# smarterclayton/kubernetes

Measured on AMD Instinct MI355X. Metric: pods scheduled/sec, higher is better.
Workload: dtype int64; 1 GPU; config2: 5000 nodes, 1776000 pods, DefaultProvider; nodes=5000, prefix_pods=0, placed_in_prefix=0, parallelism=speculative windows: all-CU snapshot scoring + in-order exact resolver

## Files before the change

kubernetes_amd/csrc/ksg_internal.h:

```cpp
#pragma once
#include <stdint.h>
#include "../../include/kschedgpu.h"

#define KSG_NT 1024
#define KSG_NWAVE (KSG_NT / 64)
#define KSG_R_LDS 32
#define KSG_R_MAX 128

#define KSG_MODE_EVAL 0
#define KSG_MODE_BEGIN 1

#define KSG_SCORE_NONE (-0x7fffffffffffffffLL - 1)
#define KSG_S32_NONE ((int32_t)0x80000000)
#define KSG_SCORE_BOUND (1LL << 30)
#define KSG_WIN_MAX_ANTI 4
#define KSG_WIN_LR_BOUND (1LL << 49)
#define KSG_WIN_XREQ_BOUND (1LL << 16)

struct KsgDev {
  uint32_t n_nodes, nw;
  uint32_t lo, hi;
  uint32_t wlo, nwords;
  uint32_t n_pairs, n_services, max_keys, n_domains_total;
  uint32_t preds;
  int64_t w_lr, w_spread;
  uint32_t n_anti;
  int64_t w_anti[KSG_MAX_ANTI];
  uint32_t anti_dom_off[KSG_MAX_ANTI];
  uint32_t n_aff;
  uint32_t n_aff_groups;
  uint32_t aff_group_mask[KSG_MAX_AFF_GROUPS];
  int32_t equal_fallback;
  int32_t empty_priorities;
  int32_t has_static_score;
  int32_t has_static_fit;
  int32_t dbg;
  int32_t wide;
  uint32_t rr_dz;
  int32_t* dbgbuf;
  const int64_t* cap_cpu;
  const int64_t* cap_mem;
  const double* inv10_cpu;
  const double* inv10_mem;
  int64_t* used_cpu;
  int64_t* used_mem;
  const uint64_t* draws;
  const uint64_t* static_fit;
  const int64_t* static_score;
  uint64_t* keymap;
  const uint64_t* pairmap;
  int32_t* svc_cnt;
  uint64_t* svc_bits;
  int32_t* svc_max;
  int32_t* svc_total;
  int32_t* svc_peer;
  const int32_t* anti_domain;
  const int32_t* aff_pair;
  void* score_scratch;
  uint32_t ext_filters;
  int32_t w_taint, w_bal;
  uint32_t n_scalar;
  const int64_t* scalar_cap;
  int64_t* scalar_used;
  const uint64_t* taintmap;
  const uint64_t* ntaint;
};

struct KsgStaticCfg {
  uint32_t n_presence;
  uint32_t presence_n_keys[KSG_MAX_PRESENCE];
  uint32_t presence_keys[KSG_MAX_PRESENCE][KSG_MAX_PRESENCE_KEYS];
  uint32_t presence_flag[KSG_MAX_PRESENCE];
  uint32_t n_pref;
  uint32_t pref_key[KSG_MAX_LABEL_PREF];
  uint32_t pref_presence[KSG_MAX_LABEL_PREF];
  int64_t w_pref[KSG_MAX_LABEL_PREF];
  int64_t w_equal;
  uint32_t n_anti;
  uint32_t anti_key[KSG_MAX_ANTI];
  uint32_t n_aff;
  uint32_t aff_key[KSG_MAX_AFF];
};

#define KSG_WIN_INLINE 24
#define KSG_WIN_SUM_AFF 4
struct KsgWinSum {
  int32_t m0;
  uint32_t k0;
  int32_t error;
  int32_t service;
  int32_t host;
  int32_t spread_max;
  int32_t svc_total;
  uint32_t n_inline;
  int64_t milli_cpu;
  int64_t memory;
  int32_t req_aff[KSG_WIN_SUM_AFF];
  uint16_t n_ports, n_pds, n_sel, n_svcs;
  uint32_t xmask;
  uint32_t ids[KSG_WIN_INLINE];
  int32_t xreq[4];
  uint32_t pad2;
};
static_assert(sizeof(KsgWinSum) == 192, "KsgWinSum layout");
#define KSG_WIN_SUM_DWORDS (sizeof(KsgWinSum) / 4)

#define KSG_MAX_WORLD 16
struct KsgWinXchg {
  const uint8_t* buf;
  uint64_t blk;
  uint32_t ostride;
  uint32_t wcap;
  uint32_t world;
  uint32_t fit_off;
  uint32_t wlo[KSG_MAX_WORLD], nw[KSG_MAX_WORLD];
  int32_t* dcnt;
  uint32_t dcnt_n;
  uint8_t* img;
  const ksg_pod_ext* exts;
  uint32_t img_stride;
  uint32_t esc;
  uint32_t efit_off;
  uint32_t d1;
  uint32_t d1_off;
  int32_t* tmax;
  uint64_t* psoft;
  int32_t* thist;
  uint32_t rr;
  uint32_t dz;
  uint32_t b_off;
  int32_t* dmb;
  const uint64_t* zmap;
};
#define KSG_TBINS 65
#define KSG_RR_MAXZ 32
#define KSG_RR_MAXSVC 4096

#define KSG_HALT_OVERSIZE 4
#define KSG_HALT_BADCOUNT 8
#define KSG_HALT_HANG 9
#define KSG_HALT_BAD 10
struct KsgWinRun {
  uint32_t pos;
  uint32_t n;
  uint32_t halt;
  uint32_t windows;
  uint32_t stops[4];
};

struct KsgFused {
  const ksg_pod* batch;
  const uint32_t* ids;
  KsgWinRun* run_out;
  uint32_t* cnt;
  uint32_t set;
  uint32_t ngroups;
};

typedef ksg_shard_record KsgRecordHdr;

#define KSG_EXPLAIN_TILE 256
#define KSG_EXPLAIN_CHUNK 32

#define KSG_ADMIT_MODE_CAPACITY 1
#define KSG_ADMIT_MODE_SELECTOR 2

struct KsgPatch {
  uint64_t addr;
  uint64_t value;
  uint32_t width;
  uint32_t pad;
};

#define KSG_SRV_CHUNKS 64
#define KSG_SRV_CHUNK_DW 3
#define KSG_SRV_HDR_DW 8
#define KSG_SRV_INLINE_DW (KSG_SRV_CHUNKS * KSG_SRV_CHUNK_DW - KSG_SRV_HDR_DW)
#define KSG_SRV_EXT_DW 4096
#define KSG_SRV_PAY_DW (KSG_SRV_INLINE_DW + KSG_SRV_EXT_DW)
#define KSG_SRV_PATCHES 4096
#define KSG_SRV_MAX_R 16
enum {
  KSG_SRV_BEGIN = 1,
  KSG_SRV_COMMIT = 2,
  KSG_SRV_PATCH = 3,
  KSG_SRV_EXIT = 4,
};
enum { KSG_SRVH_KIND = 0, KSG_SRVH_ARG, KSG_SRVH_RSV, KSG_SRVH_FLAGS, KSG_SRVH_PAYDW, KSG_SRVH_IDS_AT,
       KSG_SRVH_EXT_AT, KSG_SRVH_NPATCH };
#define KSG_SRV_BADREQ 0xFFFFFFFEu
#define KSG_SRV_RESP_REJECTED 12
#define KSG_SRVF_WANT_FAIL 1u
#define KSG_SRVF_EXT 2u
#define KSG_GSRV_NT 256
#define KSG_GSRV_MAXW 255
#define KSG_GSRV_TIEW 16
#define KSG_GSRV_MAXD 64
struct alignas(64) KsgSrvPart {
  uint32_t seq;
  int32_t max;
  uint32_t cnt;
  uint32_t err;
  uint64_t tie[4];
  uint32_t stamp[4];
};
struct KsgSrvBox {
  uint32_t req[KSG_SRV_CHUNKS * 4];
  uint32_t creq[KSG_SRV_CHUNKS * 4];
  uint32_t cext[KSG_SRV_EXT_DW];
  uint32_t resp[16];
  uint32_t ext[KSG_SRV_EXT_DW];
  KsgPatch patch[KSG_SRV_PATCHES];
  uint32_t dbg[256];
  uint64_t ties[KSG_SRV_MAX_R * 16];
  KsgSrvPart part[KSG_GSRV_MAXW];
  uint64_t part_tie[KSG_GSRV_MAXW * KSG_GSRV_TIEW];
};
struct KsgSrvGrid {
  uint32_t quit;
  uint32_t applied;
  uint32_t pad[14];
  uint64_t tmx[KSG_GSRV_MAXW];
  uint64_t dcx[KSG_GSRV_MAXW * KSG_GSRV_MAXD];
};
struct KsgSrvArgs {
  KsgSrvBox* box;
  uint8_t* fail;
  uint32_t start_seq;
  uint64_t idle_ticks;
  uint32_t stamps;
  KsgSrvGrid* grid;
  uint32_t n_workers;
  uint32_t epoch;
  uint32_t grid_opts;
};
#define KSG_GSRV_POLL1 256u

#ifdef __HIP__
#define KSG_HD __host__ __device__
#else
#define KSG_HD
#endif

static inline KSG_HD uint64_t ksg_splitmix_next(uint64_t* s) {
  uint64_t z = (*s += 0x9E3779B97F4A7C15ULL);
  z = (z ^ (z >> 30)) * 0xBF58476D1CE4E5B9ULL;
  z = (z ^ (z >> 27)) * 0x94D049BB133111EBULL;
  return z ^ (z >> 31);
}
static inline KSG_HD uint64_t ksg_rng_step(const uint64_t* draws) { return draws ? 1ULL : 0x9E3779B97F4A7C15ULL; }
static inline KSG_HD uint64_t ksg_rng_draw(const uint64_t* draws, uint64_t s) {
  if (draws) return draws[s];
  return ksg_splitmix_next(&s) >> 1;
}
```

kubernetes_amd/csrc/ksg_plain.hip:

```cpp
#include "ksg_resolver.h"
#include "ksg_score.h"

#define KSG_NCAND 6
#define KSG_CSV_MAX 10
#define KSG_NO_CAND 7u
#define KSG_CSNAP 10
#define KSG_XR_W 20
#ifndef KSG_PL_PROD_SLEEP
#define KSG_PL_PROD_SLEEP 1
#endif
#ifndef KSG_PL_CHK_SLEEP
#define KSG_PL_CHK_SLEEP 2
#endif
#ifndef KSG_PL_XN_SLEEP
#define KSG_PL_XN_SLEEP 0
#endif
__host__ __device__ constexpr uint32_t pl_nt(int P) { return P >= 32 ? 512u : 768u; }
#define KSG_PL_FW KSG_RES_P0
#define KSG_PL_P0 (KSG_PL_FW + 1)
__host__ __device__ constexpr bool pl_d1(uint32_t P) { return P <= 4; }

struct alignas(16) PlCommit {
  uint32_t kind;
  uint32_t slot;
// ... 1689 lines not shown
        const uint32_t na = (uint32_t)__builtin_amdgcn_readlane((int)(lo ? cn0 : cn1), (int)l);
        const uint32_t bd = (uint32_t)__popcll(__ballot(d0 < pa)) + (uint32_t)__popcll(__ballot(d1 < pa)) +
                            (xdp < pa ? 1u : 0u);
        const uint32_t ba = (uint32_t)__popcll(__ballot(ap0 != ~0u && (ap0 < pa || (ap0 == pa && cn0 < na)))) +
                            (uint32_t)__popcll(__ballot(ap1 != ~0u && (ap1 < pa || (ap1 == pa && cn1 < na))));
        if (pa - bd + ba == t) woff = na;
      }
      for (uint32_t j = 0; woff == ~0u && j <= n_add && j <= t; ++j) {
        const uint32_t tp = t0_minus_drops(t - j);
        if (tp >= k0) continue;
        const uint32_t ca = (uint32_t)__popcll(__ballot(ap0 != ~0u && ap0 <= tp)) +
                            (uint32_t)__popcll(__ballot(ap1 != ~0u && ap1 <= tp));
        if (ca == j) woff = t0_node(tp);
      }
    } else if (dropped == 0) {
      woff = (uint32_t)pred;
    } else if (dropped <= 2) {
      KSG_COUNTP(7, 64)
      uint32_t pa = ~0u, pb = ~0u;
      for (uint64_t mm = msk0; mm; mm &= mm - 1) {
        const uint32_t p = (uint32_t)__builtin_amdgcn_readlane((int)dp0, (int)__builtin_ctzll(mm));
        if (p < pa) { pb = pa; pa = p; } else if (p < pb) { pb = p; }
      }
      for (uint64_t mm = msk1; mm; mm &= mm - 1) {
        const uint32_t p = (uint32_t)__builtin_amdgcn_readlane((int)dp1, (int)__builtin_ctzll(mm));
        if (p < pa) { pb = pa; pa = p; } else if (p < pb) { pb = p; }
      }
      if (x_drop) {
        const uint32_t p = xpos0 + (uint32_t)__popcll(t0x & ((1ULL << (xnode & 63)) - 1ULL));
        if (p < pa) { pb = pa; pa = p; } else if (p < pb) { pb = p; }
      }
      const uint32_t ix = (uint32_t)__builtin_amdgcn_readlane((int)rmod, (int)dropped);
      const uint32_t t = k - 1 - ix;
      uint32_t tp = t;
      if (pa <= tp) ++tp;
      if (pb <= tp) ++tp;
      woff = (uint32_t)__builtin_amdgcn_readlane((int)cand, (int)((dropped == 1 ? 1u : 3u) + (tp - t)));
    } else {
      KSG_COUNTP(7, 64)
      uint32_t ix;
      if (dropped < 64) {
        ix = (uint32_t)__builtin_amdgcn_readlane((int)rmod, (int)dropped);
      } else {
        ix = umod64_32(r_draw(), k);
      }
      woff = t0_node(t0_minus_drops(k - 1 - ix));
    }
    if (KSG_UNLIKELY(woff >= d.hi - d.lo)) {
      resolved = i;
      reason = KSG_STOP_BAD;
      break;
    }
    const uint64_t cm = __ballot(cand == woff);
    const uint32_t cidx = cm ? (uint32_t)__builtin_ctzll(cm) : KSG_NO_CAND;
    if (lane == 0) {
      L_cm[i].xn = woff | (cidx << 28);
      if constexpr (STAMP) ctl->t_n = (uint32_t)__builtin_amdgcn_s_memtime();
      st_post(&ctl->xn_seq, i + 1);
    }
    KSG_STAMPP(3)
    const uint64_t hit0 = __ballot(cn0 == woff);
    const uint64_t hit1 = __ballot(cn1 == woff);
    const bool in_c = (hit0 | hit1) != 0;
    uint32_t slot, base_nk = 0, base_ns = 0;
    int64_t base_dc = 0, base_dm = 0;
    if (in_c) {
      slot = hit0 ? (uint32_t)__builtin_ctzll(hit0) : 64u + (uint32_t)__builtin_ctzll(hit1);
      const uint32_t sl = slot & 63;
      base_nk = (uint32_t)__builtin_amdgcn_readlane((int)(slot < 64 ? sk0 : sk1), (int)sl);
      base_ns = (uint32_t)__builtin_amdgcn_readlane((int)(slot < 64 ? ss0 : ss1), (int)sl);
      if (KSG_UNLIKELY(base_nk + nk > KSG_SLOT_KEYS || base_ns + n_svcs > KSG_SLOT_SVCS)) {
        resolved = i;
        reason = KSG_STOP_SLOT;
        break;
      }
      base_dc = (int64_t)readlane64((uint64_t)(slot < 64 ? dc0 : dc1), (int)sl);
      base_dm = (int64_t)readlane64((uint64_t)(slot < 64 ? dm0 : dm1), (int)sl);
    } else {
      if (KSG_UNLIKELY(n_slots == KSG_MAX_SLOTS)) {
        resolved = i;
        reason = KSG_STOP_SLOT;
        break;
      }
      slot = n_slots++;
    }
    const int64_t new_dc = (int64_t)((uint64_t)base_dc + (uint64_t)pv.req_c);
    const int64_t new_dm = (int64_t)((uint64_t)base_dm + (uint64_t)pv.req_m);
    const uint32_t wn = d.lo + woff;
    KSG_STAMPP(4)
    {
      uint32_t* row = L_cl + (size_t)slot * KSG_CL_W;
      const uint32_t kt = lane - WS_IDS, st_ = lane - (WS_IDS + nk + n_sel);
      if (kt < nk) row[KSG_CL_KEY + base_nk + kt] = rec;
      if (st_ < n_svcs) row[KSG_CL_SV + base_ns + st_] = rec;
    }
    if (lane == 0) {
      *reinterpret_cast<uint4*>(&L_cm[i]) =
          uint4{1u, slot, woff, (in_c ? 0u : 1u) | (cidx << 1) | (n_svcs << 8) | (base_ns << 16) | (base_nk << 24)};
      L_cm[i].out = (int32_t)wn;
      st_post(&ctl->sel_seq, i + 1);
    }
    if ((int32_t)woff != pred) KSG_COUNTP(8, 64)
    if (lane == (slot & 63)) {
      if (slot >= 64) {
        if (!in_c) cn1 = woff;
        dc1 = new_dc;
        dm1 = new_dm;
        sk1 = base_nk + nk;
        ss1 = base_ns + n_svcs;
      } else {
        if (!in_c) cn0 = woff;
        dc0 = new_dc;
        dm0 = new_dm;
        sk0 = base_nk + nk;
        ss0 = base_ns + n_svcs;
      }
    }
    have_x = true;
    xnode = woff;
    xslot = slot;
    x_fresh = !in_c;
    ++n_draws;
    KSG_STAMPP(5)
  }
  if (lane == 0) {
    ctl->resolved = resolved;
    st_rel(&ctl->stop, 1u);
  }
  bool drained = false;
  for (uint32_t spin = 0; spin <= 16 * KSG_SPIN_LIMIT; ++spin) {
    bool done = ld_acq(&ctl->fin_x) != 0 && ld_acq(&ctl->fin_f) != 0;
#pragma unroll
    for (int c = 0; c < KSG_RES_NCHK; ++c) done = done && ld_acq(&ctl->fin[c]) != 0;
    if (done) {
      drained = true;
      break;
    }
  }
  if (ld_acq(&ctl->bad)) reason = KSG_STOP_BAD;
  else if (!drained || ld_acq(&ctl->hang)) reason = KSG_STOP_HANG;
  if constexpr (STAMP) {
    if (d.dbgbuf && (lane < 16 || lane == 43 || lane == 44)) atomicAdd(d.dbgbuf + lane, (int32_t)(t_acc / 64));
  }
#undef KSG_STAMPP
#undef KSG_COUNTP
  const uint32_t n_peer = __builtin_amdgcn_readfirstlane(ctl->n_peer);
  for (uint32_t t = lane; t < n_peer; t += 64) {
    const uint32_t sv = L_peer[2 * t];
    int32_t expect = -1;
    __hip_atomic_compare_exchange_strong(d.svc_peer + sv, &expect, (int32_t)L_peer[2 * t + 1], __ATOMIC_RELAXED,
                                         __ATOMIC_RELAXED, __HIP_MEMORY_SCOPE_AGENT);
  }
  for (uint32_t t = lane; t < resolved; t += 64) out[t] = L_cm[t].out;
  if (esc && x.tmax) {
    for (uint32_t t = lane; t < wcap; t += 64) x.tmax[t] = 0;
    for (uint32_t t = lane; t < n_pods * KSG_TBINS; t += 64) x.thist[t] = 0;
  }
  if (XS) {
    for (uint32_t t = lane; t < resolved; t += 64) {
      if (L_cm[t].kind != 1) continue;
      const ksg_pod_ext& pe = x.exts[pos + t];
      const uint32_t wn = d.lo + L_cm[t].node;
      for (uint32_t r = 0; r < d.n_scalar; ++r)
        if (pe.scalar[r] != 0)
          __hip_atomic_fetch_add(reinterpret_cast<uint64_t*>(d.scalar_used + (size_t)r * d.n_nodes + wn),
                                 (uint64_t)pe.scalar[r], __ATOMIC_RELAXED, __HIP_MEMORY_SCOPE_AGENT);
    }
    drain_stores();
  }
  if (lane == 0) {
    *rng_io = rng0 + (uint64_t)n_draws * ksg_rng_step(d.draws);
    if constexpr (STAMP && FUSED)
      if (d.dbgbuf) __hip_atomic_store(d.dbgbuf + 55, 0, __ATOMIC_RELAXED, __HIP_MEMORY_SCOPE_AGENT);
    KsgWinRun r = *run;
    if (reason == KSG_STOP_HANG) {
      r.halt = KSG_HALT_HANG;
    } else if (reason == KSG_STOP_BAD) {
      r.halt = KSG_HALT_BAD;
    } else if (reason == KSG_STOP_OVERSIZE) {
      r.halt = KSG_HALT_OVERSIZE;
    } else if (resolved == 0 || resolved > n_pods) {
      r.halt = KSG_HALT_BADCOUNT;
    } else {
      r.pos = pos + resolved;
      r.windows += 1;
      r.stops[1] += reason == 1 ? 1u : 0u;
      r.stops[2] += reason == 2 ? 1u : 0u;
      r.stops[3] += reason == 3 ? 1u : 0u;
    }
    *run_out = r;
  }
}

template <int P, bool STAMP, bool XS>
__global__ __launch_bounds__(pl_nt(P)) void ksg_win_plain_kernel(KsgDev d, uint32_t wcap, KsgWinRun* run,
                                                            const KsgWinSum* __restrict__ sums, const KsgWinXchg x,
                                                            uint64_t* rng_io, int32_t* __restrict__ out_batch) {
  win_plain_body<P, STAMP, XS, false>(d, wcap, run, sums, x, rng_io, out_batch, KsgFused{});
}

template <int P, bool STAMP>
__global__ __launch_bounds__(pl_nt(P)) void ksg_win_fused_kernel(KsgDev d, uint32_t wcap, KsgWinRun* run,
                                                            const KsgWinSum* __restrict__ sums, const KsgWinXchg x,
                                                            uint64_t* rng_io, int32_t* __restrict__ out_batch,
                                                            const KsgFused f) {
  win_plain_body<P, STAMP, false, true>(d, wcap, run, sums, x, rng_io, out_batch, f);
}

template <int PP, bool ST, bool XS, bool FU = false>
static hipError_t win_plain_launch_x(const KsgDev& d, uint32_t wcap, size_t lds, KsgWinRun* run,
                                     const KsgWinSum* sums, const KsgWinXchg& x, uint64_t* rng, int32_t* out,
                                     hipStream_t st, const KsgFused& f = KsgFused{}, uint32_t grid = 1) {
  const void* fn;
  if constexpr (FU) fn = reinterpret_cast<const void*>(ksg_win_fused_kernel<PP, ST>);
  else fn = reinterpret_cast<const void*>(ksg_win_plain_kernel<PP, ST, XS>);
  static bool once = false;
  if (!once) {
    (void)hipFuncSetAttribute(fn, hipFuncAttributeMaxDynamicSharedMemorySize, 160 * 1024);
    (void)hipGetLastError();
    once = true;
  }
  if constexpr (FU)
    hipLaunchKernelGGL((ksg_win_fused_kernel<PP, ST>), dim3(grid), dim3(pl_nt(PP)), lds, st, d, wcap, run, sums, x,
                       rng, out, f);
  else
    hipLaunchKernelGGL((ksg_win_plain_kernel<PP, ST, XS>), dim3(grid), dim3(pl_nt(PP)), lds, st, d, wcap, run, sums,
                       x, rng, out);
  return hipGetLastError();
}

static bool plain_xs(const KsgDev& d, const KsgWinXchg& x) {
  return x.exts != nullptr && (((d.ext_filters & KSG_EXT_SCALAR) && d.n_scalar > 0) || x.esc);
}

static bool plain_stamp(const KsgDev& d) { return (d.dbg & 8) != 0 || ((uint32_t)d.dbg & KSG_DBG_RESOLVER_MASK) != 0; }

#define KSG_PLAIN_CASE(PP, XS)                                                                              \
  if (P == PP)                                                                                              \
    return plain_stamp(d) ? win_plain_launch_x<PP, true, XS>(d, wcap, lds, run, sums, x, rng, out, st)    \
                          : win_plain_launch_x<PP, false, XS>(d, wcap, lds, run, sums, x, rng, out, st);

hipError_t ksg_launch_win_plain_ilp(const KsgDev& d, uint32_t P, uint32_t wcap, size_t lds, KsgWinRun* run,
                                    const KsgWinSum* sums, const KsgWinXchg& x, uint64_t* rng, int32_t* out,
                                    hipStream_t st)
#ifdef KSG_PLAIN_LARGE_TU
{
  if (plain_xs(d, x)) {
    KSG_PLAIN_CASE(1, true)
    KSG_PLAIN_CASE(2, true)
    KSG_PLAIN_CASE(4, true)
    KSG_PLAIN_CASE(8, true)
    KSG_PLAIN_CASE(16, true)
    KSG_PLAIN_CASE(32, true)
  } else {
    KSG_PLAIN_CASE(16, false)
    KSG_PLAIN_CASE(32, false)
  }
  return hipErrorInvalidValue;
}
#else
    ;

static uint32_t plain_P(const KsgDev& d);
uint32_t ksg_win_plain_lds(const KsgDev& d, uint32_t wcap) {
  return plain_lds_offsets(plain_P(d), (d.n_services + 31) / 32, wcap).total;
}

static uint32_t plain_P(const KsgDev& d) {
  const uint32_t P = (d.nwords + 63) / 64;
  return P <= 1 ? 1 : P <= 2 ? 2 : P <= 4 ? 4 : P <= 8 ? 8 : P <= 16 ? 16 : 32;
}

uint32_t ksg_win_t0_stride(const KsgDev& d) { return t0img_stride(plain_P(d)); }

hipError_t ksg_launch_win_t0(const KsgDev& d, uint32_t wcap, const KsgWinRun* run, const KsgWinXchg& x,
                             hipStream_t st) {
  const uint32_t P = plain_P(d);
#define KSG_T0_CASE(PP) \
  if (P == PP) hipLaunchKernelGGL((ksg_win_t0_kernel<PP>), dim3(wcap), dim3(256), 0, st, d.nwords, wcap, run, x);
  KSG_T0_CASE(1)
  KSG_T0_CASE(2)
  KSG_T0_CASE(4)
  KSG_T0_CASE(8)
  KSG_T0_CASE(16)
  KSG_T0_CASE(32)
#undef KSG_T0_CASE
  return hipGetLastError();
}

hipError_t ksg_launch_win_plain(const KsgDev& d, uint32_t P, uint32_t wcap, KsgWinRun* run, const KsgWinSum* sums,
                                const KsgWinXchg& x, uint64_t* rng, int32_t* out, hipStream_t st) {
  const size_t lds = plain_lds_offsets(P, (d.n_services + 31) / 32, wcap).total;
  if (P >= 16 || plain_xs(d, x)) return ksg_launch_win_plain_ilp(d, P, wcap, lds, run, sums, x, rng, out, st);
  KSG_PLAIN_CASE(1, false)
  KSG_PLAIN_CASE(2, false)
  KSG_PLAIN_CASE(4, false)
  KSG_PLAIN_CASE(8, false)
  return hipErrorInvalidValue;
}

bool ksg_win_fused_ok(const KsgDev& d) { return plain_P(d) >= 1 && d.nwords > 0; }

uint32_t ksg_win_fused_groups(const KsgDev& d, uint32_t wcap) {
  const uint32_t pg = (uint32_t)pl_pg((int)plain_P(d));
  return (wcap + pg - 1) / pg;
}

hipError_t ksg_launch_win_fused(const KsgDev& d, uint32_t wcap, KsgWinRun* run, const KsgWinSum* sums,
                                const KsgWinXchg& x, uint64_t* rng, int32_t* out, const KsgFused& f, uint32_t grid,
                                hipStream_t st) {
  const uint32_t P = plain_P(d);
  const size_t lds = std::max<size_t>(plain_lds_offsets(P, (d.n_services + 31) / 32, wcap).total,
                                      (size_t)(pl_nt(P) / 64) * pl_pg((int)P) * sizeof(KsgWinSum));
  const bool stamp = plain_stamp(d);
#define KSG_FUSED_CASE(PP)                                                                                  \
  if (P == PP)                                                                                              \
    return stamp ? win_plain_launch_x<PP, true, false, true>(d, wcap, lds, run, sums, x, rng, out, st, f, grid) \
                 : win_plain_launch_x<PP, false, false, true>(d, wcap, lds, run, sums, x, rng, out, st, f, grid);
  KSG_FUSED_CASE(1)
  KSG_FUSED_CASE(2)
  KSG_FUSED_CASE(4)
  KSG_FUSED_CASE(8)
  KSG_FUSED_CASE(16)
  KSG_FUSED_CASE(32)
#undef KSG_FUSED_CASE
  return hipErrorInvalidValue;
}
#endif
#undef KSG_PLAIN_CASE
```

kubernetes_amd/csrc/ksg_runtime.cpp:

```cpp
#include <hip/hip_runtime.h>
#include <rccl/rccl.h>

#include <algorithm>
#include <array>
#include <atomic>
#include <chrono>
#include <cmath>
#include <cstdarg>
#include <cstdio>
#include <cstring>
#include <map>
#include <mutex>
#include <string>
#include <unordered_map>
#include <unordered_set>
#include <vector>

#include "ksg_internal.h"
#include "ksg_shard.h"


hipError_t ksg_launch_batch(int R, bool anti, const KsgDev& d, const ksg_pod* pods,
                            const uint32_t* ids, uint32_t n, uint64_t* rng, int32_t* out,
                            hipStream_t st, const ksg_pod_ext* ext = nullptr);
hipError_t ksg_launch_scan(int R, bool anti, const KsgDev& d, const ksg_pod* pods,
                           const uint32_t* ids, int mode, int phase, uint8_t* fail_out,
                           int64_t* score_out, uint8_t* record, int32_t* dpart,
                           const int32_t* dglobal, hipStream_t st, const ksg_pod_ext* ext = nullptr);
hipError_t ksg_launch_win_eval(const KsgDev& d, int mode, const ksg_pod* batch, const uint32_t* ids,
                               const KsgWinRun* run, uint32_t wcap, KsgWinSum* sums, uint64_t* wbits, int32_t* wmax,
                               uint32_t ostride, int32_t* dcnt, uint64_t* wfit, int32_t* dmb, uint64_t* wbz,
                               uint32_t dz, hipStream_t st, const ksg_pod_ext* exts = nullptr,
                               int32_t* tmax = nullptr, uint64_t* psoft = nullptr, int32_t* thist = nullptr);
hipError_t ksg_launch_zonemap(uint32_t n_nodes, const int32_t* anti_domain, uint32_t d0, uint32_t nw,
                              uint64_t* zmap, hipStream_t st);
hipError_t ksg_launch_win_t0(const KsgDev& d, uint32_t wcap, const KsgWinRun* run, const KsgWinXchg& x,
                             hipStream_t st);
uint32_t ksg_win_t0_stride(const KsgDev& d);
hipError_t ksg_launch_win_resolve(const KsgDev& d, uint32_t wcap, KsgWinRun* run, const KsgWinSum* sums,
                                  const KsgWinXchg& x, uint64_t* rng, int32_t* out, hipStream_t st);
bool ksg_win_fused_ok(const KsgDev& d);
uint32_t ksg_win_fused_groups(const KsgDev& d, uint32_t wcap);
hipError_t ksg_launch_win_fused(const KsgDev& d, uint32_t wcap, KsgWinRun* run, const KsgWinSum* sums,
                                const KsgWinXchg& x, uint64_t* rng, int32_t* out, const KsgFused& f, uint32_t grid,
                                hipStream_t st);
uint32_t ksg_win_max_window(const KsgDev& d);
hipError_t ksg_launch_decide(const KsgDev& d, const ksg_pod* pods, const uint32_t* ids,
                             const uint8_t* records, uint32_t rec_bytes, uint32_t world,
                             const uint32_t* shard_wlo, int mode, uint64_t tie_index,
                             uint64_t* rng, int32_t* out, uint32_t out_idx, int64_t* summary,
                             hipStream_t st, const ksg_pod_ext* ext = nullptr);
hipError_t ksg_launch_static(const KsgStaticCfg& sc, uint32_t n_nodes, const ksg_node* nodes,
                             const uint32_t* node_pairs, const uint32_t* pair_keys,
                             const int32_t* dom_of_pair, uint32_t n_pairs, uint32_t nw,
                             uint64_t* static_fit, int64_t* static_score, int32_t* anti_domain,
                             int32_t* aff_pair, unsigned long long* pairmap, hipStream_t st);
hipError_t ksg_launch_patch(const KsgPatch* patches, uint32_t n, hipStream_t st);
hipError_t ksg_launch_static_terms(const KsgStaticCfg& sc, uint32_t n_nodes, const ksg_node* nodes,
                                   const uint32_t* node_pairs, const uint32_t* pair_keys, uint32_t n_pairs, uint32_t nw,
                                   uint64_t* fit, int64_t* score, hipStream_t st);
hipError_t ksg_launch_static_fold(uint64_t* static_fit, int64_t* static_score, const uint64_t* xfit,
                                  const int64_t* xscore, uint32_t nw, uint32_t n, int own_fit, int own_score,
                                  hipStream_t st);
hipError_t ksg_launch_serve(int R, bool anti, bool ext, const KsgDev& d, const KsgSrvArgs& a, hipStream_t st);
hipError_t ksg_launch_serve_grid(int npt, bool ext, const KsgDev& d, const KsgSrvArgs& a, hipStream_t st);
hipError_t ksg_launch_admit(const ksg_admission_set* sets, uint32_t n_sets, const ksg_pod* pods,
                            const uint32_t* ids, const uint32_t* pairs, int mode, uint8_t* out, hipStream_t st);
hipError_t ksg_launch_explain(const KsgDev& d, const ksg_pod* pods, const ksg_pod_ext* exts, const uint32_t* ids,
                              uint32_t n_pods, uint8_t* codes, uint32_t* hist, uint8_t* err, hipStream_t st);

namespace {

struct PodRec {
  uint32_t host;
  int64_t cpu, mem;
  int64_t scalar[KSG_MAX_SCALAR];
  std::vector<uint32_t> keys;
  std::vector<uint32_t> svcs;
  uint64_t seq;
};

constexpr uint32_t kMaxNodesPerShard = KSG_R_MAX * KSG_NT;
constexpr uint32_t kFctlGroups = 1024;
constexpr size_t kFctlRuns = 2 * sizeof(KsgWinRun);
constexpr size_t kFctlBytes = kFctlRuns + (size_t)2 * kFctlGroups * 8 * sizeof(uint32_t);
constexpr size_t kExplainStageBytes = (size_t)64 << 20;

const unsigned kTimingEvent =
    (getenv("KSG_EVENT_FENCE") && atoi(getenv("KSG_EVENT_FENCE"))) ? hipEventDefault : hipEventDisableSystemFence;

}

struct ksg_ctx {
  ksg_config cfg{};
  int device = 0, rank = 0, world = 1;
  hipStream_t st = nullptr;
  ncclComm_t comm = nullptr;
  bool xchg = false;
  double ppw_est = 0.0;
  double round_margin = 1.0;
  uint8_t* h_up = nullptr;
  size_t h_up_cap = 0;
  uint8_t* h_dn = nullptr;
  size_t h_dn_cap = 0;
  ksg_allgather_fn xfn = nullptr;
  void* xuser = nullptr;
  uint8_t *h_xsend = nullptr, *h_xrecv = nullptr;
  size_t h_xsend_cap = 0, h_xrecv_cap = 0;
  hipEvent_t ev0 = nullptr, ev1 = nullptr;
  hipEvent_t ev_wait = nullptr;
  bool spin_wait = true;
  double last_ms = 0.0;
  std::string err;

  bool have_cluster = false;
  bool diverged = false;
  uint32_t N = 0, nw = 0, n_pairs = 0, S = 0, D = 0;
  uint32_t lo = 0, hi = 0, wlo = 0, nwords = 0, nwords_max = 0;
  std::vector<uint32_t> shard_wlo_h;
  int R = 1;
  size_t lds = 0;
  KsgDev dev{};
  std::vector<void*> cluster_allocs;
  uint32_t* d_shard_wlo = nullptr;

  ksg_pod* d_pods = nullptr;
  size_t pods_cap = 0;
  uint32_t* d_ids = nullptr;
  size_t ids_cap = 0;
  uint8_t* d_fail = nullptr;
  int64_t* d_score = nullptr;
  uint8_t* d_rec_send = nullptr;
  uint8_t* d_rec_recv = nullptr;
  uint32_t rec_bytes = 0;
  int32_t* d_dpart = nullptr;
  int32_t* d_dglobal = nullptr;
  int32_t* d_out = nullptr;
  size_t out_cap = 0;
  uint64_t* d_rng = nullptr;
  int64_t* d_summary = nullptr;
  uint8_t* d_one = nullptr;
  size_t one_cap = 0;
  const ksg_pod* one_pod = nullptr;
  const uint32_t* one_ids = nullptr;
  uint8_t* h_map = nullptr;
  uint8_t* d_map = nullptr;
  KsgPatch* d_patch = nullptr;
  size_t patch_cap = 0;
  uint64_t* d_draws = nullptr;
  size_t draws_cap = 0;
  uint64_t draw_tmp = 0;
  uint8_t* d_admit = nullptr;
  size_t admit_cap = 0;
  uint8_t* d_xcodes = nullptr;
  size_t xcodes_cap = 0;
  uint8_t* d_xhist = nullptr;
  size_t xhist_cap = 0;
  hipEvent_t ev_x0 = nullptr, ev_x1 = nullptr;
  double last_explain_ms = 0.0;
  std::vector<KsgPatch> patches;

  std::vector<int64_t> used_c, used_m;
  int64_t mu_max = 0;
  bool mu_neg = false, mu_dirty = true;
  std::unordered_map<uint64_t, uint32_t> key_ref;
  std::vector<int32_t> svc_cnt;
  std::vector<std::unordered_map<uint32_t, int32_t>> svc_ext;
  std::vector<int32_t> svc_max, svc_total, svc_peer;
  std::vector<int32_t> h_aff_pair;
  std::vector<std::map<uint64_t, uint32_t>> svc_members;
  std::unordered_map<uint64_t, PodRec> pods;
  uint64_t seq = 0;

  uint32_t window = 128;
  uint32_t ev_stride = 4;
  uint32_t ev_phase = 0;
  KsgWinSum* d_winsum = nullptr;
  uint8_t* d_xsend = nullptr;
  uint8_t* d_xrecv = nullptr;
  uint8_t* d_t0img = nullptr;
  size_t t0img_cap = 0;
  int32_t* d_dcnt = nullptr;
  int32_t* d_dmb = nullptr;
  uint64_t* d_zmap = nullptr;
  size_t win_cap = 0, xsend_cap = 0, xrecv_cap = 0, dcnt_cap = 0, dmb_cap = 0;
  int32_t* d_etmax = nullptr;
  int32_t* d_ethist = nullptr;
  size_t ethist_cap = 0;
  uint64_t* d_epsoft = nullptr;
  size_t etmax_cap = 0, epsoft_cap = 0;
  KsgWinRun* d_run = nullptr;
  KsgWinRun* h_run = nullptr;
  uint32_t last_stats[4] = {0, 0, 0, 0};
  std::vector<hipEvent_t> wev;
  double last_kms[3] = {0, 0, 0};
  double last_t0ms = 0;
  double last_wsum = 0;
  bool dbg_fail_next = false;
  uint32_t dbg_corrupt = 0;
  bool win_d1 = true;
  bool win_fused = true;
  uint32_t fused_grid = 0;
  uint32_t fused_max_words = 1024;
  uint8_t* d_fctl = nullptr;
  uint8_t* h_fctl = nullptr;
  double last_hus[8] = {0, 0, 0, 0, 0, 0, 0, 0};
  double totals[24] = {};
  int64_t max_cap = 0, min_cap = 0;

  std::vector<ksg_pod> dfr_pods;
  std::vector<uint32_t> dfr_ids;
  std::vector<int32_t> dfr_out;
  std::unordered_set<uint64_t> dfr_uids;
  int64_t dfr_sum = 0;
  bool dfr_neg = false;
  bool lr_wild = false;
  int64_t used_hi = 0;
  unsigned __int128 dfr_req = 0;

  bool ext_on = false;
  ksg_ext_config ext{};
  std::vector<int64_t> sc_used;
  std::unordered_map<uint64_t, std::array<int64_t, KSG_MAX_SCALAR>> ext_scalar;
  const ksg_pod_ext* cur_ext = nullptr;
  ksg_pod_ext* d_pext = nullptr;
  size_t pext_cap = 0;
  ksg_pod_ext* d_one_ext = nullptr;

  bool srv_enabled = true;
  bool srv_running = false;
  KsgSrvBox* srv_box = nullptr;
  KsgSrvBox* srv_dbox = nullptr;
  uint8_t* srv_fail = nullptr;
  uint8_t* srv_dfail = nullptr;
  size_t srv_fail_cap = 0;
  uint32_t srv_seq = 0;
  uint64_t srv_idle_us = 20000;
  bool pend_srv = false;
  uint32_t srv_bhdr[KSG_SRV_HDR_DW] = {};
  std::vector<uint64_t> srv_tw;
  uint32_t srv_unacked = 0;
  uint32_t srv_served = 0;
  uint32_t srv_last_ctl = 0;
  bool srv_pext_on = false;
  ksg_pod_ext srv_pext{};
  uint64_t srv_launches = 0;
  bool srv_grid_on = true;
  uint32_t srv_npt4_min = 16384;
  uint32_t srv_grid_min = 0;
  bool srv_grid_ext = true;
  KsgSrvGrid* srv_grid = nullptr;
  size_t srv_grid_cap = 0;
  uint32_t srv_epoch = 0;
  bool srv_stamps = false;
  int64_t srv_grid_opts = -1;
  bool srv_debug = false;
  unsigned __int128 static_mag = 0;
  const ksg_node* d_lbl_nodes = nullptr;
  const uint32_t* d_lbl_pairs = nullptr;
  const uint32_t* d_lbl_keys = nullptr;
  bool srv_trace = false;
  double srv_stage[6] = {};
  uint64_t srv_stamped = 0;

  bool pending = false;
  uint64_t pending_k = 0;
  ksg_pod pend{};
  std::vector<uint32_t> pend_ids;

  std::recursive_mutex mu;
  struct Queued {
    bool add;
    uint32_t host;
    ksg_pod pod;
    std::vector<uint32_t> ids;
    uint64_t uid;
  };
  std::vector<Queued> upd_q;
  std::unordered_set<uint64_t> q_added, q_removed;
};

#define KSG_LOCK(c) std::lock_guard<std::recursive_mutex> ksg_lock_((c)->mu)

namespace {

int fail(ksg_ctx* c, int code, const char* fmt, ...) {
  char buf[512];
  va_list ap;
  va_start(ap, fmt);
  vsnprintf(buf, sizeof buf, fmt, ap);
  va_end(ap);
  if (c) c->err = buf;
  return code;
}

#define HIPCHK(c, x)                                                                 \
  do {                                                                               \
    hipError_t e_ = (x);                                                             \
    if (e_ != hipSuccess)                                                            \
      return fail((c), KSG_ERR_HIP, "%s:%d %s: %s", __FILE__, __LINE__, #x,          \
                  hipGetErrorString(e_));                                            \
  } while (0)

#define NCCLCHK(c, x)                                                                \
  do {                                                                               \
    ncclResult_t r_ = (x);                                                           \
    if (r_ != ncclSuccess)                                                           \
      return fail((c), KSG_ERR_RCCL, "%s:%d %s: %s", __FILE__, __LINE__, #x,         \
                  ncclGetErrorString(r_));                                           \
  } while (0)

template <typename T>
int dalloc(ksg_ctx* c, T** p, size_t count, std::vector<void*>* owner) {
  void* q = nullptr;
  HIPCHK(c, hipMalloc(&q, std::max<size_t>(count, 1) * sizeof(T)));
  HIPCHK(c, hipMemsetAsync(q, 0, std::max<size_t>(count, 1) * sizeof(T), c->st));
  *p = static_cast<T*>(q);
  if (owner) owner->push_back(q);
  return KSG_OK;
}

void free_cluster(ksg_ctx* c) {
  for (void* p : c->cluster_allocs) (void)hipFree(p);
  c->cluster_allocs.clear();
  c->have_cluster = false;
}

int grow(ksg_ctx* c, void** p, size_t* cap, size_t need, size_t elem) {
  if (need <= *cap && *p) return KSG_OK;
  size_t nc = std::max<size_t>(need, std::max<size_t>(*cap * 2, 64));
  if (*p) (void)hipFree(*p);
  *p = nullptr;
  HIPCHK(c, hipMalloc(p, nc * elem));
  *cap = nc;
  return KSG_OK;
}

int pick_R(uint32_t shard_nodes) {
  const uint32_t r = (shard_nodes + KSG_NT - 1) / KSG_NT;
  int R = 1;
  while ((uint32_t)R < r) R <<= 1;
  return R;
}

void patch32(ksg_ctx* c, const void* addr, int32_t v) {
  c->patches.push_back(KsgPatch{(uint64_t)(uintptr_t)addr, (uint64_t)(uint32_t)v, 0, 0});
}
void patch64(ksg_ctx* c, const void* addr, int64_t v) {
  c->patches.push_back(KsgPatch{(uint64_t)(uintptr_t)addr, (uint64_t)v, 1, 0});
}
void patch_or(ksg_ctx* c, const void* addr, uint64_t v) {
  c->patches.push_back(KsgPatch{(uint64_t)(uintptr_t)addr, v, 2, 0});
}
void patch_andnot(ksg_ctx* c, const void* addr, uint64_t v) {
  c->patches.push_back(KsgPatch{(uint64_t)(uintptr_t)addr, v, 3, 0});
}

int srv_flush_patches(ksg_ctx* c);

int flush_patches(ksg_ctx* c) {
  if (c->patches.empty()) return KSG_OK;
  if (c->srv_running) return srv_flush_patches(c);
  int rc = grow(c, (void**)&c->d_patch, &c->patch_cap, c->patches.size(), sizeof(KsgPatch));
  if (rc) return rc;
  HIPCHK(c, hipMemcpyAsync(c->d_patch, c->patches.data(), c->patches.size() * sizeof(KsgPatch),
                           hipMemcpyHostToDevice, c->st));
  HIPCHK(c, ksg_launch_patch(c->d_patch, (uint32_t)c->patches.size(), c->st));
  HIPCHK(c, hipStreamSynchronize(c->st));
  c->patches.clear();
  return KSG_OK;
}

int32_t peer_code(ksg_ctx* c, uint32_t s) {
  if (c->svc_members[s].empty()) return -1;
  const uint32_t h = c->svc_members[s].begin()->second;
  return h < c->N ? (int32_t)h : -2;
}

int32_t recompute_max(ksg_ctx* c, uint32_t s) {
  int32_t m = 0;
  const int32_t* row = c->svc_cnt.data() + (size_t)s * c->N;
  for (uint32_t n = 0; n < c->N; ++n) m = std::max(m, row[n]);
  for (auto& kv : c->svc_ext[s]) m = std::max(m, kv.second);
  return m;
}

int mirror_add(ksg_ctx* c, uint32_t h, const ksg_pod* p, const uint32_t* ids, bool emit) {
  if (c->pods.count(p->uid)) return fail(c, KSG_ERR_ARG, "duplicate pod uid %llu", (unsigned long long)p->uid);
  PodRec r;
  r.host = h;
  r.cpu = p->milli_cpu;
  r.mem = p->memory;
  r.seq = ++c->seq;
  for (uint32_t i = 0; i < p->n_ports; ++i) r.keys.push_back(ids[p->ports_off + i]);
  for (uint32_t i = 0; i < p->n_pds; ++i) r.keys.push_back(ids[p->pds_off + i]);
  for (uint32_t i = 0; i < p->n_svcs; ++i) r.svcs.push_back(ids[p->svcs_off + i]);
  for (uint32_t k : r.keys)
    if (k >= c->cfg.max_conflict_keys)
      return fail(c, KSG_ERR_CAPACITY, "conflict key %u >= max_conflict_keys %u", k, c->cfg.max_conflict_keys);
  for (uint32_t s : r.svcs)
    if (s >= c->S) return fail(c, KSG_ERR_ARG, "service %u >= n_services %u", s, c->S);
  for (uint32_t q = 0; q < KSG_MAX_SCALAR; ++q) r.scalar[q] = 0;
  if (c->ext_on && c->ext.n_scalar) {
    auto it = c->ext_scalar.find(p->uid);
    if (it != c->ext_scalar.end())
      for (uint32_t q = 0; q < c->ext.n_scalar; ++q) r.scalar[q] = it->second[q];
    if (h < c->N)
      for (uint32_t q = 0; q < c->ext.n_scalar; ++q) {
        if (!r.scalar[q]) continue;
        int64_t& u = c->sc_used[(size_t)q * c->N + h];
        u = (int64_t)((uint64_t)u + (uint64_t)r.scalar[q]);
        if (emit) patch64(c, c->dev.scalar_used + (size_t)q * c->N + h, u);
      }
  }
  if (h < c->N) {
    c->used_c[h] = (int64_t)((uint64_t)c->used_c[h] + (uint64_t)r.cpu);
    c->used_m[h] = (int64_t)((uint64_t)c->used_m[h] + (uint64_t)r.mem);
    c->used_hi = std::max(c->used_hi, std::max(c->used_c[h], c->used_m[h]));
    if (c->mu_neg || c->used_c[h] < 0 || c->used_m[h] < 0) c->mu_dirty = true;
    else c->mu_max = std::max(c->mu_max, std::max(c->used_c[h], c->used_m[h]));
    if (emit) {
      patch64(c, c->dev.used_cpu + h, c->used_c[h]);
      patch64(c, c->dev.used_mem + h, c->used_m[h]);
    }
    for (uint32_t k : r.keys) {
      const uint32_t ref = ++c->key_ref[((uint64_t)k << 32) | h];
      if (ref == 1 && emit) patch_or(c, c->dev.keymap + (size_t)k * c->nw + (h >> 6), 1ULL << (h & 63));
    }
  }
  for (uint32_t s : r.svcs) {
    int32_t v;
    if (h < c->N) {
      v = ++c->svc_cnt[(size_t)s * c->N + h];
      if (emit) patch32(c, c->dev.svc_cnt + (size_t)s * c->N + h, v);
      if (emit && v == 1) patch_or(c, c->dev.svc_bits + (size_t)s * c->nw + (h >> 6), 1ULL << (h & 63));
    } else {
      v = ++c->svc_ext[s][h];
    }
    if (v > c->svc_max[s]) {
      c->svc_max[s] = v;
      if (emit) patch32(c, c->dev.svc_max + s, v);
    }
    ++c->svc_total[s];
    if (emit) patch32(c, c->dev.svc_total + s, c->svc_total[s]);
    c->svc_members[s][r.seq] = h;
    const int32_t pc = peer_code(c, s);
    if (pc != c->svc_peer[s]) {
      c->svc_peer[s] = pc;
      if (emit) patch32(c, c->dev.svc_peer + s, pc);
    }
  }
  c->pods.emplace(p->uid, std::move(r));
  return KSG_OK;
}

void reset_mirror(ksg_ctx* c) {
  c->used_c.assign(c->N, 0);
  c->mu_dirty = true;
  c->used_hi = 0;
  c->used_m.assign(c->N, 0);
  c->sc_used.assign((size_t)c->ext.n_scalar * c->N, 0);
  c->ext_scalar.clear();
  c->key_ref.clear();
  c->svc_cnt.assign((size_t)c->S * c->N, 0);
  c->svc_ext.assign(c->S, {});
  c->svc_max.assign(c->S, 0);
  c->svc_total.assign(c->S, 0);
  c->svc_peer.assign(c->S, -1);
  c->svc_members.assign(c->S, {});
  c->pods.clear();
  c->seq = 0;
  c->patches.clear();
  c->pending = false;
  c->pend_srv = false;
  c->upd_q.clear();
  c->q_added.clear();
  c->q_removed.clear();
}

int check_pod(ksg_ctx* c, const ksg_pod* p, const uint32_t* ids, size_t n_ids) {
  auto in = [&](uint32_t off, uint32_t n) { return (size_t)off + n <= n_ids; };
  if (!in(p->ports_off, p->n_ports) || !in(p->pds_off, p->n_pds) || !in(p->sel_off, p->n_sel) ||
      !in(p->svcs_off, p->n_svcs))
    return fail(c, KSG_ERR_ARG, "pod id list out of range");
  if (p->host < -2 || p->host >= (int32_t)c->N) return fail(c, KSG_ERR_ARG, "pod host %d out of range", p->host);
  if (p->service < -1 || p->service >= (int32_t)c->S) return fail(c, KSG_ERR_ARG, "pod service out of range");
  for (uint32_t i = 0; i < p->n_ports; ++i)
    if (ids[p->ports_off + i] >= c->cfg.max_conflict_keys) return fail(c, KSG_ERR_CAPACITY, "port key out of range");
  for (uint32_t i = 0; i < p->n_pds; ++i)
    if (ids[p->pds_off + i] >= c->cfg.max_conflict_keys) return fail(c, KSG_ERR_CAPACITY, "pd key out of range");
  for (uint32_t i = 0; i < p->n_sel; ++i)
    if (ids[p->sel_off + i] >= c->n_pairs) return fail(c, KSG_ERR_ARG, "selector pair out of range");
  for (uint32_t i = 0; i < p->n_svcs; ++i)
    if (ids[p->svcs_off + i] >= c->S) return fail(c, KSG_ERR_ARG, "service id out of range");
  for (uint32_t j = 0; j < c->cfg.n_aff_labels; ++j)
    if (p->aff_pair[j] >= (int32_t)c->n_pairs || p->aff_pair[j] < KSG_AFF_INVALID)
      return fail(c, KSG_ERR_ARG, "affinity pair out of range");
  return KSG_OK;
}

int grow_host(ksg_ctx* c, uint8_t** p, size_t* cap, size_t need);

int upload_pods(ksg_ctx* c, const ksg_pod* pods, uint32_t n, const uint32_t* ids, size_t n_ids) {
  int rc = grow(c, (void**)&c->d_pods, &c->pods_cap, n, sizeof(ksg_pod));
  if (rc) return rc;
  rc = grow(c, (void**)&c->d_ids, &c->ids_cap, std::max<size_t>(n_ids, 1), sizeof(uint32_t));
  if (rc) return rc;
  const size_t pb = (size_t)n * sizeof(ksg_pod), ib = n_ids * sizeof(uint32_t);
  if ((rc = grow_host(c, &c->h_up, &c->h_up_cap, pb + ib))) return rc;
  memcpy(c->h_up, pods, pb);
  if (n_ids) memcpy(c->h_up + pb, ids, ib);
  HIPCHK(c, hipMemcpyAsync(c->d_pods, c->h_up, pb, hipMemcpyHostToDevice, c->st));
  if (n_ids) HIPCHK(c, hipMemcpyAsync(c->d_ids, c->h_up + pb, ib, hipMemcpyHostToDevice, c->st));
  return KSG_OK;
}

int upload_one(ksg_ctx* c, const ksg_pod* pod, const uint32_t* ids, size_t n_ids) {
  const size_t pb = (sizeof(ksg_pod) + 15) & ~(size_t)15, ib = std::max<size_t>(n_ids, 1) * sizeof(uint32_t);
  const size_t eo = (pb + ib + 15) & ~(size_t)15, eb = c->ext_on ? sizeof(ksg_pod_ext) : 0;
  int rc = grow(c, (void**)&c->d_one, &c->one_cap, eo + eb, 1);
  if (rc) return rc;
  if ((rc = grow_host(c, &c->h_up, &c->h_up_cap, eo + eb))) return rc;
  memcpy(c->h_up, pod, sizeof(ksg_pod));
  if (n_ids) memcpy(c->h_up + pb, ids, n_ids * sizeof(uint32_t));
  if (eb) {
    if (c->cur_ext) memcpy(c->h_up + eo, c->cur_ext, eb);
    else memset(c->h_up + eo, 0, eb);
  }
  HIPCHK(c, hipMemcpyAsync(c->d_one, c->h_up, eb ? eo + eb : pb + (n_ids ? n_ids * sizeof(uint32_t) : 0),
                           hipMemcpyHostToDevice, c->st));
  c->one_pod = reinterpret_cast<const ksg_pod*>(c->d_one);
  c->one_ids = reinterpret_cast<const uint32_t*>(c->d_one + pb);
  c->d_one_ext = eb ? reinterpret_cast<ksg_pod_ext*>(c->d_one + eo) : nullptr;
  return KSG_OK;
}

int ensure_map(ksg_ctx* c) {
  if (c->h_map) return KSG_OK;
  HIPCHK(c, hipHostMalloc((void**)&c->h_map, 64, hipHostMallocCoherent));
  void* dp = nullptr;
  HIPCHK(c, hipHostGetDevicePointer(&dp, c->h_map, 0));
  c->d_map = static_cast<uint8_t*>(dp);
  return KSG_OK;
}

size_t pod_ids_extent(const ksg_pod* p) {
  size_t e = 0;
  e = std::max<size_t>(e, (size_t)p->ports_off + p->n_ports);
  e = std::max<size_t>(e, (size_t)p->pds_off + p->n_pds);
  e = std::max<size_t>(e, (size_t)p->sel_off + p->n_sel);
  e = std::max<size_t>(e, (size_t)p->svcs_off + p->n_svcs);
  return e;
}
size_t call_ids_extent(const ksg_ctx* c, const ksg_pod* p) {
  size_t e = pod_ids_extent(p);
  if (c->cur_ext) {
    e = std::max<size_t>(e, (size_t)c->cur_ext->hard_off + c->cur_ext->n_hard);
    e = std::max<size_t>(e, (size_t)c->cur_ext->soft_off + c->cur_ext->n_soft);
  }
  return e;
}

uint8_t* rec_buf(ksg_ctx* c) { return c->xchg ? c->d_rec_recv : c->d_rec_send; }

bool anti_on(const ksg_ctx* c) { return c->cfg.n_anti > 0 && c->dev.n_domains_total > 0; }

int grow_host(ksg_ctx* c, uint8_t** p, size_t* cap, size_t need) {
  if (*cap >= need) return KSG_OK;
  const size_t nc = std::max<size_t>(need, std::max<size_t>(*cap * 2, 4096));
  if (*p) (void)hipHostFree(*p);
  *p = nullptr;
  *cap = 0;
  HIPCHK(c, hipHostMalloc((void**)p, nc, hipHostMallocDefault));
  *cap = nc;
  return KSG_OK;
}

int allgather(ksg_ctx* c, const void* dsend, void* drecv, size_t bytes) {
  if (c->comm) {
    NCCLCHK(c, ncclAllGather(dsend, drecv, bytes, ncclUint8, c->comm, c->st));
    return KSG_OK;
  }
  if (!c->xfn) return fail(c, KSG_ERR_STATE, "sharded context has neither an RCCL communicator nor ksg_set_allgather");
  int rc;
  if ((rc = grow_host(c, &c->h_xsend, &c->h_xsend_cap, bytes)) ||
      (rc = grow_host(c, &c->h_xrecv, &c->h_xrecv_cap, bytes * c->world)))
    return rc;
  HIPCHK(c, hipMemcpyAsync(c->h_xsend, dsend, bytes, hipMemcpyDeviceToHost, c->st));
  HIPCHK(c, hipStreamSynchronize(c->st));
  if ((rc = c->xfn(c->xuser, c->h_xsend, c->h_xrecv, (uint64_t)bytes)) != 0)
    return fail(c, KSG_ERR_RCCL, "allgather callback returned %d", rc);
  HIPCHK(c, hipMemcpyAsync(drecv, c->h_xrecv, bytes * c->world, hipMemcpyHostToDevice, c->st));
  return KSG_OK;
}

int allreduce_sum_i32(ksg_ctx* c, const int32_t* dsend, int32_t* drecv, uint32_t n) {
  if (c->comm) {
    NCCLCHK(c, ncclAllReduce(dsend, drecv, n, ncclInt32, ncclSum, c->comm, c->st));
    return KSG_OK;
  }
  if (!c->xfn) return fail(c, KSG_ERR_STATE, "sharded context has neither an RCCL communicator nor ksg_set_allgather");
  const size_t bytes = (size_t)n * 4;
  int rc;
  if ((rc = grow_host(c, &c->h_xsend, &c->h_xsend_cap, bytes)) ||
      (rc = grow_host(c, &c->h_xrecv, &c->h_xrecv_cap, bytes * (c->world + 1))))
    return rc;
  HIPCHK(c, hipMemcpyAsync(c->h_xsend, dsend, bytes, hipMemcpyDeviceToHost, c->st));
  HIPCHK(c, hipStreamSynchronize(c->st));
  if ((rc = c->xfn(c->xuser, c->h_xsend, c->h_xrecv, (uint64_t)bytes)) != 0)
    return fail(c, KSG_ERR_RCCL, "allgather callback returned %d", rc);
  int32_t* all = reinterpret_cast<int32_t*>(c->h_xrecv);
  int32_t* sum = all + (size_t)n * c->world;
  for (uint32_t i = 0; i < n; ++i) {
    uint32_t acc = 0;
    for (int g = 0; g < c->world; ++g) acc += (uint32_t)all[(size_t)g * n + i];
    sum[i] = (int32_t)acc;
  }
  HIPCHK(c, hipMemcpyAsync(drecv, sum, bytes, hipMemcpyHostToDevice, c->st));
  return KSG_OK;
}

int allreduce_max_i32(ksg_ctx* c, const int32_t* dsend, int32_t* drecv, uint32_t n) {
  if (c->comm) {
    NCCLCHK(c, ncclAllReduce(dsend, drecv, n, ncclInt32, ncclMax, c->comm, c->st));
    return KSG_OK;
  }
  if (!c->xfn) return fail(c, KSG_ERR_STATE, "sharded context has neither an RCCL communicator nor ksg_set_allgather");
  const size_t bytes = (size_t)n * 4;
  int rc;
  if ((rc = grow_host(c, &c->h_xsend, &c->h_xsend_cap, bytes)) ||
      (rc = grow_host(c, &c->h_xrecv, &c->h_xrecv_cap, bytes * (c->world + 1))))
    return rc;
  HIPCHK(c, hipMemcpyAsync(c->h_xsend, dsend, bytes, hipMemcpyDeviceToHost, c->st));
  HIPCHK(c, hipStreamSynchronize(c->st));
  if ((rc = c->xfn(c->xuser, c->h_xsend, c->h_xrecv, (uint64_t)bytes)) != 0)
    return fail(c, KSG_ERR_RCCL, "allgather callback returned %d", rc);
  int32_t* all = reinterpret_cast<int32_t*>(c->h_xrecv);
  int32_t* mx = all + (size_t)n * c->world;
  for (uint32_t i = 0; i < n; ++i) {
    int32_t m = all[i];
    for (int g = 1; g < c->world; ++g) m = std::max(m, all[(size_t)g * n + i]);
    mx[i] = m;
  }
  HIPCHK(c, hipMemcpyAsync(drecv, mx, bytes, hipMemcpyHostToDevice, c->st));
  return KSG_OK;
}

int scan_exchange(ksg_ctx* c, const ksg_pod* dpod, const uint32_t* dids, int mode, uint8_t* fail_out,
                  int64_t* score_out, const ksg_pod_ext* dext) {
  const bool anti = anti_on(c);
  const bool tt = dext != nullptr && c->ext.w_taint_toleration != 0;
  if ((anti || tt) && c->xchg) {
    HIPCHK(c, ksg_launch_scan(c->R, anti, c->dev, dpod, dids, mode, 1, nullptr, nullptr, c->d_rec_send,
                              c->d_dpart, nullptr, c->st, dext));
    const uint32_t D = c->dev.n_domains_total;
    int rc = anti ? allreduce_sum_i32(c, c->d_dpart, c->d_dglobal, D) : KSG_OK;
    if (!rc && tt) rc = allreduce_max_i32(c, c->d_dpart + D, c->d_dglobal + D, 1);
    if (rc) return rc;
    HIPCHK(c, ksg_launch_scan(c->R, anti, c->dev, dpod, dids, mode, 2, fail_out, score_out, c->d_rec_send,
                              nullptr, c->d_dglobal, c->st, dext));
  } else {
    HIPCHK(c, ksg_launch_scan(c->R, anti, c->dev, dpod, dids, mode, 0, fail_out, score_out, c->d_rec_send,
                              nullptr, nullptr, c->st, dext));
  }
  if (mode == KSG_MODE_BEGIN) {
    if (c->xchg) {
      int rc = allgather(c, c->d_rec_send, c->d_rec_recv, c->rec_bytes);
      if (rc) return rc;
    }
  }
  return KSG_OK;
}

KsgDev full_geometry(const ksg_ctx* c) {
  KsgDev f = c->dev;
  f.lo = 0;
  f.hi = c->N;
  f.wlo = 0;
  f.nwords = c->nw;
  return f;
}

bool use_window(ksg_ctx* c, const ksg_pod* pods, uint32_t n) {
  if (c->window == 0 || c->nw > 32 * 64 || ksg_win_max_window(full_geometry(c)) < 8) return false;
  if (c->ext_on) {
    if (anti_on(c)) {
      if (c->ext.w_taint_toleration != 0 || c->ext.w_balanced != 0) return false;
      if (c->cur_ext)
        for (uint32_t i = 0; i < n; ++i)
          for (uint32_t r = 0; r < c->ext.n_scalar; ++r)
            if (c->cur_ext[i].scalar[r] != 0) return false;
    }
    if (c->ext.w_taint_toleration != 0 && !c->dev.ntaint) return false;
    if (c->cur_ext)
      for (uint32_t i = 0; i < n; ++i)
        for (uint32_t r = 0; r < c->ext.n_scalar; ++r)
          if (c->cur_ext[i].scalar[r] < 0 || c->cur_ext[i].scalar[r] > KSG_WIN_XREQ_BOUND) return false;
  }
  if (c->dev.wide) return false;
  if (c->cfg.w_least_requested < 0 || c->cfg.w_service_spreading < 0) return false;
  const int64_t lim = KSG_WIN_LR_BOUND;
  if (c->max_cap > lim || c->min_cap < 0) return false;
  if (c->mu_dirty) {
    c->mu_max = 0;
    c->mu_neg = false;
    for (uint32_t i = 0; i < c->N; ++i) {
      c->mu_neg |= c->used_c[i] < 0 || c->used_m[i] < 0;
      c->mu_max = std::max<int64_t>(c->mu_max, std::max<int64_t>(c->used_c[i], c->used_m[i]));
    }
    c->mu_dirty = false;
  }
  if (c->mu_neg) return false;
  const int64_t mu = c->mu_max;
  int64_t sum = c->dfr_sum;
  for (uint32_t i = 0; i < n; ++i) {
    if (pods[i].milli_cpu < 0 || pods[i].memory < 0) return false;
    sum += std::min<int64_t>(std::min<int64_t>(pods[i].milli_cpu, lim) + std::min<int64_t>(pods[i].memory, lim), lim);
    if (sum > lim) return false;
  }
  return mu + sum <= lim;
}

unsigned __int128 score_bound(const ksg_config& cf, int64_t w_taint, int64_t w_bal) {
  auto mag = [](int64_t w) -> unsigned __int128 { return w < 0 ? (unsigned __int128)(0 - (uint64_t)w) : (unsigned __int128)w; };
  unsigned __int128 b = 10 * (mag(cf.w_least_requested) + mag(cf.w_service_spreading) + mag(w_taint) + mag(w_bal)) +
                        mag(cf.w_equal);
  for (uint32_t a = 0; a < cf.n_anti; ++a) b += 10 * mag(cf.w_anti[a]);
  for (uint32_t q = 0; q < cf.n_label_pref; ++q) b += 10 * mag(cf.w_pref[q]);
  return b;
}

int cluster_ok(ksg_ctx* c) {
  if (!c->have_cluster) return fail(c, KSG_ERR_STATE, "ksg_set_cluster not called");
  if (c->diverged)
    return fail(c, KSG_ERR_STATE, "device state diverged from the host mirror (a batch failed after its device work "
                "started, or the drop-in server rejected a commit): call ksg_set_cluster");
  return KSG_OK;
}

void drop_deferred(ksg_ctx* c) {
  c->dfr_pods.clear();
  c->dfr_ids.clear();
  c->dfr_out.clear();
  c->dfr_uids.clear();
  c->dfr_sum = 0;
  c->dfr_req = 0;
  c->dfr_neg = false;
}

int flush_deferred(ksg_ctx* c) {
  int rc = KSG_OK;
  for (size_t i = 0; i < c->dfr_out.size() && rc == KSG_OK; ++i)
    if (c->dfr_out[i] >= 0) rc = mirror_add(c, (uint32_t)c->dfr_out[i], &c->dfr_pods[i], c->dfr_ids.data(), false);
  drop_deferred(c);
  return rc;
}

int ensure_out(ksg_ctx* c, size_t n) { return grow(c, (void**)&c->d_out, &c->out_cap, n, sizeof(int32_t)); }

int wait_device(ksg_ctx* c) {
  if (!c->spin_wait || !c->ev_wait) {
    HIPCHK(c, hipStreamSynchronize(c->st));
    return KSG_OK;
  }
  HIPCHK(c, hipEventRecord(c->ev_wait, c->st));
  hipError_t e;
  while ((e = hipEventQuery(c->ev_wait)) == hipErrorNotReady) {
  }
  if (e != hipSuccess) return fail(c, KSG_ERR_HIP, "hipEventQuery: %s", hipGetErrorString(e));
  return KSG_OK;
}

uint32_t srv_npt(const ksg_ctx* c) { return c->hi - c->lo > c->srv_npt4_min ? 4u : 1u; }

bool srv_grid(const ksg_ctx* c) {
  const uint32_t n = c->hi - c->lo, per = KSG_GSRV_NT * srv_npt(c);
  return c->srv_grid_on && !(anti_on(c) && (c->ext_on || c->dev.n_domains_total > KSG_GSRV_MAXD)) &&
         !(c->ext_on && !c->srv_grid_ext) &&
         n > c->srv_grid_min &&
         (n + per - 1) / per <= KSG_GSRV_MAXW;
}

bool srv_eligible(const ksg_ctx* c) {
  return c->srv_enabled && c->world == 1 && !c->xchg && (c->R <= KSG_SRV_MAX_R || srv_grid(c)) && !c->dev.wide &&
         c->N > 0;
}

int srv_alloc(ksg_ctx* c) {
  if (!c->srv_box) {
    HIPCHK(c, hipHostMalloc((void**)&c->srv_box, sizeof(KsgSrvBox), hipHostMallocCoherent | hipHostMallocMapped));
    memset(c->srv_box, 0, sizeof(KsgSrvBox));
    void* dp = nullptr;
    HIPCHK(c, hipHostGetDevicePointer(&dp, c->srv_box, 0));
    c->srv_dbox = static_cast<KsgSrvBox*>(dp);
  }
  return KSG_OK;
}

int srv_launch(ksg_ctx* c) {
  if (int rc = srv_alloc(c)) return rc;
  const uint32_t r0 = __atomic_load_n(&c->srv_box->resp[0], __ATOMIC_ACQUIRE);
  if ((int32_t)(r0 - c->srv_served) > 0) c->srv_served = r0;
  const uint32_t start_seq = c->srv_served;
  const size_t nf = ((size_t)(c->hi - c->lo) + 3 & ~(size_t)3) + 64;
  if (c->srv_fail_cap < nf) {
    if (c->srv_fail) (void)hipHostFree(c->srv_fail);
    c->srv_fail = nullptr;
    c->srv_fail_cap = 0;
    HIPCHK(c, hipHostMalloc((void**)&c->srv_fail, nf, hipHostMallocCoherent | hipHostMallocMapped));
    void* dp = nullptr;
    HIPCHK(c, hipHostGetDevicePointer(&dp, c->srv_fail, 0));
    c->srv_dfail = static_cast<uint8_t*>(dp);
    c->srv_fail_cap = nf;
  }
  KsgSrvArgs a{c->srv_dbox, c->srv_dfail, start_seq, (uint64_t)c->srv_idle_us * 100,
               (c->srv_stamps ? 1u : 0u) | (c->srv_debug ? 2u : 0u),
               nullptr, 0, ++c->srv_epoch, 0};
  if (srv_grid(c)) {
    const uint32_t n = c->hi - c->lo;
    const size_t need = sizeof(KsgSrvGrid);
    if (c->srv_grid_cap < need) {
      if (c->srv_grid) (void)hipFree(c->srv_grid);
      c->srv_grid = nullptr;
      c->srv_grid_cap = 0;
      HIPCHK(c, hipMalloc((void**)&c->srv_grid, need));
      HIPCHK(c, hipMemsetAsync(c->srv_grid, 0, need, c->st));
      c->srv_grid_cap = need;
    }
    a.grid = c->srv_grid;
    const uint32_t npt = srv_npt(c);
    a.n_workers = (n + KSG_GSRV_NT * npt - 1) / (KSG_GSRV_NT * npt);
    a.grid_opts = c->srv_grid_opts >= 0 ? (uint32_t)c->srv_grid_opts : a.n_workers > 64 ? 0x10u : 0u;
    HIPCHK(c, ksg_launch_serve_grid((int)npt, c->ext_on, c->dev, a, c->st));
  } else {
    HIPCHK(c, ksg_launch_serve(c->R, anti_on(c), c->ext_on, c->dev, a, c->st));
  }
  c->srv_running = true;
  ++c->srv_launches;
  return KSG_OK;
}

int srv_wait(ksg_ctx* c, uint32_t seq, uint32_t parts) {
  const uint32_t* rs = c->srv_box->resp;
  auto done = [&]() {
    if (!parts) return (int32_t)(__atomic_load_n(&rs[0], __ATOMIC_ACQUIRE) - seq) >= 0;
    for (uint32_t q = 0; q < parts; ++q)
      if (__atomic_load_n(&c->srv_box->part[q].seq, __ATOMIC_ACQUIRE) != seq ||
          __atomic_load_n(&c->srv_box->part[q].stamp[3], __ATOMIC_ACQUIRE) != seq)
        return false;
    return true;
  };
  auto t0 = std::chrono::steady_clock::now();
  uint32_t spins = 0, relaunches = 0;
  while (!done()) {
    if ((++spins & 255) != 0) continue;
    const double us = std::chrono::duration<double, std::micro>(std::chrono::steady_clock::now() - t0).count();
    if (us < 20.0) continue;
    const hipError_t q = hipStreamQuery(c->st);
    if (q == hipSuccess) {
      if (done()) break;
      if (++relaunches > 3) return fail(c, KSG_ERR_HIP, "drop-in server exits without serving request %u", seq);
      c->srv_running = false;
      if (c->srv_trace) fprintf(stderr, "srv relaunch start %u (waiting %u)\n", c->srv_served, seq);
      if (int rc = srv_launch(c)) return rc;
      t0 = std::chrono::steady_clock::now();
    } else if (q != hipErrorNotReady) {
      c->srv_running = false;
      std::string marks;
      if (c->srv_debug)
        for (int i = 0; i < 12; ++i) {
          const uint32_t m = __atomic_load_n(&c->srv_box->dbg[i], __ATOMIC_RELAXED);
          marks += " " + std::to_string(m >> 8) + ":" + std::to_string(m & 255);
        }
      return fail(c, KSG_ERR_HIP, "drop-in server: %s (request %u%s)", hipGetErrorString(q), seq, marks.c_str());
    } else if (us > 5e6) {
      return fail(c, KSG_ERR_HIP, "drop-in server did not answer request %u in 5 s", seq);
    }
  }
  std::atomic_thread_fence(std::memory_order_acquire);
  if ((int32_t)(seq - c->srv_served) > 0) c->srv_served = seq;
  return KSG_OK;
}

int srv_settle(ksg_ctx* c) {
  if (!c->srv_unacked) return KSG_OK;
  const uint32_t u = c->srv_unacked;
  c->srv_unacked = 0;
  if ((int32_t)(c->srv_served - u) < 0)
    if (int rc = srv_wait(c, u, 0)) return rc;
  if (__atomic_load_n(&c->srv_box->resp[KSG_SRV_RESP_REJECTED], __ATOMIC_ACQUIRE) == u) {
    c->diverged = true;
    return fail(c, KSG_ERR_STATE, "drop-in server rejected commit request %u (ksg_set_cluster resyncs)", u);
  }
  return KSG_OK;
}

int srv_post(ksg_ctx* c, const uint32_t* hdr_in, uint32_t* seq_out) {
  if (!c->srv_running) {
    if (int rc = srv_launch(c)) return rc;
  }
  const bool ctl = hdr_in[KSG_SRVH_KIND] != KSG_SRV_BEGIN;
  if (ctl) {
    if (int rc = srv_settle(c)) return rc;
  }
  uint32_t hdr[KSG_SRV_HDR_DW];
  memcpy(hdr, hdr_in, sizeof hdr);
  if (!ctl) hdr[KSG_SRVH_ARG] = c->srv_last_ctl;
  if (c->dbg_corrupt) {
    const uint32_t bit = hdr[KSG_SRVH_KIND] == KSG_SRV_COMMIT ? 1u : hdr[KSG_SRVH_KIND] == KSG_SRV_BEGIN ? 2u : 0u;
    if (c->dbg_corrupt & bit) {
      hdr[KSG_SRVH_IDS_AT] = KSG_SRV_PAY_DW + 1;
      c->dbg_corrupt &= ~bit;
    }
  }
  const uint32_t seq = ++c->srv_seq;
  if (ctl) c->srv_last_ctl = seq;
  if (c->srv_trace)
    fprintf(stderr, "srv post %u kind %u arg %u served %u\n", seq, hdr[KSG_SRVH_KIND], hdr[KSG_SRVH_ARG], c->srv_served);
  uint32_t* req = ctl ? c->srv_box->creq : c->srv_box->req;
  for (uint32_t i = 0; i < KSG_SRV_HDR_DW; ++i) req[4 * (i / KSG_SRV_CHUNK_DW) + i % KSG_SRV_CHUNK_DW] = hdr[i];
  std::atomic_thread_fence(std::memory_order_release);
  for (uint32_t q = 0; q < KSG_SRV_CHUNKS; ++q) __atomic_store_n(&req[4 * q + 3], seq, __ATOMIC_RELEASE);
// ... 90 lines not shown
                    (unsigned __int128)KSG_SCORE_BOUND ||
                (c->lr_wild && c->cfg.w_least_requested != 0);
}

int note_requests(ksg_ctx* c, const ksg_pod* pods, uint32_t n) {
  if (c->lr_wild || c->cfg.w_least_requested == 0) return KSG_OK;
  bool wild = c->used_hi < 0;
  unsigned __int128 sum = 0;
  for (uint32_t i = 0; i < n; ++i) {
    wild |= pods[i].milli_cpu < 0 || pods[i].memory < 0;
    if (!wild) sum += (uint64_t)std::max(pods[i].milli_cpu, pods[i].memory);
  }
  wild = wild || (unsigned __int128)(uint64_t)std::max<int64_t>(c->used_hi, 0) + c->dfr_req + sum >
                     (unsigned __int128)INT64_MAX;
  if (!wild) return KSG_OK;
  c->lr_wild = true;
  if (!c->dev.wide) {
    if (int rc = srv_stop(c)) return rc;
    set_wide(c);
  }
  return KSG_OK;
}

int srv_flush_patches(ksg_ctx* c) {
  if (int rc = srv_alloc(c)) return rc;
  size_t at = 0;
  while (at < c->patches.size()) {
    const uint32_t n = (uint32_t)std::min<size_t>(c->patches.size() - at, KSG_SRV_PATCHES);
    memcpy(c->srv_box->patch, c->patches.data() + at, (size_t)n * sizeof(KsgPatch));
    uint32_t hdr[KSG_SRV_HDR_DW] = {KSG_SRV_PATCH};
    hdr[KSG_SRVH_NPATCH] = n;
    uint32_t r[4];
    if (int rc = srv_call(c, hdr, r)) return rc;
    at += n;
  }
  c->patches.clear();
  return KSG_OK;
}

bool srv_put_pod(ksg_ctx* c, const ksg_pod* pod, const uint32_t* ids, size_t n_ids, const ksg_pod_ext* ext,
                 uint32_t* hdr, bool ctl = false) {
  const uint32_t pod_dw = (uint32_t)(sizeof(ksg_pod) / 4), ext_dw = (uint32_t)(sizeof(ksg_pod_ext) / 4);
  const uint32_t ids_at = pod_dw;
  const uint32_t ext_at = (ids_at + (uint32_t)n_ids + 1) & ~1u;
  const uint64_t paydw = ext ? (uint64_t)ext_at + ext_dw : (uint64_t)ids_at + n_ids;
  if (paydw > KSG_SRV_PAY_DW) return false;
  uint32_t* req = ctl ? c->srv_box->creq : c->srv_box->req;
  uint32_t* xa = ctl ? c->srv_box->cext : c->srv_box->ext;
  auto put = [&](uint32_t i, uint32_t v) {
    if (i < KSG_SRV_INLINE_DW) {
      const uint32_t j = KSG_SRV_HDR_DW + i;
      req[4 * (j / KSG_SRV_CHUNK_DW) + j % KSG_SRV_CHUNK_DW] = v;
    } else {
      xa[i - KSG_SRV_INLINE_DW] = v;
    }
  };
  const uint32_t* pw = reinterpret_cast<const uint32_t*>(pod);
  for (uint32_t i = 0; i < pod_dw; ++i) put(i, pw[i]);
  for (uint32_t i = 0; i < n_ids; ++i) put(ids_at + i, ids[i]);
  if (ext) {
    const uint32_t* ew = reinterpret_cast<const uint32_t*>(ext);
    for (uint32_t i = 0; i < ext_dw; ++i) put(ext_at + i, ew[i]);
  }
  hdr[KSG_SRVH_PAYDW] = (uint32_t)paydw;
  hdr[KSG_SRVH_IDS_AT] = ids_at;
  hdr[KSG_SRVH_EXT_AT] = ext_at;
  if (ext) hdr[KSG_SRVH_FLAGS] |= KSG_SRVF_EXT;
  return true;
}

}

extern "C" {

int ksg_shard_range(uint32_t n_nodes, int rank, int world, uint32_t* lo, uint32_t* hi) {
  if (world < 1 || rank < 0 || rank >= world || !lo || !hi) return KSG_ERR_ARG;
  uint32_t a, b;
  ksg_shard_words((n_nodes + 63) / 64, (uint32_t)rank, (uint32_t)world, &a, &b);
  *lo = std::min(a * 64, n_nodes);
  *hi = std::min(b * 64, n_nodes);
  return KSG_OK;
}

int ksg_merge_records(const void* records, uint32_t rec_bytes, uint32_t world, uint32_t n_nodes,
                      int empty_priorities, uint64_t* rng_state, uint64_t tie_index, int32_t* out_node,
                      int64_t* max_score, uint64_t* tie_count) {
  if (!records || world < 1 || rec_bytes < sizeof(KsgRecordHdr) || !out_node) return KSG_ERR_ARG;
  const uint8_t* rec = static_cast<const uint8_t*>(records);
  const KsgMerged m = ksg_merge_summary(rec, rec_bytes, world, empty_priorities);
  if (max_score) *max_score = m.max_score;
  if (tie_count) *tie_count = m.tie_count;
  *out_node = -1;
  if (m.error) return KSG_ERR_NOPEER;
  if (m.tie_count == 0) return KSG_NOFIT;
  const uint64_t ix = rng_state ? (ksg_splitmix_next(rng_state) >> 1) % m.tie_count : tie_index % m.tie_count;
  uint64_t lix = 0, kg = 0;
  const int32_t g = ksg_merge_owner(rec, rec_bytes, world, m.max_score, ix, &lix, &kg);
  if (g < 0) return KSG_ERR_ARG;
  uint32_t a, b;
  ksg_shard_words((n_nodes + 63) / 64, (uint32_t)g, world, &a, &b);
  const uint32_t nwords = (rec_bytes - (uint32_t)sizeof(KsgRecordHdr)) / 8;
  const uint64_t* words = reinterpret_cast<const uint64_t*>(rec + (size_t)g * rec_bytes + sizeof(KsgRecordHdr));
  uint64_t target = kg - 1 - lix;
  for (uint32_t w = 0; w < std::min(nwords, b - a); ++w) {
    uint64_t x = words[w];
    const uint32_t cnt = (uint32_t)__builtin_popcountll(x);
    if (target >= cnt) {
      target -= cnt;
      continue;
    }
    for (; target; --target) x &= x - 1;
    *out_node = (int32_t)((a + w) * 64 + (uint32_t)__builtin_ctzll(x));
    return *out_node < (int32_t)n_nodes ? KSG_OK : KSG_ERR_ARG;
  }
  return KSG_ERR_ARG;
}

int ksg_nccl_unique_id(void* out128) {
  ncclUniqueId id;
  if (ncclGetUniqueId(&id) != ncclSuccess) return KSG_ERR_RCCL;
  static_assert(sizeof(ncclUniqueId) == 128, "ncclUniqueId size");
  memcpy(out128, &id, sizeof id);
  return KSG_OK;
}

static int create_impl(const ksg_config* cfg, int device, int rank, int world, const void* nccl_id,
                       ksg_ctx** out) {
  if (!cfg || !out || world < 1 || rank < 0 || rank >= world) return KSG_ERR_ARG;
  if (cfg->n_anti > KSG_MAX_ANTI || cfg->n_label_pref > KSG_MAX_LABEL_PREF ||
      cfg->n_presence > KSG_MAX_PRESENCE || cfg->n_aff_labels > KSG_MAX_AFF ||
      cfg->n_aff_groups > KSG_MAX_AFF_GROUPS)
    return KSG_ERR_ARG;
  for (uint32_t g = 0; g < cfg->n_aff_groups; ++g)
    if (cfg->aff_group_mask[g] >> cfg->n_aff_labels) return KSG_ERR_ARG;
  for (uint32_t q = 0; q < cfg->n_presence; ++q)
    if (cfg->presence_n_keys[q] > KSG_MAX_PRESENCE_KEYS) return KSG_ERR_ARG;
  ksg_ctx* c = new ksg_ctx();
  c->cfg = *cfg;
  if (c->cfg.max_conflict_keys == 0) c->cfg.max_conflict_keys = 1024;
  if (c->cfg.max_domains == 0) c->cfg.max_domains = 4096;
  c->device = device;
  c->rank = rank;
  c->world = world;
  auto bail = [&](int rc) {
    if (rc != KSG_OK) {
      fprintf(stderr, "ksg_create: %s\n", c->err.c_str());
      delete c;
    }
    return rc;
  };
  hipError_t e = hipSetDevice(device);
  if (e != hipSuccess) return bail(fail(c, KSG_ERR_HIP, "hipSetDevice(%d): %s", device, hipGetErrorString(e)));
  if ((e = hipStreamCreateWithFlags(&c->st, hipStreamNonBlocking)) != hipSuccess ||
      (e = hipEventCreateWithFlags(&c->ev0, kTimingEvent)) != hipSuccess ||
      (e = hipEventCreateWithFlags(&c->ev1, kTimingEvent)) != hipSuccess ||
      (e = hipEventCreateWithFlags(&c->ev_wait, hipEventDisableTiming)) != hipSuccess)
    return bail(fail(c, KSG_ERR_HIP, "stream/event: %s", hipGetErrorString(e)));
  c->spin_wait = !(getenv("KSG_SPIN_WAIT") && atoi(getenv("KSG_SPIN_WAIT")) == 0);
  c->srv_enabled = !(getenv("KSG_SERVE") && atoi(getenv("KSG_SERVE")) == 0);
  c->srv_stamps = getenv("KSG_SERVE_STAMPS") && atoi(getenv("KSG_SERVE_STAMPS")) != 0;
  c->srv_debug = getenv("KSG_SERVE_DEBUG") && atoi(getenv("KSG_SERVE_DEBUG")) != 0;
  c->srv_trace = getenv("KSG_SERVE_TRACE") && atoi(getenv("KSG_SERVE_TRACE")) != 0;
  if (const char* go = getenv("KSG_SERVE_GRID_OPTS")) c->srv_grid_opts = (int64_t)strtoul(go, nullptr, 0);
  if (const char* iu = getenv("KSG_SERVE_IDLE_US")) c->srv_idle_us = (uint64_t)std::max(atoll(iu), 1LL);
  c->srv_grid_on = !(getenv("KSG_SERVE_GRID") && atoi(getenv("KSG_SERVE_GRID")) == 0);
  if (const char* gm = getenv("KSG_SERVE_GRID_MIN")) c->srv_grid_min = (uint32_t)std::max(atoi(gm), 0);
  if (const char* g4 = getenv("KSG_SERVE_GRID_NPT4_MIN")) c->srv_npt4_min = (uint32_t)std::max(atoi(g4), 0);
  c->srv_grid_ext = !(getenv("KSG_SERVE_GRID_EXT") && atoi(getenv("KSG_SERVE_GRID_EXT")) == 0);
  if (const char* rm = getenv("KSG_ROUND_MARGIN")) c->round_margin = std::min(std::max(atof(rm), 0.5), 4.0);
  c->xchg = world > 1 || nccl_id != nullptr;
  if (c->xchg) {
    if (world > KSG_MAX_WORLD) return bail(fail(c, KSG_ERR_ARG, "world %d > %d", world, KSG_MAX_WORLD));
    if (nccl_id) {
      ncclUniqueId id;
      memcpy(&id, nccl_id, sizeof id);
      ncclResult_t r = ncclCommInitRank(&c->comm, world, id, rank);
      if (r != ncclSuccess) return bail(fail(c, KSG_ERR_RCCL, "ncclCommInitRank: %s", ncclGetErrorString(r)));
    }
  }
  int rc;
  if (const char* wenv = getenv("KSG_WINDOW")) c->window = (uint32_t)atoi(wenv);
  if (const char* kev = getenv("KSG_KERNEL_EVENTS")) c->ev_stride = (uint32_t)std::max(atoi(kev), 0);
  if ((rc = dalloc(c, &c->d_rng, 1, nullptr)) || (rc = dalloc(c, &c->d_summary, 4, nullptr)) ||
      (rc = dalloc(c, &c->d_run, 1, nullptr)))
    return bail(rc);
  if ((e = hipHostMalloc((void**)&c->h_run, sizeof(KsgWinRun), hipHostMallocDefault)) != hipSuccess)
    return bail(fail(c, KSG_ERR_HIP, "hipHostMalloc: %s", hipGetErrorString(e)));
  c->win_fused = !(getenv("KSG_FUSED") && atoi(getenv("KSG_FUSED")) == 0);
  {
    int cus = 0;
    if (hipDeviceGetAttribute(&cus, hipDeviceAttributeMultiprocessorCount, device) != hipSuccess || cus < 16) cus = 0;
    c->fused_grid = (uint32_t)cus;
    if (const char* fg = getenv("KSG_FUSED_GRID")) c->fused_grid = (uint32_t)std::min(std::max(atoi(fg), 9), 4096);
    if (c->fused_grid == 0) c->win_fused = false;
    if (const char* fw = getenv("KSG_FUSED_MAX_WORDS")) c->fused_max_words = (uint32_t)std::max(atoi(fw), 0);
  }
  if ((e = hipMalloc((void**)&c->d_fctl, kFctlBytes)) != hipSuccess ||
      (e = hipHostMalloc((void**)&c->h_fctl, kFctlBytes, hipHostMallocDefault)) != hipSuccess)
    return bail(fail(c, KSG_ERR_HIP, "fused window control: %s", hipGetErrorString(e)));
  memset(c->h_fctl, 0, kFctlBytes);
  *out = c;
  return KSG_OK;
}

int ksg_create(const ksg_config* cfg, int device, ksg_ctx** out) {
  return create_impl(cfg, device, 0, 1, nullptr, out);
}

int ksg_create_sharded(const ksg_config* cfg, int device, int rank, int world, const void* nccl_id,
                       ksg_ctx** out) {
  return create_impl(cfg, device, rank, world, nccl_id, out);
}

int ksg_destroy(ksg_ctx* c) {
  if (!c) return KSG_OK;
  if (c->dev.dbgbuf) {
    int32_t h[32];
    (void)hipMemcpy(h, c->dev.dbgbuf, sizeof h, hipMemcpyDeviceToHost);
    fprintf(stderr, "ksg stamps (x64 cycles, committer wave): ring-wait %d head %d recheck-last-slot %d "
            "wait-checkers %d select %d commit %d | drop-path pods %d unpredicted commits %d\n",
            h[0], h[1], h[2], h[3], h[4], h[5], h[7], h[8]);
    fprintf(stderr, "ksg ring-wait split: first 4 pods of each window %d, later pods %d\n", h[10], h[11]);
    fprintf(stderr, "ksg producers (sum over waves): slot-wait %d loads %d draw-wait %d stage %d\n", h[12], h[13],
            h[14], h[15]);
    fprintf(stderr, "ksg stamps raw:");
    for (int q = 0; q < 32; ++q) fprintf(stderr, " %d", h[q]);
    fprintf(stderr, "\n");
  }
  {
    KSG_LOCK(c);
    (void)hipSetDevice(c->device);
    (void)srv_stop(c);
  }
  if (c->srv_stamped && srv_grid(c)) {
    const double n = (double)c->srv_stamped;
    fprintf(stderr, "ksg grid serve stamps (10-ns ticks per begin, %llu begins, scan workgroup 0): request seen -> "
            "masks + loads done %.1f, -> eval + part stored %.1f\n",
            (unsigned long long)c->srv_stamped, c->srv_stage[0] / n, c->srv_stage[1] / n);
  } else if (c->srv_stamped) {
    const double n = (double)c->srv_stamped;
    fprintf(stderr, "ksg serve stamps (s_memtime cycles per begin, %llu begins): to-LDS %.0f check %.0f resolve %.0f "
            "scan %.0f reduce %.0f fail-codes %.0f\n", (unsigned long long)c->srv_stamped, c->srv_stage[0] / n,
            c->srv_stage[1] / n, c->srv_stage[2] / n, c->srv_stage[3] / n, c->srv_stage[4] / n, c->srv_stage[5] / n);
  }
  (void)hipSetDevice(c->device);
  if (c->st) (void)hipStreamSynchronize(c->st);
  free_cluster(c);
  void* scratch[] = {c->d_pods, c->d_ids, c->d_fail, c->d_score, c->d_rec_send, c->d_rec_recv, c->d_dpart,
                     c->d_dglobal, c->d_out, c->d_rng, c->d_summary, c->d_patch, c->d_shard_wlo,
                     c->d_winsum, c->d_xsend, c->d_xrecv, c->d_run, c->d_dcnt, c->d_admit, c->d_one,
                     c->d_t0img, c->d_draws, c->d_etmax, c->d_epsoft, c->d_ethist, c->d_xcodes, c->d_xhist};
  for (void* p : scratch)
    if (p) (void)hipFree(p);
  if (c->comm) ncclCommDestroy(c->comm);
  if (c->h_xsend) (void)hipHostFree(c->h_xsend);
  if (c->h_run) (void)hipHostFree(c->h_run);
  if (c->h_fctl) (void)hipHostFree(c->h_fctl);
  if (c->d_fctl) (void)hipFree(c->d_fctl);
  if (c->h_up) (void)hipHostFree(c->h_up);
  if (c->h_dn) (void)hipHostFree(c->h_dn);
  if (c->h_map) (void)hipHostFree(c->h_map);
  if (c->srv_box) (void)hipHostFree(c->srv_box);
  if (c->srv_grid) (void)hipFree(c->srv_grid);
  if (c->srv_fail) (void)hipHostFree(c->srv_fail);
  if (c->h_xrecv) (void)hipHostFree(c->h_xrecv);
  if (c->ev0) (void)hipEventDestroy(c->ev0);
  if (c->ev1) (void)hipEventDestroy(c->ev1);
  if (c->ev_wait) (void)hipEventDestroy(c->ev_wait);
  if (c->ev_x0) (void)hipEventDestroy(c->ev_x0);
  if (c->ev_x1) (void)hipEventDestroy(c->ev_x1);
  for (auto& e : c->wev)
    if (e) (void)hipEventDestroy(e);
  if (c->st) (void)hipStreamDestroy(c->st);
  delete c;
  return KSG_OK;
}

const char* ksg_last_error(ksg_ctx* c) { return c ? c->err.c_str() : "null context"; }

int ksg_set_cluster(ksg_ctx* c, const ksg_node* nodes, uint32_t n_nodes, const uint32_t* node_pairs,
                    uint32_t n_node_pairs, const uint32_t* pair_keys, uint32_t n_pairs, uint32_t n_services) {
  if (!c) return KSG_ERR_ARG;
  KSG_LOCK(c);
  if (int rs_ = srv_stop(c)) return rs_;
  HIPCHK(c, hipSetDevice(c->device));
  HIPCHK(c, hipStreamSynchronize(c->st));
  if (n_nodes && !nodes) return fail(c, KSG_ERR_ARG, "nodes == NULL");
  if (n_pairs == 0) n_pairs = 1;
  for (uint32_t i = 0; i < n_nodes; ++i) {
    if ((size_t)nodes[i].label_off + nodes[i].n_labels > n_node_pairs)
      return fail(c, KSG_ERR_ARG, "node %u label range out of bounds", i);
    for (uint32_t k = 0; k < nodes[i].n_labels; ++k)
      if (node_pairs[nodes[i].label_off + k] >= n_pairs || node_pairs[nodes[i].label_off + k] == 0)
        return fail(c, KSG_ERR_ARG, "node %u has invalid pair id", i);
  }
  free_cluster(c);
  drop_deferred(c);
  c->diverged = false;
  c->ppw_est = 0.0;
  c->N = n_nodes;
  c->nw = (n_nodes + 63) / 64;
  c->n_pairs = n_pairs;
  c->S = n_services;
  c->shard_wlo_h.resize(c->world);
  c->nwords_max = 0;
  uint32_t max_shard_nodes = 0;
  for (int g = 0; g < c->world; ++g) {
    uint32_t a, b;
    ksg_shard_words(c->nw, (uint32_t)g, (uint32_t)c->world, &a, &b);
    c->shard_wlo_h[g] = a;
    c->nwords_max = std::max(c->nwords_max, b - a);
    max_shard_nodes = std::max(max_shard_nodes, std::min(b * 64, n_nodes) - std::min(a * 64, n_nodes));
    if (g == c->rank) {
      c->wlo = a;
      c->nwords = b - a;
      c->lo = std::min(a * 64, n_nodes);
      c->hi = std::min(b * 64, n_nodes);
    }
  }
  if (max_shard_nodes > kMaxNodesPerShard)
    return fail(c, KSG_ERR_CAPACITY, "shard of %u nodes exceeds %u (use more GPUs)", max_shard_nodes,
                kMaxNodesPerShard);
  c->R = pick_R(std::max<uint32_t>(max_shard_nodes, 1));

  std::vector<int32_t> dom_of_pair((size_t)std::max<uint32_t>(c->cfg.n_anti, 1) * n_pairs, -1);
  c->D = 0;
  KsgDev& d = c->dev;
  d = KsgDev{};
  for (uint32_t a = 0; a < c->cfg.n_anti; ++a) {
    d.anti_dom_off[a] = c->D;
    uint32_t nd = 0;
    for (uint32_t p = 1; p < n_pairs; ++p)
      if ((pair_keys[p] & ~KSG_PAIR_INVALID) == c->cfg.anti_key[a]) dom_of_pair[(size_t)a * n_pairs + p] = (int32_t)nd++;
    c->D += nd;
  }
  if (c->D > c->cfg.max_domains)
    return fail(c, KSG_ERR_CAPACITY, "%u anti-affinity domains > max_domains %u", c->D, c->cfg.max_domains);
  c->lds = (size_t)c->D * sizeof(int32_t);

  auto* owner = &c->cluster_allocs;
  int rc;
  int64_t *cap_c, *cap_m;
  double *inv_c, *inv_m;
  uint64_t *sfit, *keymap, *pairmap;
  int64_t* sscore;
  int32_t *anti_dom, *aff_pair;
  int64_t* gscore = nullptr;
  const size_t NN = std::max<uint32_t>(n_nodes, 1);
  if ((rc = dalloc(c, &cap_c, NN, owner)) || (rc = dalloc(c, &cap_m, NN, owner)) ||
      (rc = dalloc(c, &inv_c, NN, owner)) || (rc = dalloc(c, &inv_m, NN, owner)) ||
      (rc = dalloc(c, &d.used_cpu, NN, owner)) || (rc = dalloc(c, &d.used_mem, NN, owner)) ||
      (rc = dalloc(c, &sfit, std::max<uint32_t>(c->nw, 1), owner)) ||
      (rc = dalloc(c, &sscore, NN, owner)) ||
      (rc = dalloc(c, &keymap, (size_t)c->cfg.max_conflict_keys * std::max<uint32_t>(c->nw, 1), owner)) ||
      (rc = dalloc(c, &pairmap, (size_t)n_pairs * std::max<uint32_t>(c->nw, 1), owner)) ||
      (rc = dalloc(c, &d.svc_cnt, (size_t)std::max<uint32_t>(n_services, 1) * NN, owner)) ||
      (rc = dalloc(c, &d.svc_bits, (size_t)std::max<uint32_t>(n_services, 1) * std::max<uint32_t>(c->nw, 1), owner)) ||
      (rc = dalloc(c, &d.svc_max, std::max<uint32_t>(n_services, 1), owner)) ||
      (rc = dalloc(c, &d.svc_total, std::max<uint32_t>(n_services, 1), owner)) ||
      (rc = dalloc(c, &d.svc_peer, std::max<uint32_t>(n_services, 1), owner)) ||
      (rc = dalloc(c, &anti_dom, (size_t)std::max<uint32_t>(c->cfg.n_anti, 1) * NN, owner)) ||
      (rc = dalloc(c, &aff_pair, (size_t)std::max<uint32_t>(c->cfg.n_aff_labels, 1) * NN, owner)) ||
      (c->R > KSG_R_LDS / 2 && (rc = dalloc(c, &gscore, (size_t)c->R * KSG_NT, owner))))
    return rc;
  if (n_services) HIPCHK(c, hipMemsetAsync(d.svc_peer, 0xff, n_services * sizeof(int32_t), c->st));

  std::vector<int64_t> hc(NN, 0), hm(NN, 0);
  c->max_cap = 0;
  c->min_cap = 0;
  for (uint32_t i = 0; i < n_nodes; ++i) {
    hc[i] = nodes[i].cap_milli_cpu;
    hm[i] = nodes[i].cap_memory;
    c->max_cap = std::max<int64_t>(c->max_cap, std::max<int64_t>(std::llabs(hc[i]), std::llabs(hm[i])));
    c->min_cap = std::min<int64_t>(c->min_cap, std::min<int64_t>(hc[i], hm[i]));
  }
  HIPCHK(c, hipMemcpyAsync(cap_c, hc.data(), NN * 8, hipMemcpyHostToDevice, c->st));
  HIPCHK(c, hipMemcpyAsync(cap_m, hm.data(), NN * 8, hipMemcpyHostToDevice, c->st));
  std::vector<double> ic(NN, 0.0), im(NN, 0.0);
  for (uint32_t i = 0; i < n_nodes; ++i) {
    ic[i] = hc[i] > 0 ? 10.0 / (double)hc[i] : 0.0;
    im[i] = hm[i] > 0 ? 10.0 / (double)hm[i] : 0.0;
  }
  HIPCHK(c, hipMemcpyAsync(inv_c, ic.data(), NN * 8, hipMemcpyHostToDevice, c->st));
  HIPCHK(c, hipMemcpyAsync(inv_m, im.data(), NN * 8, hipMemcpyHostToDevice, c->st));
  ksg_node* dn = nullptr;
  uint32_t *dnp = nullptr, *dpk = nullptr;
  int32_t* ddom = nullptr;
  std::vector<void*> tmp;
  if ((rc = dalloc(c, &dn, NN, owner)) || (rc = dalloc(c, &dnp, std::max<uint32_t>(n_node_pairs, 1), owner)) ||
      (rc = dalloc(c, &dpk, n_pairs, owner)) || (rc = dalloc(c, &ddom, dom_of_pair.size(), &tmp)))
    return rc;
  c->d_lbl_nodes = dn;
  c->d_lbl_pairs = dnp;
  c->d_lbl_keys = dpk;
  if (n_nodes) HIPCHK(c, hipMemcpyAsync(dn, nodes, n_nodes * sizeof(ksg_node), hipMemcpyHostToDevice, c->st));
  if (n_node_pairs)
    HIPCHK(c, hipMemcpyAsync(dnp, node_pairs, n_node_pairs * 4, hipMemcpyHostToDevice, c->st));
  std::vector<uint32_t> pk(n_pairs, 0xffffffffu);
  if (pair_keys)
    for (uint32_t p = 1; p < n_pairs; ++p) pk[p] = pair_keys[p];
  HIPCHK(c, hipMemcpyAsync(dpk, pk.data(), n_pairs * 4, hipMemcpyHostToDevice, c->st));
  HIPCHK(c, hipMemcpyAsync(ddom, dom_of_pair.data(), dom_of_pair.size() * 4, hipMemcpyHostToDevice, c->st));
  KsgStaticCfg sc{};
  sc.n_presence = c->cfg.n_presence;
  memcpy(sc.presence_n_keys, c->cfg.presence_n_keys, sizeof sc.presence_n_keys);
  memcpy(sc.presence_keys, c->cfg.presence_keys, sizeof sc.presence_keys);
  memcpy(sc.presence_flag, c->cfg.presence_flag, sizeof sc.presence_flag);
  sc.n_pref = c->cfg.n_label_pref;
  memcpy(sc.pref_key, c->cfg.pref_key, sizeof sc.pref_key);
  memcpy(sc.pref_presence, c->cfg.pref_presence, sizeof sc.pref_presence);
  memcpy(sc.w_pref, c->cfg.w_pref, sizeof sc.w_pref);
  sc.w_equal = c->cfg.w_equal;
  sc.n_anti = c->cfg.n_anti;
  memcpy(sc.anti_key, c->cfg.anti_key, sizeof sc.anti_key);
  sc.n_aff = c->cfg.n_aff_labels;
  memcpy(sc.aff_key, c->cfg.aff_key, sizeof sc.aff_key);
  HIPCHK(c, ksg_launch_static(sc, n_nodes, dn, dnp, dpk, ddom, n_pairs, c->nw, sfit, sscore, anti_dom, aff_pair,
                              (unsigned long long*)pairmap, c->st));
  c->h_aff_pair.clear();
  if ((c->cfg.predicates & KSG_PRED_SERVICEAFFINITY) && c->cfg.n_aff_labels > 0 && c->world == 1) {
    c->h_aff_pair.resize((size_t)c->cfg.n_aff_labels * NN);
    HIPCHK(c, hipMemcpyAsync(c->h_aff_pair.data(), aff_pair, c->h_aff_pair.size() * sizeof(int32_t),
                             hipMemcpyDeviceToHost, c->st));
    HIPCHK(c, hipStreamSynchronize(c->st));
  }
  c->d_zmap = nullptr;
  uint32_t rr_dz = 0;
  if (c->cfg.n_anti == 1 && c->cfg.w_anti[0] != 0 && c->D > 0 && c->D + 1 <= KSG_RR_MAXZ && c->world == 1 &&
      n_services <= KSG_RR_MAXSVC && !(getenv("KSG_DEBUG") && (atoi(getenv("KSG_DEBUG")) & 2048))) {
    rr_dz = c->D + 1;
    if ((rc = dalloc(c, &c->d_zmap, (size_t)rr_dz * std::max<uint32_t>(c->nw, 1), owner))) return rc;
    HIPCHK(c, ksg_launch_zonemap(n_nodes, anti_dom, c->D, c->nw, c->d_zmap, c->st));
  }
  HIPCHK(c, hipStreamSynchronize(c->st));
  for (void* p : tmp) (void)hipFree(p);

  d.n_nodes = n_nodes;
  d.nw = c->nw;
  d.lo = c->lo;
// ... 312 lines not shown
  c->upd_q.push_back({false, 0, ksg_pod{}, {}, uid});
  c->q_added.erase(uid);
  c->q_removed.insert(uid);
  return KSG_OK;
}

int ksg_schedule_begin(ksg_ctx* c, const ksg_pod* pod, const uint32_t* ids, int64_t* max_score,
                       uint32_t* tie_count, uint8_t* fail_codes) {
  if (!c || !pod) return KSG_ERR_ARG;
  KSG_LOCK(c);
  if (int rc0 = flush_deferred(c)) return rc0;
  if (int rs = cluster_ok(c)) return rs;
  HIPCHK(c, hipSetDevice(c->device));
  if (c->pending) {
    c->pending = false;
    c->pend_srv = false;
    if (int rq = apply_queued(c)) return rq;
  }
  if (c->N == 0) return KSG_NONODES;
  if (c->ext_on && !c->cur_ext) c->ext_scalar.erase(pod->uid);
  const size_t ext = call_ids_extent(c, pod);
  int rc = check_pod(c, pod, ids, ext);
  if (rc) return rc;
  if ((rc = note_requests(c, pod, 1))) return rc;
  if (srv_eligible(c)) {
    uint32_t hdr[KSG_SRV_HDR_DW] = {KSG_SRV_BEGIN};
    if ((rc = srv_alloc(c))) return rc;
    static const ksg_pod_ext zero_ext{};
    const ksg_pod_ext* xr = c->ext_on ? (c->cur_ext ? c->cur_ext : &zero_ext) : nullptr;
    ksg_pod rp;
    const ksg_pod* sp = pod;
    if (!c->h_aff_pair.empty() && pod->service >= 0 && (uint32_t)pod->service < c->S) {
      const int32_t peer = c->svc_peer[pod->service];
      bool given = true;
      for (uint32_t j = 0; j < c->cfg.n_aff_labels && j < KSG_MAX_AFF; ++j) given = given && pod->aff_pair[j] != -1;
      if (!given && peer >= 0 && (uint32_t)peer < c->N) {
        rp = *pod;
        for (uint32_t j = 0; j < c->cfg.n_aff_labels && j < KSG_MAX_AFF; ++j)
          if (rp.aff_pair[j] == -1) rp.aff_pair[j] = c->h_aff_pair[(size_t)j * c->N + (uint32_t)peer];
        sp = &rp;
      }
    }
    if (srv_put_pod(c, sp, ids, ext, xr, hdr)) {
      if ((rc = flush_patches(c)) || (!c->srv_running && (rc = srv_flush_patches(c)))) return rc;
      if (fail_codes) hdr[KSG_SRVH_FLAGS] |= KSG_SRVF_WANT_FAIL;
      uint32_t r[4];
      if ((rc = srv_begin(c, hdr, r))) return rc;
      if ((rc = srv_settle(c))) return rc;
      if (r[1] == KSG_SRV_BADREQ) return fail(c, KSG_ERR_STATE, "drop-in server rejected begin request");
      if (r[1] == ~0u) return fail(c, KSG_ERR_NOPEER, "service affinity peer is not on a known node");
      if (fail_codes) memcpy(fail_codes, c->srv_fail, (size_t)(c->hi - c->lo));
      const int64_t m = (int64_t)((uint64_t)r[2] | ((uint64_t)r[3] << 32));
      if (max_score) *max_score = r[1] > 0 ? m : 0;
      if (tie_count) *tie_count = r[1];
      if (r[1] == 0) return KSG_NOFIT;
      c->pending = true;
      c->pending_k = r[1];
      c->pend = *pod;
      c->pend_ids.assign(ids, ids + ext);
      c->pend_srv = true;
      memcpy(c->srv_bhdr, hdr, sizeof hdr);
      c->srv_pext_on = xr != nullptr;
      if (xr) c->srv_pext = *xr;
      return KSG_OK;
    }
  }
  if ((rc = srv_stop(c))) return rc;
  if ((rc = flush_patches(c))) return rc;
  if ((rc = ensure_map(c)) || (rc = upload_one(c, pod, ids, ext))) return rc;
  if ((rc = scan_exchange(c, c->one_pod, c->one_ids, KSG_MODE_BEGIN, fail_codes ? c->d_fail : nullptr, nullptr,
                          c->ext_on ? c->d_one_ext : nullptr)))
    return rc;
  HIPCHK(c, ksg_launch_decide(c->dev, c->one_pod, c->one_ids, rec_buf(c), c->rec_bytes, c->world,
                              c->d_shard_wlo, 0, 0, c->d_rng, nullptr, 0, reinterpret_cast<int64_t*>(c->d_map),
                              c->st));
  int64_t summ[3];
  const size_t nf = fail_codes ? (size_t)(c->hi - c->lo) : 0;
  if (nf) {
    if ((rc = grow_host(c, &c->h_dn, &c->h_dn_cap, nf))) return rc;
    HIPCHK(c, hipMemcpyAsync(c->h_dn, c->d_fail, nf, hipMemcpyDeviceToHost, c->st));
  }
  HIPCHK(c, hipStreamSynchronize(c->st));
  memcpy(summ, c->h_map, sizeof summ);
  if (nf) memcpy(fail_codes, c->h_dn, nf);
  if (summ[2]) return fail(c, KSG_ERR_NOPEER, "service affinity peer is not on a known node");
  if (max_score) *max_score = summ[1] > 0 ? summ[0] : 0;
  if (tie_count) *tie_count = (uint32_t)summ[1];
  if (summ[1] == 0) return KSG_NOFIT;
  c->pending = true;
  c->pending_k = (uint64_t)summ[1];
  c->pend = *pod;
  c->pend_ids.assign(ids, ids + ext);
  return KSG_OK;
}

static int commit_on_device(ksg_ctx* c, uint32_t tie_index, int32_t* node) {
  HIPCHK(c, hipSetDevice(c->device));
  if (c->pend_srv) {
    c->pend_srv = false;
    const int64_t off = srv_pick(c->srv_tw, c->pending_k - 1 - tie_index);
    if (off < 0 || off >= (int64_t)(c->hi - c->lo)) return fail(c, KSG_ERR_STATE, "commit selected no node");
    *node = (int32_t)(c->lo + (uint32_t)off);
    uint32_t hdr[KSG_SRV_HDR_DW] = {KSG_SRV_COMMIT};
    if (int rc = srv_settle(c)) return rc;
    if (!srv_put_pod(c, &c->pend, c->pend_ids.data(), c->pend_ids.size(), c->srv_pext_on ? &c->srv_pext : nullptr,
                     hdr, true))
      return fail(c, KSG_ERR_STATE, "pending pod does not fit the request block");
    hdr[KSG_SRVH_ARG] = (uint32_t)*node;
    if (c->srv_trace) fprintf(stderr, "srv commit node %d\n", *node);
    uint32_t seq = 0;
    if (int rc = srv_post(c, hdr, &seq)) return rc;
    c->srv_unacked = seq;
    return KSG_OK;
  }
  int rc = ensure_map(c);
  if (rc) return rc;
  if ((rc = srv_stop(c))) return rc;
  HIPCHK(c, ksg_launch_decide(c->dev, c->one_pod, c->one_ids, rec_buf(c), c->rec_bytes, c->world,
                              c->d_shard_wlo, 2, tie_index, c->d_rng, reinterpret_cast<int32_t*>(c->d_map + 32), 0,
                              c->d_summary, c->st, c->ext_on ? c->d_one_ext : nullptr));
  HIPCHK(c, hipStreamSynchronize(c->st));
  memcpy(node, c->h_map + 32, 4);
  if (*node < 0) return fail(c, KSG_ERR_STATE, "commit selected no node (%d)", *node);
  return KSG_OK;
}

int ksg_schedule_commit(ksg_ctx* c, uint32_t tie_index, int32_t* out_node) {
  if (!c) return KSG_ERR_ARG;
  KSG_LOCK(c);
  if (!c->pending) return fail(c, KSG_ERR_STATE, "no schedule_begin pending");
  if (tie_index >= c->pending_k) return fail(c, KSG_ERR_ARG, "tie_index %u >= tie_count %llu", tie_index,
                                             (unsigned long long)c->pending_k);
  int32_t node = -1;
  int rc = commit_on_device(c, tie_index, &node);
  c->pending = false;
  if (rc == KSG_OK) rc = mirror_add(c, (uint32_t)node, &c->pend, c->pend_ids.data(), false);
  c->pend.uid = ~0ULL;
  const int rq = apply_queued(c);
  if (rc) return rc;
  if (rq) return rq;
  if (out_node) *out_node = node;
  return KSG_OK;
}

int ksg_schedule_batch(ksg_ctx* c, const ksg_pod* pods, uint32_t n, const uint32_t* ids, uint32_t n_ids,
                       uint64_t* rng_state, int32_t* out_nodes) {
  if (!c || (n && (!pods || !out_nodes)) || !rng_state) return KSG_ERR_ARG;
  KSG_LOCK(c);
  if (c->pending) return fail(c, KSG_ERR_STATE, "schedule_begin pending");
  if (int rs_ = srv_stop(c)) return rs_;
  if (int rs = cluster_ok(c)) return rs;
  HIPCHK(c, hipSetDevice(c->device));
  c->last_ms = 0.0;
  if (n == 0) return KSG_OK;
  if (c->N == 0) {
    for (uint32_t i = 0; i < n; ++i) out_nodes[i] = KSG_OUT_NONODES;
    return KSG_OK;
  }
  for (double& v : c->last_hus) v = 0.0;
  auto t_last = std::chrono::steady_clock::now();
  auto hphase = [&](int k) {
    const auto t = std::chrono::steady_clock::now();
    c->last_hus[k] += std::chrono::duration<double, std::micro>(t - t_last).count();
    t_last = t;
  };
  for (uint32_t i = 0; i < n; ++i) {
    int rc = check_pod(c, pods + i, ids, n_ids);
    if (rc) return rc;
    if (c->pods.count(pods[i].uid) || c->dfr_uids.count(pods[i].uid))
      return fail(c, KSG_ERR_ARG, "pod %u: duplicate uid", i);
  }
  hphase(0);
  int rc;
  if ((rc = note_requests(c, pods, n))) return rc;
  if (c->dfr_neg && (rc = flush_deferred(c))) return rc;
  if ((rc = flush_patches(c))) return rc;
  if ((rc = upload_pods(c, pods, n, ids, n_ids))) return rc;
  if ((rc = ensure_out(c, n))) return rc;
  const size_t dn_rng = ((size_t)n * 4 + 7) & ~(size_t)7;
  if ((rc = grow_host(c, &c->h_dn, &c->h_dn_cap, dn_rng + 8))) return rc;
  bool tail_queued = false;
  auto enqueue_tail = [&]() -> int {
    HIPCHK(c, hipEventRecord(c->ev1, c->st));
    HIPCHK(c, hipMemcpyAsync(c->h_dn, c->d_out, (size_t)n * 4, hipMemcpyDeviceToHost, c->st));
    HIPCHK(c, hipMemcpyAsync(c->h_dn + dn_rng, c->d_rng, 8, hipMemcpyDeviceToHost, c->st));
    return KSG_OK;
  };
  bool stashed = false, dup_any = false;
  std::vector<ksg_pod> st_pods;
  std::vector<uint32_t> st_ids;
  std::unordered_set<uint64_t> st_uids;
  auto overlap_work = [&]() -> int {
    if (stashed) return KSG_OK;
    int rc2 = flush_deferred(c);
    if (rc2) return rc2;
    hphase(4);
    st_pods.assign(pods, pods + n);
    st_ids.assign(ids, ids + n_ids);
    st_uids.swap(c->dfr_uids);
    st_uids.reserve(2 * (size_t)n);
    for (uint32_t i = 0; i < n; ++i) dup_any |= !st_uids.insert(pods[i].uid).second;
    stashed = true;
    hphase(7);
    return KSG_OK;
  };
  struct DivergeGuard {
    ksg_ctx* c;
    bool armed = false;
    ~DivergeGuard() {
      if (armed) {
        drop_deferred(c);
        c->diverged = true;
      }
    }
  } guard{c};
  if (c->dev.dbg & 16384) c->dbg_fail_next = true;
  guard.armed = true;
  HIPCHK(c, hipMemcpyAsync(c->d_rng, rng_state, 8, hipMemcpyHostToDevice, c->st));
  HIPCHK(c, hipEventRecord(c->ev0, c->st));
  c->last_stats[0] = c->last_stats[1] = c->last_stats[2] = c->last_stats[3] = 0;
  c->last_kms[0] = c->last_kms[1] = c->last_kms[2] = c->last_t0ms = 0;
  c->last_wsum = 0;
  hphase(1);
  const ksg_pod_ext* dext = nullptr;
  if (c->ext_on) {
    if ((rc = grow(c, (void**)&c->d_pext, &c->pext_cap, n, sizeof(ksg_pod_ext)))) return rc;
    if (c->cur_ext) {
      HIPCHK(c, hipMemcpyAsync(c->d_pext, c->cur_ext, (size_t)n * sizeof(ksg_pod_ext), hipMemcpyHostToDevice, c->st));
    } else {
      HIPCHK(c, hipMemsetAsync(c->d_pext, 0, (size_t)n * sizeof(ksg_pod_ext), c->st));
    }
    dext = c->d_pext;
  }
  if (use_window(c, pods, n)) {
    const KsgDev full = full_geometry(c);
    uint32_t W = std::min(c->window, ksg_win_max_window(full));
    if (!c->xchg && c->ppw_est > 0.0) {
      const uint32_t want = ((uint32_t)std::ceil(3.0 * c->ppw_est) + 7u) & ~7u;
      W = std::min(W, std::max<uint32_t>(want, 16u));
    }
    KsgWinXchg x{};
    x.exts = dext;
    x.ostride = std::max<uint32_t>(c->nwords_max, 1);
    x.wcap = W;
    x.world = (uint32_t)c->world;
    for (int g = 0; g < c->world; ++g) {
      uint32_t a, b;
      ksg_shard_words(c->nw, (uint32_t)g, (uint32_t)c->world, &a, &b);
      x.wlo[g] = a;
      x.nw[g] = b - a;
    }
    const bool anti = anti_on(c);
    const bool rr = anti && c->dev.rr_dz != 0 && c->d_zmap;
    const size_t fit_off = ((size_t)W * x.ostride * 12 + 7) & ~(size_t)7;
    x.fit_off = anti ? (uint32_t)fit_off : 0u;
    x.b_off = rr ? (uint32_t)(fit_off + (size_t)W * x.ostride * 8) : 0u;
    const bool esc = c->ext_on && (c->ext.w_taint_toleration != 0 || c->ext.w_balanced != 0);
    const bool etm = esc && c->ext.w_taint_toleration != 0;
    x.esc = esc ? 1u : 0u;
    x.efit_off = esc ? (uint32_t)fit_off : 0u;
    const bool d1 = !anti && !dext && c->win_d1 && c->nw <= 4 * 64;
    x.d1 = d1 ? 1u : 0u;
    x.d1_off = d1 ? (uint32_t)fit_off : 0u;
    x.blk = ((rr                  ? fit_off + (size_t)W * x.ostride * 16
              : anti || esc || d1 ? fit_off + (size_t)W * x.ostride * 8
                                  : (size_t)W * x.ostride * 12) +
             255) & ~(size_t)255;
    if (esc) {
      if ((rc = grow(c, (void**)&c->d_etmax, &c->etmax_cap, W, sizeof(int32_t))) ||
          (rc = grow(c, (void**)&c->d_ethist, &c->ethist_cap, (size_t)W * KSG_TBINS, sizeof(int32_t))) ||
          (rc = grow(c, (void**)&c->d_epsoft, &c->epsoft_cap, W, sizeof(uint64_t))))
        return rc;
      HIPCHK(c, hipMemsetAsync(c->d_etmax, 0, (size_t)W * sizeof(int32_t), c->st));
      HIPCHK(c, hipMemsetAsync(c->d_ethist, 0, (size_t)W * KSG_TBINS * sizeof(int32_t), c->st));
      x.tmax = c->d_etmax;
      x.thist = c->d_ethist;
      x.psoft = c->d_epsoft;
    }
    const size_t dcnt_n = (size_t)W * std::max<uint32_t>(c->D, 1);
    if (anti) {
      if ((rc = grow(c, (void**)&c->d_dcnt, &c->dcnt_cap, dcnt_n, sizeof(int32_t)))) return rc;
      HIPCHK(c, hipMemsetAsync(c->d_dcnt, 0, dcnt_n * sizeof(int32_t), c->st));
      x.dcnt = c->d_dcnt;
      x.dcnt_n = (uint32_t)dcnt_n;
    }
    if (rr) {
      const size_t dmb_n = (size_t)W * c->dev.rr_dz;
      if ((rc = grow(c, (void**)&c->d_dmb, &c->dmb_cap, 2 * dmb_n, sizeof(int32_t)))) return rc;
      HIPCHK(c, hipMemsetD32Async((hipDeviceptr_t)c->d_dmb, (int)0x80000000, dmb_n, c->st));
      HIPCHK(c, hipMemsetAsync(c->d_dmb + dmb_n, 0, dmb_n * sizeof(int32_t), c->st));
      x.rr = 1;
      x.dz = c->dev.rr_dz;
      x.dmb = c->d_dmb;
      x.zmap = c->d_zmap;
    }
    if ((rc = grow(c, (void**)&c->d_winsum, &c->win_cap, W, sizeof(KsgWinSum)))) return rc;
    if ((rc = grow(c, (void**)&c->d_xsend, &c->xsend_cap, x.blk, 1))) return rc;
    if (c->xchg && (rc = grow(c, (void**)&c->d_xrecv, &c->xrecv_cap, x.blk * c->world, 1))) return rc;
    x.buf = c->xchg ? c->d_xrecv : c->d_xsend;
    const bool plain = !anti;
    if (plain) {
      x.img_stride = ksg_win_t0_stride(full);
      if ((rc = grow(c, (void**)&c->d_t0img, &c->t0img_cap, (size_t)W * x.img_stride, 1))) return rc;
      x.img = c->d_t0img;
    }
    const uint32_t fgroups = plain && !c->xchg && !dext && c->win_fused && full.nwords <= c->fused_max_words &&
                                     ksg_win_fused_ok(full)
                                 ? ksg_win_fused_groups(full, W) : 0u;
    const bool fused = fgroups > 0 && fgroups <= kFctlGroups;
    KsgWinRun* const fruns = reinterpret_cast<KsgWinRun*>(c->d_fctl);
    uint32_t* const fcnt = reinterpret_cast<uint32_t*>(c->d_fctl + kFctlRuns);
    uint64_t* wbits = reinterpret_cast<uint64_t*>(c->d_xsend);
    int32_t* wmax = reinterpret_cast<int32_t*>(c->d_xsend + (size_t)W * x.ostride * 8);
    double ppw_est = c->xchg ? 0.0 : c->ppw_est;
    auto round_k = [&](uint32_t left) -> uint32_t {
      const double ppw = ppw_est > 0.0 ? std::min<double>(std::max(ppw_est, 1.0), (double)W) : 0.8 * W;
      const double k = std::ceil((double)left / ppw * c->round_margin) + 1.0;
      return (uint32_t)std::min(k, 8192.0);
    };
    uint32_t pos = 0, K = round_k(n);
    c->last_kms[0] = c->last_kms[1] = c->last_kms[2] = c->last_t0ms = 0;
    c->last_wsum = 0;
    hphase(2);
    while (pos < n) {
      if (c->wev.size() < 3 * (size_t)K + 1) {
        const size_t old = c->wev.size();
        c->wev.resize(3 * (size_t)K + 1, nullptr);
        for (size_t i = old; i < c->wev.size(); ++i) HIPCHK(c, hipEventCreateWithFlags(&c->wev[i], kTimingEvent));
      }
      const uint32_t es = std::min(c->ev_stride, K);
      const uint32_t ev_off = es ? c->ev_phase++ % es : 0u;
      *c->h_run = KsgWinRun{pos, n, 0, 0, {0, 0, 0, 0}};
      if (fused) {
        *reinterpret_cast<KsgWinRun*>(c->h_fctl) = *c->h_run;
        HIPCHK(c, hipMemcpyAsync(c->d_fctl, c->h_fctl, kFctlRuns + (size_t)2 * fgroups * 8 * sizeof(uint32_t),
                                 hipMemcpyHostToDevice, c->st));
      } else {
        HIPCHK(c, hipMemcpyAsync(c->d_run, c->h_run, sizeof(KsgWinRun), hipMemcpyHostToDevice, c->st));
      }
      HIPCHK(c, hipEventRecord(c->wev[0], c->st));
      for (uint32_t k = 0; k < K; ++k) {
        const bool evk = es && (k + ev_off) % es == 0;
        if (evk && k > 0) HIPCHK(c, hipEventRecord(c->wev[3 * k], c->st));
        if (fused) {
          KsgFused f{c->d_pods, c->d_ids, fruns + ((k + 1) & 1), fcnt, k & 1u, fgroups};
          HIPCHK(c, ksg_launch_win_fused(full, W, fruns + (k & 1), c->d_winsum, x, c->d_rng, c->d_out, f,
                                         c->fused_grid, c->st));
          if (evk) HIPCHK(c, hipEventRecord(c->wev[3 * k + 3], c->st));
          continue;
        }
        if (anti) {
          HIPCHK(c, ksg_launch_win_eval(c->dev, 1, c->d_pods, c->d_ids, c->d_run, W, c->d_winsum, wbits, wmax,
                                        x.ostride, c->d_dcnt, nullptr, x.dmb, nullptr, x.dz, c->st, dext));
          if (c->xchg && (rc = allreduce_sum_i32(c, c->d_dcnt, c->d_dcnt, (uint32_t)dcnt_n))) return rc;
        }
        if (etm) {
          HIPCHK(c, ksg_launch_win_eval(c->dev, 3, c->d_pods, c->d_ids, c->d_run, W, c->d_winsum, wbits, wmax,
                                        x.ostride, nullptr, nullptr, nullptr, nullptr, 0, c->st, dext, x.tmax,
                                        x.psoft, x.thist));
          if (c->xchg && ((rc = allreduce_max_i32(c, x.tmax, x.tmax, W)) ||
                          (rc = allreduce_sum_i32(c, x.thist, x.thist, W * KSG_TBINS))))
            return rc;
        }
        HIPCHK(c, ksg_launch_win_eval(c->dev, anti ? 2 : 0, c->d_pods, c->d_ids, c->d_run, W, c->d_winsum, wbits,
                                      wmax, x.ostride, c->d_dcnt,
                                      (anti || esc || d1) ? reinterpret_cast<uint64_t*>(c->d_xsend + fit_off) : nullptr,
                                      x.dmb, rr ? reinterpret_cast<uint64_t*>(c->d_xsend + x.b_off) : nullptr, x.dz,
                                      c->st, dext, x.tmax, x.psoft));
        if (evk) HIPCHK(c, hipEventRecord(c->wev[3 * k + 1], c->st));
        if (c->xchg && (rc = allgather(c, c->d_xsend, c->d_xrecv, x.blk))) return rc;
        if (plain) HIPCHK(c, ksg_launch_win_t0(full, W, c->d_run, x, c->st));
        if (evk) HIPCHK(c, hipEventRecord(c->wev[3 * k + 2], c->st));
        HIPCHK(c, ksg_launch_win_resolve(full, W, c->d_run, c->d_winsum, x, c->d_rng, c->d_out, c->st));
        if (evk) HIPCHK(c, hipEventRecord(c->wev[3 * k + 3], c->st));
      }
      HIPCHK(c, hipMemcpyAsync(c->h_run, fused ? fruns + (K & 1) : c->d_run, sizeof(KsgWinRun), hipMemcpyDeviceToHost,
                               c->st));
      if ((rc = enqueue_tail())) return rc;
      hphase(3);
      if ((rc = overlap_work())) return rc;
      if ((rc = wait_device(c))) return rc;
      hphase(5);
      const KsgWinRun r = *c->h_run;
      if (r.windows > 0 && r.pos > pos) {
        const double ppw = (double)(r.pos - pos) / (double)r.windows;
        ppw_est = ppw_est > 0.0 ? 0.5 * ppw_est + 0.5 * ppw : ppw;
        if (!c->xchg) c->ppw_est = ppw_est;
      }
      double ea = 0.0, eb = 0.0, et = 0.0;
      uint32_t nt = 0;
      for (uint32_t k = es ? (es - ev_off) % es : 0u; es && k < K; k += es) {
        float a = 0.f, t0 = 0.f, b = 0.f;
        if (fused) {
          HIPCHK(c, hipEventElapsedTime(&b, c->wev[3 * k], c->wev[3 * k + 3]));
        } else {
          HIPCHK(c, hipEventElapsedTime(&a, c->wev[3 * k], c->wev[3 * k + 1]));
          HIPCHK(c, hipEventElapsedTime(&t0, c->wev[3 * k + 1], c->wev[3 * k + 2]));
          HIPCHK(c, hipEventElapsedTime(&b, c->wev[3 * k + 2], c->wev[3 * k + 3]));
        }
        ea += a;
        et += t0;
        eb += b;
        ++nt;
      }
      if (nt) {
        c->last_kms[0] += ea * K / nt;
        c->last_kms[1] += eb * K / nt;
        c->last_t0ms += et * K / nt;
      }
      c->last_kms[2] += K;
      c->last_wsum += (double)W * K;
      c->last_stats[0] += r.windows;
      for (int q = 1; q <= 3; ++q) c->last_stats[q] += r.stops[q];
      if (c->dbg_fail_next) {
        c->dbg_fail_next = false;
        return fail(c, KSG_ERR_STATE, "window resolver: injected failure (KSG_DEBUG & 16384) at pod %u", r.pos);
      }
      if (r.halt == KSG_HALT_HANG) return fail(c, KSG_ERR_STATE, "window resolver: ring wait timed out at pod %u", r.pos);
      if (r.halt == KSG_HALT_BAD)
        return fail(c, KSG_ERR_STATE,
                    "window resolver: selection outside T0 at pod %u (inconsistent prefixes or drop positions: a bug, "
                    "or stale verdicts under the KSG_DEBUG timing switches)", r.pos);
      if (r.halt == KSG_HALT_BADCOUNT || r.pos < pos || r.pos > n)
        return fail(c, KSG_ERR_STATE, "window resolver: bad progress (halt %u, pos %u -> %u)", r.halt, pos, r.pos);
      pos = r.pos;
      tail_queued = pos >= n && r.halt != KSG_HALT_OVERSIZE;
      if (r.halt == KSG_HALT_OVERSIZE) {
        if (!c->xchg) {
          HIPCHK(c, ksg_launch_batch(c->R, anti, c->dev, c->d_pods + pos, c->d_ids, 1, c->d_rng,
                                     c->d_out + pos, c->st, dext ? dext + pos : nullptr));
        } else {
          if ((rc = scan_exchange(c, c->d_pods + pos, c->d_ids, KSG_MODE_BEGIN, nullptr, nullptr,
                                  dext ? dext + pos : nullptr)))
            return rc;
          HIPCHK(c, ksg_launch_decide(c->dev, c->d_pods + pos, c->d_ids, rec_buf(c), c->rec_bytes, c->world,
                                      c->d_shard_wlo, 1, 0, c->d_rng, c->d_out, pos, c->d_summary, c->st,
                                      dext ? dext + pos : nullptr));
        }
        pos += 1;
        ++c->last_stats[3];
      }
      K = round_k(n - std::min(pos, n));
      hphase(2);
    }
  } else if (!c->xchg) {
    HIPCHK(c, ksg_launch_batch(c->R, anti_on(c), c->dev, c->d_pods, c->d_ids, n, c->d_rng, c->d_out, c->st, dext));
  } else {
    for (uint32_t i = 0; i < n; ++i) {
      if ((rc = scan_exchange(c, c->d_pods + i, c->d_ids, KSG_MODE_BEGIN, nullptr, nullptr, dext ? dext + i : nullptr)))
        return rc;
      HIPCHK(c, ksg_launch_decide(c->dev, c->d_pods + i, c->d_ids, rec_buf(c), c->rec_bytes, c->world,
                                  c->d_shard_wlo, 1, 0, c->d_rng, c->d_out, i, c->d_summary, c->st,
                                  dext ? dext + i : nullptr));
    }
  }
  if (!tail_queued) {
    if ((rc = enqueue_tail())) return rc;
    hphase(3);
    if ((rc = overlap_work())) return rc;
    if ((rc = wait_device(c))) return rc;
    hphase(6);
  }
  memcpy(out_nodes, c->h_dn, (size_t)n * 4);
  memcpy(rng_state, c->h_dn + dn_rng, 8);
  float ms = 0.f;
  HIPCHK(c, hipEventElapsedTime(&ms, c->ev0, c->ev1));
  c->last_ms = ms;
  if (!stashed) {
    return fail(c, KSG_ERR_STATE, "internal: batch replay inputs missing");
  }
  guard.armed = false;
  if (c->ext_on && !c->cur_ext)
    for (uint32_t i = 0; i < n; ++i) c->ext_scalar.erase(pods[i].uid);
  c->dfr_pods.swap(st_pods);
  c->dfr_ids.swap(st_ids);
  c->dfr_uids.swap(st_uids);
  c->dfr_out.assign(out_nodes, out_nodes + n);
  for (uint32_t i = 0; i < n; ++i)
    if (out_nodes[i] < 0 && !dup_any) c->dfr_uids.erase(pods[i].uid);
  if (dup_any) {
    for (uint32_t i = 0; i < n; ++i) c->dfr_uids.erase(pods[i].uid);
    for (uint32_t i = 0; i < n; ++i)
      if (out_nodes[i] >= 0 && !c->dfr_uids.insert(pods[i].uid).second)
        return fail(c, KSG_ERR_ARG, "pod %u: duplicate uid within the batch", i);
  }
  for (uint32_t i = 0; i < n; ++i) {
    if (out_nodes[i] < 0) continue;
    c->dfr_req += (uint64_t)std::max<int64_t>(std::max(pods[i].milli_cpu, pods[i].memory), 0);
    if (pods[i].milli_cpu < 0 || pods[i].memory < 0) c->dfr_neg = true;
    else c->dfr_sum = std::min<int64_t>(c->dfr_sum + std::min<int64_t>(std::min<int64_t>(pods[i].milli_cpu, KSG_WIN_LR_BOUND) +
                                                                        std::min<int64_t>(pods[i].memory, KSG_WIN_LR_BOUND),
                                                                        KSG_WIN_LR_BOUND), KSG_WIN_LR_BOUND + 1);
  }
  hphase(7);
  double* t = c->totals;
  t[0] += 1;
  t[1] += c->last_ms;
  for (int q = 0; q < 3; ++q) t[2 + q] += c->last_kms[q];
  t[17] += c->last_wsum;
  t[18] += c->last_t0ms;
  for (int q = 0; q < 4; ++q) t[5 + q] += c->last_stats[q];
  for (int q = 0; q < 8; ++q) t[9 + q] += c->last_hus[q];
  return KSG_OK;
}

int ksg_evaluate(ksg_ctx* c, const ksg_pod* pod, const uint32_t* ids, uint8_t* fail_out, int64_t* score_out) {
  if (!c || !pod) return KSG_ERR_ARG;
  KSG_LOCK(c);
  if (c->pending) return fail(c, KSG_ERR_STATE, "schedule_begin pending");
  if (int rs_ = srv_stop(c)) return rs_;
  if (int rc0 = flush_deferred(c)) return rc0;
  if (int rs = cluster_ok(c)) return rs;
  HIPCHK(c, hipSetDevice(c->device));
  if (c->N == 0) return KSG_NONODES;
  const size_t ext = call_ids_extent(c, pod);
  int rc = check_pod(c, pod, ids, ext);
  if (rc) return rc;
  if ((rc = note_requests(c, pod, 1))) return rc;
  if ((rc = flush_patches(c))) return rc;
  if ((rc = upload_one(c, pod, ids, ext))) return rc;
  if ((rc = scan_exchange(c, c->one_pod, c->one_ids, KSG_MODE_BEGIN, nullptr, nullptr, c->ext_on ? c->d_one_ext : nullptr)))
    return rc;
  HIPCHK(c, ksg_launch_decide(c->dev, c->one_pod, c->one_ids, rec_buf(c), c->rec_bytes, c->world,
                              c->d_shard_wlo, 0, 0, c->d_rng, nullptr, 0, c->d_summary, c->st));
  if ((rc = scan_exchange(c, c->one_pod, c->one_ids, KSG_MODE_EVAL, c->d_fail, c->d_score, c->ext_on ? c->d_one_ext : nullptr)))
    return rc;
  int64_t summ[3];
  HIPCHK(c, hipMemcpyAsync(summ, c->d_summary, sizeof summ, hipMemcpyDeviceToHost, c->st));
  const size_t ns = c->hi - c->lo;
  if (fail_out && ns) HIPCHK(c, hipMemcpyAsync(fail_out, c->d_fail, ns, hipMemcpyDeviceToHost, c->st));
  if (score_out && ns) HIPCHK(c, hipMemcpyAsync(score_out, c->d_score, ns * 8, hipMemcpyDeviceToHost, c->st));
  HIPCHK(c, hipStreamSynchronize(c->st));
  if (summ[2]) return fail(c, KSG_ERR_NOPEER, "service affinity peer is not on a known node");
  return KSG_OK;
}

int ksg_set_allgather(ksg_ctx* c, ksg_allgather_fn fn, void* user) {
  if (!c) return KSG_ERR_ARG;
  KSG_LOCK(c);
  if (c->comm) return fail(c, KSG_ERR_STATE, "context already exchanges over RCCL");
  c->xfn = fn;
  c->xuser = user;
  return KSG_OK;
}

int ksg_set_window(ksg_ctx* c, uint32_t window) {
  if (!c) return KSG_ERR_ARG;
  KSG_LOCK(c);
  c->window = window;
  c->ppw_est = 0.0;
  return KSG_OK;
}

int ksg_last_batch_stats(ksg_ctx* c, uint32_t* stats4) {
  if (!c || !stats4) return KSG_ERR_ARG;
  KSG_LOCK(c);
  for (int i = 0; i < 4; ++i) stats4[i] = c->last_stats[i];
  return KSG_OK;
}

int ksg_last_batch_kernel_ms(ksg_ctx* c, double* out3) {
  if (!c || !out3) return KSG_ERR_ARG;
  KSG_LOCK(c);
  for (int i = 0; i < 3; ++i) out3[i] = c->last_kms[i];
  return KSG_OK;
}

int ksg_batch_totals(ksg_ctx* c, double* out24) {
  if (!c || !out24) return KSG_ERR_ARG;
  KSG_LOCK(c);
  for (int k = 0; k < 24; ++k) out24[k] = c->totals[k];
  return KSG_OK;
}

int ksg_last_batch_host_us(ksg_ctx* c, double* out8) {
  if (!c || !out8) return KSG_ERR_ARG;
  KSG_LOCK(c);
  for (int k = 0; k < 8; ++k) out8[k] = c->last_hus[k];
  return KSG_OK;
}

int ksg_serve_stats(ksg_ctx* c, uint64_t* out4) {
  if (!c || !out4) return KSG_ERR_ARG;
  KSG_LOCK(c);
  out4[0] = c->srv_launches;
  out4[1] = c->srv_seq;
  out4[2] = c->srv_running ? 1 : 0;
  out4[3] = srv_eligible(c) ? (srv_grid(c) ? 2 : 1) : 0;
  return KSG_OK;
}

int ksg_debug_counters(ksg_ctx* c, int32_t* out, uint32_t n_words) {
  if (!c || (!out && n_words)) return KSG_ERR_ARG;
  KSG_LOCK(c);
  if (int rs_ = srv_stop(c)) return rs_;
  if (!c->dev.dbgbuf) return fail(c, KSG_ERR_STATE, "debug counters need KSG_DEBUG=8 at ksg_create");
  (void)hipSetDevice(c->device);
  HIPCHK(c, hipStreamSynchronize(c->st));
  int32_t words[KSG_DEBUG_COUNTER_WORDS];
  HIPCHK(c, hipMemcpy(words, c->dev.dbgbuf, sizeof(words), hipMemcpyDeviceToHost));
  for (uint32_t k = 0; k < n_words; ++k) out[k] = k < KSG_DEBUG_COUNTER_WORDS ? words[k] : 0;
  return KSG_OK;
}

int ksg_last_batch_ms(ksg_ctx* c, double* ms) {
  if (!c || !ms) return KSG_ERR_ARG;
  KSG_LOCK(c);
  *ms = c->last_ms;
  return KSG_OK;
}

int ksg_shard(ksg_ctx* c, uint32_t* lo, uint32_t* hi) {
  if (!c) return KSG_ERR_ARG;
  KSG_LOCK(c);
  if (lo) *lo = c->lo;
  if (hi) *hi = c->hi;
  return KSG_OK;
}

int ksg_read_requested(ksg_ctx* c, int64_t* milli_cpu, int64_t* memory) {
  if (!c || !c->have_cluster) return KSG_ERR_ARG;
  KSG_LOCK(c);
  if (int rs_ = srv_stop(c)) return rs_;
  HIPCHK(c, hipSetDevice(c->device));
  int rc = flush_patches(c);
  if (rc) return rc;
  if (c->N) {
    if (milli_cpu) HIPCHK(c, hipMemcpyAsync(milli_cpu, c->dev.used_cpu, c->N * 8, hipMemcpyDeviceToHost, c->st));
    if (memory) HIPCHK(c, hipMemcpyAsync(memory, c->dev.used_mem, c->N * 8, hipMemcpyDeviceToHost, c->st));
  }
  HIPCHK(c, hipStreamSynchronize(c->st));
  return KSG_OK;
}

static int admit_impl(ksg_ctx* c, int mode, const ksg_admission_set* sets, uint32_t n_sets, const ksg_pod* pods,
                      uint32_t n_pods, const uint32_t* ids, uint32_t n_ids, const uint32_t* pairs, uint32_t n_pairs,
                      uint8_t* out) {
  if (!c || (n_sets && !sets) || (n_pods && (!pods || !out))) return KSG_ERR_ARG;
  KSG_LOCK(c);
  if (int rs_ = srv_stop(c)) return rs_;
  for (uint32_t s = 0; s < n_sets; ++s) {
    if ((uint64_t)sets[s].pod_off + sets[s].n_pods > n_pods)
      return fail(c, KSG_ERR_ARG, "admission set %u: pods out of range", s);
    if ((mode & KSG_ADMIT_MODE_SELECTOR) && (uint64_t)sets[s].label_off + sets[s].n_labels > n_pairs)
      return fail(c, KSG_ERR_ARG, "admission set %u: labels out of range", s);
  }
  if (mode & KSG_ADMIT_MODE_SELECTOR) {
    if ((n_ids && !ids) || (n_pairs && !pairs)) return fail(c, KSG_ERR_ARG, "admission: ids / pairs == NULL");
    for (uint32_t i = 0; i < n_pods; ++i)
      if ((uint64_t)pods[i].sel_off + pods[i].n_sel > n_ids)
        return fail(c, KSG_ERR_ARG, "pod %u: nodeSelector ids out of range", i);
  }
  std::vector<uint8_t> in_set(n_pods, 0);
  for (uint32_t s = 0; s < n_sets; ++s)
    for (uint32_t k = 0; k < sets[s].n_pods; ++k)
      if (in_set[sets[s].pod_off + k]++)
        return fail(c, KSG_ERR_ARG, "admission sets %u and an earlier one share pod %u", s, sets[s].pod_off + k);
  for (uint32_t i = 0; i < n_pods; ++i) out[i] = KSG_ADMIT_OK;
  if (n_sets == 0 || n_pods == 0) return KSG_OK;
  HIPCHK(c, hipSetDevice(c->device));
  const bool sel = (mode & KSG_ADMIT_MODE_SELECTOR) != 0;
  const size_t b_sets = (size_t)n_sets * sizeof(ksg_admission_set), b_pods = (size_t)n_pods * sizeof(ksg_pod);
  const size_t b_ids = sel ? (size_t)n_ids * 4 : 0, b_pairs = sel ? (size_t)n_pairs * 4 : 0;
  const size_t o_pods = (b_sets + 15) & ~(size_t)15, o_ids = o_pods + ((b_pods + 15) & ~(size_t)15);
  const size_t o_pairs = o_ids + ((b_ids + 15) & ~(size_t)15), o_out = o_pairs + ((b_pairs + 15) & ~(size_t)15);
  const size_t total = o_out + n_pods;
  int rc;
  if ((rc = grow(c, (void**)&c->d_admit, &c->admit_cap, total, 1))) return rc;
  if ((rc = grow_host(c, &c->h_up, &c->h_up_cap, o_out))) return rc;
  memcpy(c->h_up, sets, b_sets);
  memcpy(c->h_up + o_pods, pods, b_pods);
  if (b_ids) memcpy(c->h_up + o_ids, ids, b_ids);
  if (b_pairs) memcpy(c->h_up + o_pairs, pairs, b_pairs);
  HIPCHK(c, hipMemcpyAsync(c->d_admit, c->h_up, o_out, hipMemcpyHostToDevice, c->st));
  HIPCHK(c, ksg_launch_admit(reinterpret_cast<const ksg_admission_set*>(c->d_admit), n_sets,
                             reinterpret_cast<const ksg_pod*>(c->d_admit + o_pods),
                             reinterpret_cast<const uint32_t*>(c->d_admit + o_ids),
                             reinterpret_cast<const uint32_t*>(c->d_admit + o_pairs), mode, c->d_admit + o_out, c->st));
  if ((rc = grow_host(c, &c->h_dn, &c->h_dn_cap, n_pods))) return rc;
  HIPCHK(c, hipMemcpyAsync(c->h_dn, c->d_admit + o_out, n_pods, hipMemcpyDeviceToHost, c->st));
  HIPCHK(c, hipStreamSynchronize(c->st));
  for (uint32_t i = 0; i < n_pods; ++i)
    if (in_set[i]) out[i] = c->h_dn[i];
  return KSG_OK;
}

int ksg_set_extensions(ksg_ctx* c, const ksg_ext_config* e) {
  if (!c || !e) return KSG_ERR_ARG;
  KSG_LOCK(c);
  if (c->have_cluster) return fail(c, KSG_ERR_STATE, "ksg_set_extensions: call before ksg_set_cluster");
  if (int rs_ = srv_stop(c)) return rs_;
  if ((e->filters & ~(KSG_EXT_TAINTS | KSG_EXT_SCALAR)) || e->n_scalar > KSG_MAX_SCALAR)
    return fail(c, KSG_ERR_ARG, "extensions: bad filters / n_scalar");
  c->ext = *e;
  c->ext_on = e->filters || e->w_taint_toleration || e->w_balanced || e->n_scalar;
  return KSG_OK;
}

int ksg_set_node_ext(ksg_ctx* c, uint32_t n_nodes, const int64_t* scalar_cap, const uint32_t* taint_off,
                     const uint32_t* taint_n, const uint32_t* taint_ids, uint32_t n_taint_ids) {
  if (!c) return KSG_ERR_ARG;
  KSG_LOCK(c);
  if (c->pending) return fail(c, KSG_ERR_STATE, "schedule_begin pending");
  if (int rs_ = srv_stop(c)) return rs_;
  if (!c->ext_on) return fail(c, KSG_ERR_STATE, "ksg_set_node_ext: extensions are off");
  if (!c->have_cluster || n_nodes != c->N) return fail(c, KSG_ERR_ARG, "ksg_set_node_ext: node count != cluster");
  if (int rc0 = flush_deferred(c)) return rc0;
  if (!c->pods.empty()) return fail(c, KSG_ERR_STATE, "ksg_set_node_ext: call before adding pods");
  HIPCHK(c, hipSetDevice(c->device));
  const size_t NN = std::max<uint32_t>(c->N, 1);
  if (c->ext.n_scalar && n_nodes) {
    if (!scalar_cap) return fail(c, KSG_ERR_ARG, "ksg_set_node_ext: scalar_cap missing");
    HIPCHK(c, hipMemcpyAsync(const_cast<int64_t*>(c->dev.scalar_cap), scalar_cap, (size_t)c->ext.n_scalar * n_nodes * 8,
                             hipMemcpyHostToDevice, c->st));
  }
  std::vector<uint64_t> tm((size_t)std::max<uint32_t>(c->ext.max_taints, 1) * std::max<uint32_t>(c->nw, 1), 0);
  if (taint_off && taint_n)
    for (uint32_t n = 0; n < n_nodes; ++n)
      for (uint32_t i = 0; i < taint_n[n]; ++i) {
        if ((size_t)taint_off[n] + i >= n_taint_ids || !taint_ids) return fail(c, KSG_ERR_ARG, "taint list out of range");
        const uint32_t t = taint_ids[taint_off[n] + i];
        if (t >= c->ext.max_taints) return fail(c, KSG_ERR_CAPACITY, "taint id %u >= max_taints", t);
        tm[(size_t)t * c->nw + (n >> 6)] |= 1ULL << (n & 63);
      }
  HIPCHK(c, hipMemcpyAsync(const_cast<uint64_t*>(c->dev.taintmap), tm.data(), tm.size() * 8, hipMemcpyHostToDevice,
                           c->st));
  if (c->dev.ntaint) {
    std::vector<uint64_t> ntm(std::max<uint32_t>(n_nodes, 1), 0);
    if (taint_off && taint_n)
      for (uint32_t n = 0; n < n_nodes; ++n)
        for (uint32_t i = 0; i < taint_n[n]; ++i) ntm[n] |= 1ULL << (taint_ids[taint_off[n] + i] & 63);
    HIPCHK(c, hipMemcpyAsync(const_cast<uint64_t*>(c->dev.ntaint), ntm.data(), ntm.size() * 8, hipMemcpyHostToDevice,
                             c->st));
  }
  HIPCHK(c, hipMemsetAsync(c->dev.scalar_used, 0, (size_t)std::max<uint32_t>(c->ext.n_scalar, 1) * NN * 8, c->st));
  HIPCHK(c, hipStreamSynchronize(c->st));
  c->sc_used.assign((size_t)c->ext.n_scalar * c->N, 0);
  return KSG_OK;
}

int ksg_read_ext_used(ksg_ctx* c, int64_t* used) {
  if (!c || !used || !c->have_cluster) return KSG_ERR_ARG;
  KSG_LOCK(c);
  if (!c->ext_on) return fail(c, KSG_ERR_STATE, "ksg_read_ext_used: extensions are off");
  if (int rs_ = srv_stop(c)) return rs_;
  HIPCHK(c, hipSetDevice(c->device));
  if (int rc = flush_patches(c)) return rc;
  const size_t nb = (size_t)c->ext.n_scalar * c->N * 8;
  if (nb) HIPCHK(c, hipMemcpyAsync(used, c->dev.scalar_used, nb, hipMemcpyDeviceToHost, c->st));
  HIPCHK(c, hipStreamSynchronize(c->st));
  return KSG_OK;
}

static int check_ext_range(ksg_ctx* c, const ksg_pod_ext* e, size_t n_ids) {
  if ((size_t)e->hard_off + e->n_hard > n_ids || (size_t)e->soft_off + e->n_soft > n_ids)
    return fail(c, KSG_ERR_ARG, "extension taint list out of range");
  return KSG_OK;
}
static int note_ext(ksg_ctx* c, const ksg_pod* p, const ksg_pod_ext* e, size_t n_ids) {
  if (int rc = check_ext_range(c, e, n_ids)) return rc;
// ... 11 lines not shown
  if (n <= 64) {
    for (uint32_t i = 1; i < n; ++i)
      for (uint32_t j = 0; j < i; ++j)
        if (v[i] == v[j]) return true;
    return false;
  }
  std::vector<uint32_t> s(v, v + n);
  std::sort(s.begin(), s.end());
  return std::adjacent_find(s.begin(), s.end()) != s.end();
}
static int check_taint_ids(ksg_ctx* c, const ksg_pod_ext* e, const uint32_t* ids) {
  for (uint32_t i = 0; i < e->n_hard; ++i)
    if (ids[e->hard_off + i] >= c->ext.max_taints) return fail(c, KSG_ERR_CAPACITY, "taint id out of range");
  for (uint32_t i = 0; i < e->n_soft; ++i)
    if (ids[e->soft_off + i] >= c->ext.max_taints) return fail(c, KSG_ERR_CAPACITY, "taint id out of range");
  if ((e->n_hard && has_repeat(ids + e->hard_off, e->n_hard)) || (e->n_soft && has_repeat(ids + e->soft_off, e->n_soft)))
    return fail(c, KSG_ERR_ARG, "a taint id repeats in the pod's hard or soft list (each list is a set)");
  return KSG_OK;
}

int ksg_add_pod_ext(ksg_ctx* c, uint32_t host_id, const ksg_pod* pod, const ksg_pod_ext* ext, const uint32_t* ids) {
  if (!c || !pod) return KSG_ERR_ARG;
  KSG_LOCK(c);
  if (ext && !c->ext_on) return fail(c, KSG_ERR_STATE, "extensions are off");
  if (c->ext_on) {
    const ksg_pod_ext z{};
    const ksg_pod_ext* e = ext ? ext : &z;
    const size_t n_ids = std::max(pod_ids_extent(pod), std::max<size_t>((size_t)e->hard_off + e->n_hard,
                                                                         (size_t)e->soft_off + e->n_soft));
    if (int rc = note_ext(c, pod, e, n_ids)) return rc;
  }
  c->cur_ext = ext;
  const int rc = ksg_add_pod(c, host_id, pod, ids);
  c->cur_ext = nullptr;
  return rc;
}

int ksg_schedule_batch_draws(ksg_ctx* c, const ksg_pod* pods, uint32_t n, const uint32_t* ids, uint32_t n_ids,
                             const uint64_t* draws, uint32_t n_draws, uint32_t* draws_used, int32_t* out_nodes) {
  if (!c || (n && (!pods || !out_nodes || !draws)) || !draws_used) return KSG_ERR_ARG;
  KSG_LOCK(c);
  if (n_draws < n) return fail(c, KSG_ERR_ARG, "%u draws for %u pods: one per pod that may find a node", n_draws, n);
  for (uint32_t k = 0; k < n; ++k)
    if (draws[k] > (uint64_t)INT64_MAX) return fail(c, KSG_ERR_ARG, "draw %u is not a rand.Int() value", k);
  *draws_used = 0;
  if (c->pending) return fail(c, KSG_ERR_STATE, "schedule_begin pending");
  if (n == 0) return ksg_schedule_batch(c, pods, 0, ids, n_ids, &c->draw_tmp, out_nodes);
  HIPCHK(c, hipSetDevice(c->device));
  if (int rs_ = srv_stop(c)) return rs_;
  if (int rc = grow(c, (void**)&c->d_draws, &c->draws_cap, n, sizeof(uint64_t))) return rc;
  HIPCHK(c, hipMemcpy(c->d_draws, draws, (size_t)n * sizeof(uint64_t), hipMemcpyHostToDevice));
  c->dev.draws = c->d_draws;
  uint64_t state = 0;
  const int rc = ksg_schedule_batch(c, pods, n, ids, n_ids, &state, out_nodes);
  c->dev.draws = nullptr;
  if (rc == KSG_OK) *draws_used = (uint32_t)state;
  return rc;
}

int ksg_batch_unwind(ksg_ctx* c, const ksg_pod* pods, const int32_t* out_nodes, uint32_t n, uint32_t k,
                     uint64_t* rng_state, uint32_t* draws_kept) {
  if (!c || !pods || !out_nodes || !draws_kept || k >= n) return KSG_ERR_ARG;
  KSG_LOCK(c);
  if (c->pending) return fail(c, KSG_ERR_STATE, "schedule_begin pending");
  if (out_nodes[k] < 0) return fail(c, KSG_ERR_ARG, "pod %u found no node: there was no Bind to reject", k);
  if (int rs = cluster_ok(c)) return rs;
  HIPCHK(c, hipSetDevice(c->device));
  if (int rc0 = flush_deferred(c)) return rc0;
  for (uint32_t i = k; i < n; ++i)
    if (out_nodes[i] >= 0 && !c->pods.count(pods[i].uid))
      return fail(c, KSG_ERR_ARG, "pod %u (uid %llu) is not a committed pod of this context", i,
                  (unsigned long long)pods[i].uid);
  uint32_t kept = 0, back = 0;
  for (uint32_t i = 0; i <= k; ++i) kept += out_nodes[i] >= 0 ? 1u : 0u;
  for (uint32_t i = n; i-- > k;) {
    if (out_nodes[i] < 0) continue;
    if (i > k) ++back;
    if (int rc = remove_pod_impl(c, pods[i].uid)) return rc;
  }
  if (rng_state) *rng_state -= (uint64_t)back * ksg_rng_step(nullptr);
  *draws_kept = kept;
  return flush_patches(c);
}

int ksg_schedule_batch_ext(ksg_ctx* c, const ksg_pod* pods, const ksg_pod_ext* ext, uint32_t n, const uint32_t* ids,
                           uint32_t n_ids, uint64_t* rng_state, int32_t* out_nodes) {
  if (!c || (n && (!pods || !out_nodes)) || !rng_state) return KSG_ERR_ARG;
  KSG_LOCK(c);
  if (ext && !c->ext_on) return fail(c, KSG_ERR_STATE, "extensions are off");
  if (c->ext_on && ext)
    for (uint32_t i = 0; i < n; ++i) {
      if (int rc = check_ext_range(c, ext + i, n_ids)) return rc;
      if (int rc = check_taint_ids(c, ext + i, ids)) return rc;
    }
  c->cur_ext = ext;
  const int rc = ksg_schedule_batch(c, pods, n, ids, n_ids, rng_state, out_nodes);
  c->cur_ext = nullptr;
  if (rc == KSG_OK && c->ext_on && ext)
    for (uint32_t i = 0; i < n; ++i) {
      if (out_nodes[i] >= 0) (void)note_ext(c, pods + i, ext + i, n_ids);
      else c->ext_scalar.erase(pods[i].uid);
    }
  return rc;
}

int ksg_schedule_begin_ext(ksg_ctx* c, const ksg_pod* pod, const ksg_pod_ext* ext, const uint32_t* ids,
                           int64_t* max_score, uint32_t* tie_count, uint8_t* fail_codes) {
  if (!c || !pod) return KSG_ERR_ARG;
  KSG_LOCK(c);
  if (ext && !c->ext_on) return fail(c, KSG_ERR_STATE, "extensions are off");
  c->cur_ext = ext;
  int rc = KSG_OK;
  if (ext) {
    const size_t n_ids = call_ids_extent(c, pod);
    if (!(rc = check_ext_range(c, ext, n_ids)) && !(rc = check_taint_ids(c, ext, ids))) rc = note_ext(c, pod, ext, n_ids);
  }
  if (!rc) rc = ksg_schedule_begin(c, pod, ids, max_score, tie_count, fail_codes);
  c->cur_ext = nullptr;
  return rc;
}

int ksg_evaluate_ext(ksg_ctx* c, const ksg_pod* pod, const ksg_pod_ext* ext, const uint32_t* ids, uint8_t* fail_out,
                     int64_t* score_out) {
  if (!c || !pod) return KSG_ERR_ARG;
  KSG_LOCK(c);
  if (ext && !c->ext_on) return fail(c, KSG_ERR_STATE, "extensions are off");
  c->cur_ext = ext;
  int rc = ext ? check_taint_ids(c, ext, ids) : KSG_OK;
  if (!rc) rc = ksg_evaluate(c, pod, ids, fail_out, score_out);
  c->cur_ext = nullptr;
  return rc;
}

int ksg_explain_batch(ksg_ctx* c, const ksg_pod* pods, const ksg_pod_ext* ext, uint32_t n, const uint32_t* ids,
                      uint32_t n_ids, uint8_t* codes, uint32_t* hist, uint8_t* err) {
  if (!c || (n && (!pods || !hist || !err))) return KSG_ERR_ARG;
  KSG_LOCK(c);
  if (c->pending) return fail(c, KSG_ERR_STATE, "schedule_begin pending");
  if (ext && !c->ext_on) return fail(c, KSG_ERR_STATE, "extensions are off");
  if (int rs_ = srv_stop(c)) return rs_;
  if (int rc0 = flush_deferred(c)) return rc0;
  if (int rs = cluster_ok(c)) return rs;
  HIPCHK(c, hipSetDevice(c->device));
  c->last_explain_ms = 0.0;
  if (n == 0) return KSG_OK;
  if (c->N == 0) return KSG_NONODES;
  if (n_ids && !ids) return fail(c, KSG_ERR_ARG, "ids missing");
  int rc;
  for (uint32_t i = 0; i < n; ++i) {
    if ((rc = check_pod(c, pods + i, ids, n_ids))) return rc;
    if (ext && ((rc = check_ext_range(c, ext + i, n_ids)) || (rc = check_taint_ids(c, ext + i, ids)))) return rc;
  }
  if ((rc = flush_patches(c))) return rc;
  if ((rc = upload_pods(c, pods, n, ids, n_ids))) return rc;
  const ksg_pod_ext* dext = nullptr;
  if (ext) {
    if ((rc = grow(c, (void**)&c->d_pext, &c->pext_cap, n, sizeof(ksg_pod_ext)))) return rc;
    HIPCHK(c, hipMemcpyAsync(c->d_pext, ext, (size_t)n * sizeof(ksg_pod_ext), hipMemcpyHostToDevice, c->st));
    dext = c->d_pext;
  }
  const size_t hb = (size_t)n * KSG_EXPLAIN_SLOTS * sizeof(uint32_t);
  if ((rc = grow(c, (void**)&c->d_xhist, &c->xhist_cap, hb + n, 1))) return rc;
  uint32_t* d_hist = reinterpret_cast<uint32_t*>(c->d_xhist);
  uint8_t* d_err = c->d_xhist + hb;
  HIPCHK(c, hipMemsetAsync(c->d_xhist, 0, hb + n, c->st));
  uint32_t per = 1u << 20;
  if (codes) {
    per = (uint32_t)std::min<size_t>(per, std::max<size_t>(kExplainStageBytes / c->N, 1));
    if (per > KSG_EXPLAIN_CHUNK) per -= per % KSG_EXPLAIN_CHUNK;
    per = std::min(per, n);
    if ((rc = grow(c, (void**)&c->d_xcodes, &c->xcodes_cap, (size_t)per * c->N, 1))) return rc;
  }
  if (!c->ev_x0) {
    HIPCHK(c, hipEventCreate(&c->ev_x0));
    HIPCHK(c, hipEventCreate(&c->ev_x1));
  }
  for (uint32_t a = 0; a < n; a += per) {
    const uint32_t m = std::min(per, n - a);
    HIPCHK(c, hipEventRecord(c->ev_x0, c->st));
    HIPCHK(c, ksg_launch_explain(c->dev, c->d_pods + a, dext ? dext + a : nullptr, c->d_ids, m,
                                 codes ? c->d_xcodes : nullptr, d_hist + (size_t)a * KSG_EXPLAIN_SLOTS, d_err + a, c->st));
    HIPCHK(c, hipEventRecord(c->ev_x1, c->st));
    if (codes)
      HIPCHK(c, hipMemcpyAsync(codes + (size_t)a * c->N, c->d_xcodes, (size_t)m * c->N, hipMemcpyDeviceToHost, c->st));
    if (a + per >= n) {
      HIPCHK(c, hipMemcpyAsync(hist, d_hist, hb, hipMemcpyDeviceToHost, c->st));
      HIPCHK(c, hipMemcpyAsync(err, d_err, n, hipMemcpyDeviceToHost, c->st));
    }
    HIPCHK(c, hipStreamSynchronize(c->st));
    float ms = 0.f;
    HIPCHK(c, hipEventElapsedTime(&ms, c->ev_x0, c->ev_x1));
    c->last_explain_ms += ms;
  }
  return KSG_OK;
}

int ksg_last_explain_ms(ksg_ctx* c, double* ms) {
  if (!c || !ms) return KSG_ERR_ARG;
  KSG_LOCK(c);
  *ms = c->last_explain_ms;
  return KSG_OK;
}

int ksg_check_pods_exceeding_capacity(ksg_ctx* c, const ksg_admission_set* sets, uint32_t n_sets,
                                      const ksg_pod* pods, uint32_t n_pods, uint8_t* fits) {
  const int rc = admit_impl(c, KSG_ADMIT_MODE_CAPACITY, sets, n_sets, pods, n_pods, nullptr, 0, nullptr, 0, fits);
  if (rc == KSG_OK)
    for (uint32_t i = 0; i < n_pods; ++i) fits[i] = fits[i] == KSG_ADMIT_OK;
  return rc;
}

int ksg_pod_matches_node_labels(ksg_ctx* c, const ksg_admission_set* sets, uint32_t n_sets, const ksg_pod* pods,
                                uint32_t n_pods, const uint32_t* ids, uint32_t n_ids, const uint32_t* pairs,
                                uint32_t n_pairs, uint8_t* matches) {
  const int rc = admit_impl(c, KSG_ADMIT_MODE_SELECTOR, sets, n_sets, pods, n_pods, ids, n_ids, pairs, n_pairs,
                            matches);
  if (rc == KSG_OK)
    for (uint32_t i = 0; i < n_pods; ++i) matches[i] = matches[i] == KSG_ADMIT_OK;
  return rc;
}

int ksg_admit_pods(ksg_ctx* c, const ksg_admission_set* sets, uint32_t n_sets, const ksg_pod* pods, uint32_t n_pods,
                   const uint32_t* ids, uint32_t n_ids, const uint32_t* pairs, uint32_t n_pairs, uint8_t* codes) {
  return admit_impl(c, KSG_ADMIT_MODE_SELECTOR | KSG_ADMIT_MODE_CAPACITY, sets, n_sets, pods, n_pods, ids, n_ids,
                    pairs, n_pairs, codes);
}

}
```

Before: 783,600 pods/s.

## Return batch results through a mapped host mailbox and fold timing lazily

The resolver kernel now writes final placements, RNG state and run record straight into coherent mapped host memory, guarded by a head/tail tag. The host spins on that tag instead of issuing a device-to-host copy and waiting for the stream. Pod, id, RNG and control uploads are merged into one arena and a single host-to-device copy. Event timing reads are deferred to a lazy fold using double-buffered event sets. This is meant to cut per-batch launch, copy and sync latency, at the cost of system-scope fences and PCIe writes from the kernel plus more complex state handling.

```diff
diff --git a/kubernetes_amd/csrc/ksg_internal.h b/kubernetes_amd/csrc/ksg_internal.h
--- a/kubernetes_amd/csrc/ksg_internal.h
+++ b/kubernetes_amd/csrc/ksg_internal.h
@@ -106,7 +106,16 @@
 #define KSG_WIN_SUM_DWORDS (sizeof(KsgWinSum) / 4)
 
 #define KSG_MAX_WORLD 16
+struct KsgRetRec;
+struct KsgRet {
+  int32_t* places;
+  KsgRetRec* rec;
+  uint32_t tag;
+  uint32_t k, K;
+  uint32_t pad;
+};
 struct KsgWinXchg {
+  KsgRet ret;
   const uint8_t* buf;
   uint64_t blk;
   uint32_t ostride;
@@ -147,6 +156,15 @@
   uint32_t windows;
   uint32_t stops[4];
 };
+struct alignas(64) KsgRetRec {
+  uint32_t tag_head;
+  uint32_t pad0;
+  uint64_t rng;
+  KsgWinRun run;
+  uint32_t pad1[3];
+  uint32_t tag_tail;
+};
+static_assert(sizeof(KsgRetRec) == 64, "KsgRetRec layout");
 
 struct KsgFused {
   const ksg_pod* batch;
diff --git a/kubernetes_amd/csrc/ksg_plain.hip b/kubernetes_amd/csrc/ksg_plain.hip
--- a/kubernetes_amd/csrc/ksg_plain.hip
+++ b/kubernetes_amd/csrc/ksg_plain.hip
@@ -1865,6 +1865,14 @@
                                          __ATOMIC_RELAXED, __HIP_MEMORY_SCOPE_AGENT);
   }
   for (uint32_t t = lane; t < resolved; t += 64) out[t] = L_cm[t].out;
+  bool publish = false;
+  if (x.ret.rec) {
+    for (uint32_t t = lane; t < resolved; t += 64) x.ret.places[pos + t] = L_cm[t].out;
+    const bool moved = reason != KSG_STOP_HANG && reason != KSG_STOP_BAD && reason != KSG_STOP_OVERSIZE &&
+                       resolved != 0 && resolved <= n_pods;
+    publish = !moved || pos + resolved >= n_batch || x.ret.k + 1 >= x.ret.K;
+    if (publish) __threadfence_system();
+  }
   if (esc && x.tmax) {
     for (uint32_t t = lane; t < wcap; t += 64) x.tmax[t] = 0;
     for (uint32_t t = lane; t < n_pods * KSG_TBINS; t += 64) x.thist[t] = 0;
@@ -1882,7 +1890,8 @@
     drain_stores();
   }
   if (lane == 0) {
-    *rng_io = rng0 + (uint64_t)n_draws * ksg_rng_step(d.draws);
+    const uint64_t rng1 = rng0 + (uint64_t)n_draws * ksg_rng_step(d.draws);
+    *rng_io = rng1;
     if constexpr (STAMP && FUSED)
       if (d.dbgbuf) __hip_atomic_store(d.dbgbuf + 55, 0, __ATOMIC_RELAXED, __HIP_MEMORY_SCOPE_AGENT);
     KsgWinRun r = *run;
@@ -1902,6 +1911,13 @@
       r.stops[3] += reason == 3 ? 1u : 0u;
     }
     *run_out = r;
+    if (publish) {
+      KsgRetRec* const q = x.ret.rec;
+      __hip_atomic_store(&q->tag_head, x.ret.tag, __ATOMIC_RELAXED, __HIP_MEMORY_SCOPE_SYSTEM);
+      q->rng = rng1;
+      q->run = r;
+      __hip_atomic_store(&q->tag_tail, x.ret.tag, __ATOMIC_RELEASE, __HIP_MEMORY_SCOPE_SYSTEM);
+    }
   }
 }
 
diff --git a/kubernetes_amd/csrc/ksg_runtime.cpp b/kubernetes_amd/csrc/ksg_runtime.cpp
--- a/kubernetes_amd/csrc/ksg_runtime.cpp
+++ b/kubernetes_amd/csrc/ksg_runtime.cpp
@@ -84,6 +84,9 @@
 constexpr uint32_t kFctlGroups = 1024;
 constexpr size_t kFctlRuns = 2 * sizeof(KsgWinRun);
 constexpr size_t kFctlBytes = kFctlRuns + (size_t)2 * kFctlGroups * 8 * sizeof(uint32_t);
+constexpr size_t kArRng = 0, kArCtl = 16;
+constexpr size_t ar_ctl_bytes(uint32_t groups) { return kFctlRuns + (size_t)2 * groups * 8 * sizeof(uint32_t); }
+constexpr size_t ar_pods(uint32_t groups) { return (kArCtl + ar_ctl_bytes(groups) + 15) & ~(size_t)15; }
 constexpr size_t kExplainStageBytes = (size_t)64 << 20;
 
 const unsigned kTimingEvent =
@@ -107,7 +110,23 @@
   void* xuser = nullptr;
   uint8_t *h_xsend = nullptr, *h_xrecv = nullptr;
   size_t h_xsend_cap = 0, h_xrecv_cap = 0;
-  hipEvent_t ev0 = nullptr, ev1 = nullptr;
+  struct EvSet {
+    hipEvent_t ev0 = nullptr, ev1 = nullptr;
+    std::vector<hipEvent_t> wev;
+  } evs[2];
+  int evset = 0;
+  struct Lazy {
+    bool on = false;
+    bool into_last = false;
+    int set = 0;
+    uint32_t K = 0, es = 0, ev_off = 0;
+    bool fused = false;
+  } lazy;
+  bool mailbox = true;
+  uint8_t* h_ret = nullptr;
+  uint8_t* d_ret = nullptr;
+  size_t ret_cap = 0;
+  uint32_t ret_tag = 0;
   hipEvent_t ev_wait = nullptr;
   bool spin_wait = true;
   double last_ms = 0.0;
@@ -124,10 +143,10 @@
   std::vector<void*> cluster_allocs;
   uint32_t* d_shard_wlo = nullptr;
 
+  uint8_t* d_arena = nullptr;
+  size_t arena_cap = 0;
   ksg_pod* d_pods = nullptr;
-  size_t pods_cap = 0;
   uint32_t* d_ids = nullptr;
-  size_t ids_cap = 0;
   uint8_t* d_fail = nullptr;
   int64_t* d_score = nullptr;
   uint8_t* d_rec_send = nullptr;
@@ -190,9 +209,7 @@
   uint64_t* d_epsoft = nullptr;
   size_t etmax_cap = 0, epsoft_cap = 0;
   KsgWinRun* d_run = nullptr;
-  KsgWinRun* h_run = nullptr;
   uint32_t last_stats[4] = {0, 0, 0, 0};
-  std::vector<hipEvent_t> wev;
   double last_kms[3] = {0, 0, 0};
   double last_t0ms = 0;
   double last_wsum = 0;
@@ -203,7 +220,6 @@
   uint32_t fused_grid = 0;
   uint32_t fused_max_words = 1024;
   uint8_t* d_fctl = nullptr;
-  uint8_t* h_fctl = nullptr;
   double last_hus[8] = {0, 0, 0, 0, 0, 0, 0, 0};
   double totals[24] = {};
   int64_t max_cap = 0, min_cap = 0;
@@ -501,17 +517,34 @@
 
 int grow_host(ksg_ctx* c, uint8_t** p, size_t* cap, size_t need);
 
-int upload_pods(ksg_ctx* c, const ksg_pod* pods, uint32_t n, const uint32_t* ids, size_t n_ids) {
-  int rc = grow(c, (void**)&c->d_pods, &c->pods_cap, n, sizeof(ksg_pod));
+int grow_arena(ksg_ctx* c, size_t bytes, uint32_t groups) {
+  int rc = grow(c, (void**)&c->d_arena, &c->arena_cap, std::max<size_t>(bytes, 4096), 1);
   if (rc) return rc;
-  rc = grow(c, (void**)&c->d_ids, &c->ids_cap, std::max<size_t>(n_ids, 1), sizeof(uint32_t));
+  c->d_rng = reinterpret_cast<uint64_t*>(c->d_arena + kArRng);
+  c->d_fctl = c->d_arena + kArCtl;
+  c->d_run = reinterpret_cast<KsgWinRun*>(c->d_arena + kArCtl);
+  c->d_pods = reinterpret_cast<ksg_pod*>(c->d_arena + ar_pods(groups));
+  return KSG_OK;
+}
+
+int stage_batch(ksg_ctx* c, const ksg_pod* pods, uint32_t n, const uint32_t* ids, size_t n_ids,
+                const uint64_t* rng_state, uint32_t groups) {
+  const size_t po = ar_pods(groups), pb = (size_t)n * sizeof(ksg_pod), ib = n_ids * sizeof(uint32_t);
+  const size_t total = po + pb + std::max<size_t>(ib, sizeof(uint32_t));
+  int rc = grow_arena(c, total, groups);
   if (rc) return rc;
-  const size_t pb = (size_t)n * sizeof(ksg_pod), ib = n_ids * sizeof(uint32_t);
-  if ((rc = grow_host(c, &c->h_up, &c->h_up_cap, pb + ib))) return rc;
-  memcpy(c->h_up, pods, pb);
-  if (n_ids) memcpy(c->h_up + pb, ids, ib);
-  HIPCHK(c, hipMemcpyAsync(c->d_pods, c->h_up, pb, hipMemcpyHostToDevice, c->st));
-  if (n_ids) HIPCHK(c, hipMemcpyAsync(c->d_ids, c->h_up + pb, ib, hipMemcpyHostToDevice, c->st));
+  c->d_ids = reinterpret_cast<uint32_t*>(c->d_arena + po + pb);
+  if ((rc = grow_host(c, &c->h_up, &c->h_up_cap, total))) return rc;
+  memcpy(c->h_up + po, pods, pb);
+  if (n_ids) memcpy(c->h_up + po + pb, ids, ib);
+  size_t from = po;
+  if (rng_state) {
+    memset(c->h_up, 0, po);
+    memcpy(c->h_up + kArRng, rng_state, 8);
+    *reinterpret_cast<KsgWinRun*>(c->h_up + kArCtl) = KsgWinRun{0, n, 0, 0, {0, 0, 0, 0}};
+    from = 0;
+  }
+  HIPCHK(c, hipMemcpyAsync(c->d_arena + from, c->h_up + from, po + pb + ib - from, hipMemcpyHostToDevice, c->st));
   return KSG_OK;
 }
 
@@ -768,6 +801,78 @@
   while ((e = hipEventQuery(c->ev_wait)) == hipErrorNotReady) {
   }
   if (e != hipSuccess) return fail(c, KSG_ERR_HIP, "hipEventQuery: %s", hipGetErrorString(e));
+  return KSG_OK;
+}
+
+int ensure_ret(ksg_ctx* c, size_t n) {
+  if (c->h_ret && c->ret_cap >= n) return KSG_OK;
+  const size_t nc = std::max<size_t>(n, std::max<size_t>(c->ret_cap * 2, 1024));
+  if (c->h_ret) (void)hipHostFree(c->h_ret);
+  c->h_ret = c->d_ret = nullptr;
+  c->ret_cap = 0;
+  const size_t bytes = sizeof(KsgRetRec) + nc * sizeof(int32_t);
+  HIPCHK(c, hipHostMalloc((void**)&c->h_ret, bytes, hipHostMallocCoherent | hipHostMallocMapped));
+  memset(c->h_ret, 0, bytes);
+  void* dp = nullptr;
+  HIPCHK(c, hipHostGetDevicePointer(&dp, c->h_ret, 0));
+  c->d_ret = static_cast<uint8_t*>(dp);
+  c->ret_cap = nc;
+  return KSG_OK;
+}
+
+int wait_ret(ksg_ctx* c, uint32_t tag, hipEvent_t ev1, KsgWinRun* run, uint64_t* rng) {
+  KsgRetRec* const q = reinterpret_cast<KsgRetRec*>(c->h_ret);
+  for (uint32_t spin = 1; __atomic_load_n(&q->tag_tail, __ATOMIC_ACQUIRE) != tag; ++spin) {
+    if (spin & 4095u) continue;
+    const hipError_t e = hipEventQuery(ev1);
+    if (e == hipErrorNotReady) continue;
+    if (e != hipSuccess) return fail(c, KSG_ERR_HIP, "hipEventQuery: %s", hipGetErrorString(e));
+    if (__atomic_load_n(&q->tag_tail, __ATOMIC_ACQUIRE) == tag) break;
+    return fail(c, KSG_ERR_STATE, "window round %u ended without its return record", tag);
+  }
+  memcpy(run, &q->run, sizeof *run);
+  memcpy(rng, &q->rng, sizeof *rng);
+  if (__atomic_load_n(&q->tag_head, __ATOMIC_ACQUIRE) != tag)
+    return fail(c, KSG_ERR_STATE, "window round %u: torn return record", tag);
+  return KSG_OK;
+}
+
+int fold_lazy(ksg_ctx* c) {
+  if (!c->lazy.on) return KSG_OK;
+  const ksg_ctx::Lazy z = c->lazy;
+  c->lazy.on = false;
+  ksg_ctx::EvSet& s = c->evs[z.set];
+  (void)hipSetDevice(c->device);
+  HIPCHK(c, hipEventSynchronize(s.ev1));
+  float ms = 0.f;
+  HIPCHK(c, hipEventElapsedTime(&ms, s.ev0, s.ev1));
+  double ea = 0.0, eb = 0.0, et = 0.0;
+  uint32_t nt = 0;
+  for (uint32_t k = z.es ? (z.es - z.ev_off) % z.es : 0u; z.es && k < z.K; k += z.es) {
+    float a = 0.f, t0 = 0.f, b = 0.f;
+    if (z.fused) {
+      HIPCHK(c, hipEventElapsedTime(&b, s.wev[3 * k], s.wev[3 * k + 3]));
+    } else {
+      HIPCHK(c, hipEventElapsedTime(&a, s.wev[3 * k], s.wev[3 * k + 1]));
+      HIPCHK(c, hipEventElapsedTime(&t0, s.wev[3 * k + 1], s.wev[3 * k + 2]));
+      HIPCHK(c, hipEventElapsedTime(&b, s.wev[3 * k + 2], s.wev[3 * k + 3]));
+    }
+    ea += a;
+    et += t0;
+    eb += b;
+    ++nt;
+  }
+  const double ka = nt ? ea * z.K / nt : 0.0, kb = nt ? eb * z.K / nt : 0.0, kt = nt ? et * z.K / nt : 0.0;
+  c->totals[1] += ms;
+  c->totals[2] += ka;
+  c->totals[3] += kb;
+  c->totals[18] += kt;
+  if (z.into_last) {
+    c->last_ms = ms;
+    c->last_kms[0] += ka;
+    c->last_kms[1] += kb;
+    c->last_t0ms += kt;
+  }
   return KSG_OK;
 }
 
@@ -1164,11 +1269,14 @@
   hipError_t e = hipSetDevice(device);
   if (e != hipSuccess) return bail(fail(c, KSG_ERR_HIP, "hipSetDevice(%d): %s", device, hipGetErrorString(e)));
   if ((e = hipStreamCreateWithFlags(&c->st, hipStreamNonBlocking)) != hipSuccess ||
-      (e = hipEventCreateWithFlags(&c->ev0, kTimingEvent)) != hipSuccess ||
-      (e = hipEventCreateWithFlags(&c->ev1, kTimingEvent)) != hipSuccess ||
+      (e = hipEventCreateWithFlags(&c->evs[0].ev0, kTimingEvent)) != hipSuccess ||
+      (e = hipEventCreateWithFlags(&c->evs[0].ev1, kTimingEvent)) != hipSuccess ||
+      (e = hipEventCreateWithFlags(&c->evs[1].ev0, kTimingEvent)) != hipSuccess ||
+      (e = hipEventCreateWithFlags(&c->evs[1].ev1, kTimingEvent)) != hipSuccess ||
       (e = hipEventCreateWithFlags(&c->ev_wait, hipEventDisableTiming)) != hipSuccess)
     return bail(fail(c, KSG_ERR_HIP, "stream/event: %s", hipGetErrorString(e)));
   c->spin_wait = !(getenv("KSG_SPIN_WAIT") && atoi(getenv("KSG_SPIN_WAIT")) == 0);
+  c->mailbox = !(getenv("KSG_BATCH_MAILBOX") && atoi(getenv("KSG_BATCH_MAILBOX")) == 0);
   c->srv_enabled = !(getenv("KSG_SERVE") && atoi(getenv("KSG_SERVE")) == 0);
   c->srv_stamps = getenv("KSG_SERVE_STAMPS") && atoi(getenv("KSG_SERVE_STAMPS")) != 0;
   c->srv_debug = getenv("KSG_SERVE_DEBUG") && atoi(getenv("KSG_SERVE_DEBUG")) != 0;
@@ -1193,11 +1301,11 @@
   int rc;
   if (const char* wenv = getenv("KSG_WINDOW")) c->window = (uint32_t)atoi(wenv);
   if (const char* kev = getenv("KSG_KERNEL_EVENTS")) c->ev_stride = (uint32_t)std::max(atoi(kev), 0);
-  if ((rc = dalloc(c, &c->d_rng, 1, nullptr)) || (rc = dalloc(c, &c->d_summary, 4, nullptr)) ||
-      (rc = dalloc(c, &c->d_run, 1, nullptr)))
+  if ((rc = dalloc(c, &c->d_summary, 4, nullptr)) || (rc = grow_arena(c, 0, 0)) ||
+      (rc = grow_host(c, &c->h_up, &c->h_up_cap, 4096)))
     return bail(rc);
-  if ((e = hipHostMalloc((void**)&c->h_run, sizeof(KsgWinRun), hipHostMallocDefault)) != hipSuccess)
-    return bail(fail(c, KSG_ERR_HIP, "hipHostMalloc: %s", hipGetErrorString(e)));
+  if ((e = hipMemsetAsync(c->d_arena, 0, c->arena_cap, c->st)) != hipSuccess)
+    return bail(fail(c, KSG_ERR_HIP, "hipMemsetAsync: %s", hipGetErrorString(e)));
   c->win_fused = !(getenv("KSG_FUSED") && atoi(getenv("KSG_FUSED")) == 0);
   {
     int cus = 0;
@@ -1207,10 +1315,6 @@
     if (c->fused_grid == 0) c->win_fused = false;
     if (const char* fw = getenv("KSG_FUSED_MAX_WORDS")) c->fused_max_words = (uint32_t)std::max(atoi(fw), 0);
   }
-  if ((e = hipMalloc((void**)&c->d_fctl, kFctlBytes)) != hipSuccess ||
-      (e = hipHostMalloc((void**)&c->h_fctl, kFctlBytes, hipHostMallocDefault)) != hipSuccess)
-    return bail(fail(c, KSG_ERR_HIP, "fused window control: %s", hipGetErrorString(e)));
-  memset(c->h_fctl, 0, kFctlBytes);
   *out = c;
   return KSG_OK;
 }
@@ -1243,6 +1347,7 @@
     KSG_LOCK(c);
     (void)hipSetDevice(c->device);
     (void)srv_stop(c);
+    (void)fold_lazy(c);
   }
   if (c->srv_stamped && srv_grid(c)) {
     const double n = (double)c->srv_stamped;
@@ -1258,17 +1363,15 @@
   (void)hipSetDevice(c->device);
   if (c->st) (void)hipStreamSynchronize(c->st);
   free_cluster(c);
-  void* scratch[] = {c->d_pods, c->d_ids, c->d_fail, c->d_score, c->d_rec_send, c->d_rec_recv, c->d_dpart,
-                     c->d_dglobal, c->d_out, c->d_rng, c->d_summary, c->d_patch, c->d_shard_wlo,
-                     c->d_winsum, c->d_xsend, c->d_xrecv, c->d_run, c->d_dcnt, c->d_admit, c->d_one,
+  void* scratch[] = {c->d_arena, c->d_fail, c->d_score, c->d_rec_send, c->d_rec_recv, c->d_dpart,
+                     c->d_dglobal, c->d_out, c->d_summary, c->d_patch, c->d_shard_wlo,
+                     c->d_winsum, c->d_xsend, c->d_xrecv, c->d_dcnt, c->d_admit, c->d_one,
                      c->d_t0img, c->d_draws, c->d_etmax, c->d_epsoft, c->d_ethist, c->d_xcodes, c->d_xhist};
   for (void* p : scratch)
     if (p) (void)hipFree(p);
   if (c->comm) ncclCommDestroy(c->comm);
   if (c->h_xsend) (void)hipHostFree(c->h_xsend);
-  if (c->h_run) (void)hipHostFree(c->h_run);
-  if (c->h_fctl) (void)hipHostFree(c->h_fctl);
-  if (c->d_fctl) (void)hipFree(c->d_fctl);
+  if (c->h_ret) (void)hipHostFree(c->h_ret);
   if (c->h_up) (void)hipHostFree(c->h_up);
   if (c->h_dn) (void)hipHostFree(c->h_dn);
   if (c->h_map) (void)hipHostFree(c->h_map);
@@ -1276,13 +1379,15 @@
   if (c->srv_grid) (void)hipFree(c->srv_grid);
   if (c->srv_fail) (void)hipHostFree(c->srv_fail);
   if (c->h_xrecv) (void)hipHostFree(c->h_xrecv);
-  if (c->ev0) (void)hipEventDestroy(c->ev0);
-  if (c->ev1) (void)hipEventDestroy(c->ev1);
+  for (auto& s : c->evs) {
+    if (s.ev0) (void)hipEventDestroy(s.ev0);
+    if (s.ev1) (void)hipEventDestroy(s.ev1);
+    for (auto& e : s.wev)
+      if (e) (void)hipEventDestroy(e);
+  }
   if (c->ev_wait) (void)hipEventDestroy(c->ev_wait);
   if (c->ev_x0) (void)hipEventDestroy(c->ev_x0);
   if (c->ev_x1) (void)hipEventDestroy(c->ev_x1);
-  for (auto& e : c->wev)
-    if (e) (void)hipEventDestroy(e);
   if (c->st) (void)hipStreamDestroy(c->st);
   delete c;
   return KSG_OK;
@@ -1297,6 +1402,7 @@
   if (int rs_ = srv_stop(c)) return rs_;
   HIPCHK(c, hipSetDevice(c->device));
   HIPCHK(c, hipStreamSynchronize(c->st));
+  if (int rf = fold_lazy(c)) return rf;
   if (n_nodes && !nodes) return fail(c, KSG_ERR_ARG, "nodes == NULL");
   if (n_pairs == 0) n_pairs = 1;
   for (uint32_t i = 0; i < n_nodes; ++i) {
@@ -1915,6 +2021,7 @@
   if (int rs = cluster_ok(c)) return rs;
   HIPCHK(c, hipSetDevice(c->device));
   c->last_ms = 0.0;
+  c->lazy.into_last = false;
   if (n == 0) return KSG_OK;
   if (c->N == 0) {
     for (uint32_t i = 0; i < n; ++i) out_nodes[i] = KSG_OUT_NONODES;
@@ -1927,24 +2034,39 @@
     c->last_hus[k] += std::chrono::duration<double, std::micro>(t - t_last).count();
     t_last = t;
   };
-  for (uint32_t i = 0; i < n; ++i) {
-    int rc = check_pod(c, pods + i, ids, n_ids);
-    if (rc) return rc;
-    if (c->pods.count(pods[i].uid) || c->dfr_uids.count(pods[i].uid))
-      return fail(c, KSG_ERR_ARG, "pod %u: duplicate uid", i);
+  int rc;
+  if (!c->patches.empty() && (rc = flush_patches(c))) return rc;
+  uint32_t fg_up = 0;
+  if (c->window && c->win_fused && !c->xchg) {
+    const KsgDev fullg = full_geometry(c);
+    if (ksg_win_fused_ok(fullg))
+      fg_up = std::min(ksg_win_fused_groups(fullg, std::min(c->window, ksg_win_max_window(fullg))), kFctlGroups);
+  }
+  const size_t dn_rng = ((size_t)n * 4 + 7) & ~(size_t)7;
+  if ((rc = ensure_out(c, n)) || (rc = grow_host(c, &c->h_dn, &c->h_dn_cap, dn_rng + 8 + sizeof(KsgWinRun))) ||
+      (c->mailbox && (rc = ensure_ret(c, n))))
+    return rc;
+  if (c->lazy.on) c->evset = c->lazy.set ^ 1;
+  ksg_ctx::EvSet& evs = c->evs[c->evset];
+  if ((rc = stage_batch(c, pods, n, ids, n_ids, rng_state, fg_up))) return rc;
+  HIPCHK(c, hipEventRecord(evs.ev0, c->st));
+  hphase(1);
+  for (uint32_t i = 0; i < n && rc == KSG_OK; ++i) {
+    rc = check_pod(c, pods + i, ids, n_ids);
+    if (rc == KSG_OK && (c->pods.count(pods[i].uid) || c->dfr_uids.count(pods[i].uid)))
+      rc = fail(c, KSG_ERR_ARG, "pod %u: duplicate uid", i);
   }
   hphase(0);
-  int rc;
-  if ((rc = note_requests(c, pods, n))) return rc;
-  if (c->dfr_neg && (rc = flush_deferred(c))) return rc;
-  if ((rc = flush_patches(c))) return rc;
-  if ((rc = upload_pods(c, pods, n, ids, n_ids))) return rc;
-  if ((rc = ensure_out(c, n))) return rc;
-  const size_t dn_rng = ((size_t)n * 4 + 7) & ~(size_t)7;
-  if ((rc = grow_host(c, &c->h_dn, &c->h_dn_cap, dn_rng + 8))) return rc;
+  if (rc == KSG_OK) rc = note_requests(c, pods, n);
+  if (rc == KSG_OK && c->dfr_neg) rc = flush_deferred(c);
+  if (rc == KSG_OK) rc = flush_patches(c);
+  if (rc) {
+    (void)hipStreamSynchronize(c->st);
+    return rc;
+  }
   bool tail_queued = false;
   auto enqueue_tail = [&]() -> int {
-    HIPCHK(c, hipEventRecord(c->ev1, c->st));
+    HIPCHK(c, hipEventRecord(evs.ev1, c->st));
     HIPCHK(c, hipMemcpyAsync(c->h_dn, c->d_out, (size_t)n * 4, hipMemcpyDeviceToHost, c->st));
     HIPCHK(c, hipMemcpyAsync(c->h_dn + dn_rng, c->d_rng, 8, hipMemcpyDeviceToHost, c->st));
     return KSG_OK;
@@ -1955,7 +2077,8 @@
   std::unordered_set<uint64_t> st_uids;
   auto overlap_work = [&]() -> int {
     if (stashed) return KSG_OK;
-    int rc2 = flush_deferred(c);
+    int rc2 = fold_lazy(c);
+    if (rc2 == KSG_OK) rc2 = flush_deferred(c);
     if (rc2) return rc2;
     hphase(4);
     st_pods.assign(pods, pods + n);
@@ -1979,12 +2102,9 @@
   } guard{c};
   if (c->dev.dbg & 16384) c->dbg_fail_next = true;
   guard.armed = true;
-  HIPCHK(c, hipMemcpyAsync(c->d_rng, rng_state, 8, hipMemcpyHostToDevice, c->st));
-  HIPCHK(c, hipEventRecord(c->ev0, c->st));
   c->last_stats[0] = c->last_stats[1] = c->last_stats[2] = c->last_stats[3] = 0;
   c->last_kms[0] = c->last_kms[1] = c->last_kms[2] = c->last_t0ms = 0;
   c->last_wsum = 0;
-  hphase(1);
   const ksg_pod_ext* dext = nullptr;
   if (c->ext_on) {
     if ((rc = grow(c, (void**)&c->d_pext, &c->pext_cap, n, sizeof(ksg_pod_ext)))) return rc;
@@ -1995,6 +2115,8 @@
     }
     dext = c->d_pext;
   }
+  bool from_mb = false;
+  uint64_t mb_rng = 0;
   if (use_window(c, pods, n)) {
     const KsgDev full = full_geometry(c);
     uint32_t W = std::min(c->window, ksg_win_max_window(full));
@@ -2084,32 +2206,40 @@
     uint32_t pos = 0, K = round_k(n);
     c->last_kms[0] = c->last_kms[1] = c->last_kms[2] = c->last_t0ms = 0;
     c->last_wsum = 0;
+    const bool mb = c->mailbox && plain && !c->xchg;
+    bool mb_hole = false, first_round = true;
+    KsgWinRun* const h_ctl = reinterpret_cast<KsgWinRun*>(c->h_up + kArCtl);
+    KsgWinRun* const h_run = reinterpret_cast<KsgWinRun*>(c->h_dn + dn_rng + 8);
+    std::vector<hipEvent_t>& wev = evs.wev;
     hphase(2);
     while (pos < n) {
-      if (c->wev.size() < 3 * (size_t)K + 1) {
-        const size_t old = c->wev.size();
-        c->wev.resize(3 * (size_t)K + 1, nullptr);
-        for (size_t i = old; i < c->wev.size(); ++i) HIPCHK(c, hipEventCreateWithFlags(&c->wev[i], kTimingEvent));
+      if (wev.size() < 3 * (size_t)K + 1) {
+        const size_t old = wev.size();
+        wev.resize(3 * (size_t)K + 1, nullptr);
+        for (size_t i = old; i < wev.size(); ++i) HIPCHK(c, hipEventCreateWithFlags(&wev[i], kTimingEvent));
       }
       const uint32_t es = std::min(c->ev_stride, K);
       const uint32_t ev_off = es ? c->ev_phase++ % es : 0u;
-      *c->h_run = KsgWinRun{pos, n, 0, 0, {0, 0, 0, 0}};
-      if (fused) {
-        *reinterpret_cast<KsgWinRun*>(c->h_fctl) = *c->h_run;
-        HIPCHK(c, hipMemcpyAsync(c->d_fctl, c->h_fctl, kFctlRuns + (size_t)2 * fgroups * 8 * sizeof(uint32_t),
-                                 hipMemcpyHostToDevice, c->st));
-      } else {
-        HIPCHK(c, hipMemcpyAsync(c->d_run, c->h_run, sizeof(KsgWinRun), hipMemcpyHostToDevice, c->st));
+      if (!first_round) {
+        *h_ctl = KsgWinRun{pos, n, 0, 0, {0, 0, 0, 0}};
+        HIPCHK(c, hipMemcpyAsync(c->d_fctl, h_ctl, ar_ctl_bytes(fused ? fgroups : 0u), hipMemcpyHostToDevice, c->st));
       }
-      HIPCHK(c, hipEventRecord(c->wev[0], c->st));
+      first_round = false;
+      if (mb) {
+        if (++c->ret_tag == 0) c->ret_tag = 1;
+        x.ret = KsgRet{reinterpret_cast<int32_t*>(c->d_ret + sizeof(KsgRetRec)),
+                       reinterpret_cast<KsgRetRec*>(c->d_ret), c->ret_tag, 0, K, 0};
+      }
+      HIPCHK(c, hipEventRecord(wev[0], c->st));
       for (uint32_t k = 0; k < K; ++k) {
+        x.ret.k = k;
         const bool evk = es && (k + ev_off) % es == 0;
-        if (evk && k > 0) HIPCHK(c, hipEventRecord(c->wev[3 * k], c->st));
+        if (evk && k > 0) HIPCHK(c, hipEventRecord(wev[3 * k], c->st));
         if (fused) {
           KsgFused f{c->d_pods, c->d_ids, fruns + ((k + 1) & 1), fcnt, k & 1u, fgroups};
           HIPCHK(c, ksg_launch_win_fused(full, W, fruns + (k & 1), c->d_winsum, x, c->d_rng, c->d_out, f,
                                          c->fused_grid, c->st));
-          if (evk) HIPCHK(c, hipEventRecord(c->wev[3 * k + 3], c->st));
+          if (evk) HIPCHK(c, hipEventRecord(wev[3 * k + 3], c->st));
           continue;
         }
         if (anti) {
@@ -2130,36 +2260,47 @@
                                       (anti || esc || d1) ? reinterpret_cast<uint64_t*>(c->d_xsend + fit_off) : nullptr,
                                       x.dmb, rr ? reinterpret_cast<uint64_t*>(c->d_xsend + x.b_off) : nullptr, x.dz,
                                       c->st, dext, x.tmax, x.psoft));
-        if (evk) HIPCHK(c, hipEventRecord(c->wev[3 * k + 1], c->st));
+        if (evk) HIPCHK(c, hipEventRecord(wev[3 * k + 1], c->st));
         if (c->xchg && (rc = allgather(c, c->d_xsend, c->d_xrecv, x.blk))) return rc;
         if (plain) HIPCHK(c, ksg_launch_win_t0(full, W, c->d_run, x, c->st));
-        if (evk) HIPCHK(c, hipEventRecord(c->wev[3 * k + 2], c->st));
+        if (evk) HIPCHK(c, hipEventRecord(wev[3 * k + 2], c->st));
         HIPCHK(c, ksg_launch_win_resolve(full, W, c->d_run, c->d_winsum, x, c->d_rng, c->d_out, c->st));
-        if (evk) HIPCHK(c, hipEventRecord(c->wev[3 * k + 3], c->st));
+        if (evk) HIPCHK(c, hipEventRecord(wev[3 * k + 3], c->st));
       }
-      HIPCHK(c, hipMemcpyAsync(c->h_run, fused ? fruns + (K & 1) : c->d_run, sizeof(KsgWinRun), hipMemcpyDeviceToHost,
-                               c->st));
-      if ((rc = enqueue_tail())) return rc;
-      hphase(3);
-      if ((rc = overlap_work())) return rc;
-      if ((rc = wait_device(c))) return rc;
+      KsgWinRun r;
+      if (mb) {
+        HIPCHK(c, hipEventRecord(evs.ev1, c->st));
+        hphase(3);
+        if ((rc = overlap_work())) return rc;
+        if ((rc = wait_ret(c, c->ret_tag, evs.ev1, &r, &mb_rng))) return rc;
+      } else {
+        HIPCHK(c, hipMemcpyAsync(h_run, fused ? fruns + (K & 1) : c->d_run, sizeof(KsgWinRun), hipMemcpyDeviceToHost,
+                                 c->st));
+        if ((rc = enqueue_tail())) return rc;
+        hphase(3);
+        if ((rc = overlap_work())) return rc;
+        if ((rc = wait_device(c))) return rc;
+        r = *h_run;
+      }
       hphase(5);
-      const KsgWinRun r = *c->h_run;
       if (r.windows > 0 && r.pos > pos) {
         const double ppw = (double)(r.pos - pos) / (double)r.windows;
         ppw_est = ppw_est > 0.0 ? 0.5 * ppw_est + 0.5 * ppw : ppw;
         if (!c->xchg) c->ppw_est = ppw_est;
       }
+      const bool ends = mb && !mb_hole && r.halt == 0 && r.pos >= n && !c->dbg_fail_next;
+      if (ends) c->lazy = ksg_ctx::Lazy{true, true, c->evset, K, es, ev_off, fused};
+      else if (mb) HIPCHK(c, hipEventSynchronize(evs.ev1));
       double ea = 0.0, eb = 0.0, et = 0.0;
       uint32_t nt = 0;
-      for (uint32_t k = es ? (es - ev_off) % es : 0u; es && k < K; k += es) {
+      for (uint32_t k = es ? (es - ev_off) % es : 0u; es && k < K && !ends; k += es) {
         float a = 0.f, t0 = 0.f, b = 0.f;
         if (fused) {
-          HIPCHK(c, hipEventElapsedTime(&b, c->wev[3 * k], c->wev[3 * k + 3]));
+          HIPCHK(c, hipEventElapsedTime(&b, wev[3 * k], wev[3 * k + 3]));
         } else {
-          HIPCHK(c, hipEventElapsedTime(&a, c->wev[3 * k], c->wev[3 * k + 1]));
-          HIPCHK(c, hipEventElapsedTime(&t0, c->wev[3 * k + 1], c->wev[3 * k + 2]));
-          HIPCHK(c, hipEventElapsedTime(&b, c->wev[3 * k + 2], c->wev[3 * k + 3]));
+          HIPCHK(c, hipEventElapsedTime(&a, wev[3 * k], wev[3 * k + 1]));
+          HIPCHK(c, hipEventElapsedTime(&t0, wev[3 * k + 1], wev[3 * k + 2]));
+          HIPCHK(c, hipEventElapsedTime(&b, wev[3 * k + 2], wev[3 * k + 3]));
         }
         ea += a;
         et += t0;
@@ -2187,8 +2328,10 @@
       if (r.halt == KSG_HALT_BADCOUNT || r.pos < pos || r.pos > n)
         return fail(c, KSG_ERR_STATE, "window resolver: bad progress (halt %u, pos %u -> %u)", r.halt, pos, r.pos);
       pos = r.pos;
-      tail_queued = pos >= n && r.halt != KSG_HALT_OVERSIZE;
+      tail_queued = pos >= n && r.halt != KSG_HALT_OVERSIZE && !(mb && mb_hole);
+      from_mb = mb && tail_queued;
       if (r.halt == KSG_HALT_OVERSIZE) {
+        mb_hole = true;
         if (!c->xchg) {
           HIPCHK(c, ksg_launch_batch(c->R, anti, c->dev, c->d_pods + pos, c->d_ids, 1, c->d_rng,
                                      c->d_out + pos, c->st, dext ? dext + pos : nullptr));
@@ -2224,11 +2367,16 @@
     if ((rc = wait_device(c))) return rc;
     hphase(6);
   }
-  memcpy(out_nodes, c->h_dn, (size_t)n * 4);
-  memcpy(rng_state, c->h_dn + dn_rng, 8);
-  float ms = 0.f;
-  HIPCHK(c, hipEventElapsedTime(&ms, c->ev0, c->ev1));
-  c->last_ms = ms;
+  if (from_mb) {
+    memcpy(out_nodes, c->h_ret + sizeof(KsgRetRec), (size_t)n * 4);
+    memcpy(rng_state, &mb_rng, 8);
+  } else {
+    memcpy(out_nodes, c->h_dn, (size_t)n * 4);
+    memcpy(rng_state, c->h_dn + dn_rng, 8);
+    float ms = 0.f;
+    HIPCHK(c, hipEventElapsedTime(&ms, evs.ev0, evs.ev1));
+    c->last_ms = ms;
+  }
   if (!stashed) {
     return fail(c, KSG_ERR_STATE, "internal: batch replay inputs missing");
   }
@@ -2325,6 +2473,7 @@
 int ksg_last_batch_kernel_ms(ksg_ctx* c, double* out3) {
   if (!c || !out3) return KSG_ERR_ARG;
   KSG_LOCK(c);
+  if (int rc = fold_lazy(c)) return rc;
   for (int i = 0; i < 3; ++i) out3[i] = c->last_kms[i];
   return KSG_OK;
 }
@@ -2332,6 +2481,7 @@
 int ksg_batch_totals(ksg_ctx* c, double* out24) {
   if (!c || !out24) return KSG_ERR_ARG;
   KSG_LOCK(c);
+  if (int rc = fold_lazy(c)) return rc;
   for (int k = 0; k < 24; ++k) out24[k] = c->totals[k];
   return KSG_OK;
 }
@@ -2339,6 +2489,7 @@
 int ksg_last_batch_host_us(ksg_ctx* c, double* out8) {
   if (!c || !out8) return KSG_ERR_ARG;
   KSG_LOCK(c);
+  if (int rc = fold_lazy(c)) return rc;
   for (int k = 0; k < 8; ++k) out8[k] = c->last_hus[k];
   return KSG_OK;
 }
@@ -2369,6 +2520,7 @@
 int ksg_last_batch_ms(ksg_ctx* c, double* ms) {
   if (!c || !ms) return KSG_ERR_ARG;
   KSG_LOCK(c);
+  if (int rc = fold_lazy(c)) return rc;
   *ms = c->last_ms;
   return KSG_OK;
 }
@@ -2686,7 +2838,7 @@
     if (ext && ((rc = check_ext_range(c, ext + i, n_ids)) || (rc = check_taint_ids(c, ext + i, ids)))) return rc;
   }
   if ((rc = flush_patches(c))) return rc;
-  if ((rc = upload_pods(c, pods, n, ids, n_ids))) return rc;
+  if ((rc = stage_batch(c, pods, n, ids, n_ids, nullptr, 0))) return rc;
   const ksg_pod_ext* dext = nullptr;
   if (ext) {
     if ((rc = grow(c, (void**)&c->d_pext, &c->pext_cap, n, sizeof(ksg_pod_ext)))) return rc;
```

Result: faster. 824,300 pods/s (median of 5 runs) (+5.2%).
